# wangkenpu/rsrgan

Measured on AMD Instinct MI355X. Metric: GAN train frames/sec (G+D step), 257-dim LPS->40-dim MFCC, higher is better.
Workload: dtype f32

## Files before the change

rsrgan_amd/csrc/capi_ops.cpp:

```cpp
#include "capi_common.h"

extern "C" {

int rsrgan_op_launch_floor(int32_t n, int32_t mode, double* us_per_launch, void* stream) {
  if (n <= 0 || !us_per_launch) { set_error("op_launch_floor: bad argument"); return RSRGAN_ERR_INVALID; }
  static float* buf = nullptr;
  if (!buf && hipMalloc((void**)&buf, 2 * 65536 * 4 * sizeof(float)) != hipSuccess) { set_error("hipMalloc failed"); return RSRGAN_ERR_HIP; }
  hipStream_t s = nullptr;
  hipGraph_t g = nullptr; hipGraphExec_t ge = nullptr;
  hipEvent_t e0 = nullptr, e1 = nullptr;
  int rc = RSRGAN_ERR_HIP;
  do {
    if (hipStreamCreateWithFlags(&s, hipStreamNonBlocking) != hipSuccess) break;
    if (hipMemsetAsync(buf, 0, 2 * 65536 * 4 * sizeof(float), s) != hipSuccess) break;
    if (hipStreamBeginCapture(s, hipStreamCaptureModeThreadLocal) != hipSuccess) break;
    launch_floor_chain(buf, buf + 65536 * 4, n, mode, s);
    if (hipStreamEndCapture(s, &g) != hipSuccess) break;
    if (hipGraphInstantiate(&ge, g, nullptr, nullptr, 0) != hipSuccess) break;
    if (hipEventCreate(&e0) != hipSuccess || hipEventCreate(&e1) != hipSuccess) break;
    if (hipGraphLaunch(ge, s) != hipSuccess) break;
    if (hipEventRecord(e0, s) != hipSuccess || hipGraphLaunch(ge, s) != hipSuccess || hipEventRecord(e1, s) != hipSuccess) break;
    if (hipEventSynchronize(e1) != hipSuccess) break;
    float ms = 0.f;
    if (hipEventElapsedTime(&ms, e0, e1) != hipSuccess) break;
    *us_per_launch = 1e3 * ms / n;
    rc = RSRGAN_OK;
  } while (0);
  if (rc != RSRGAN_OK) set_error("op_launch_floor: HIP call failed");
  if (e0) (void)hipEventDestroy(e0);
  if (e1) (void)hipEventDestroy(e1);
  if (ge) (void)hipGraphExecDestroy(ge);
  if (g) (void)hipGraphDestroy(g);
  if (s) (void)hipStreamDestroy(s);
  (void)stream;
  return rc;
}

static const size_t g_op_ws_floats = (size_t)32 << 20;
static const size_t g_op_scratch_floats = (size_t)2 << 20;
static float* op_ws() {
  static float* ws = nullptr;
  if (!ws && hipMalloc((void**)&ws, g_op_ws_floats * sizeof(float)) != hipSuccess) ws = nullptr;
  return ws;
}
static float* op_scratch() {
  static float* sc = nullptr;
  if (!sc && hipMalloc((void**)&sc, g_op_scratch_floats * sizeof(float)) != hipSuccess) sc = nullptr;
  return sc;
}
struct WorkersScope {
  int saved;
  explicit WorkersScope(int w) : saved(g_gemm_workers) { if (w > 0) g_gemm_workers = w; }
  ~WorkersScope() { g_gemm_workers = saved; }
};

int rsrgan_op_gemm(const float* A, int32_t lda, int32_t a_kc, const float* B, int32_t ldb, int32_t b_kc, float* C, int32_t ldc,
                   int32_t M, int32_t N, int32_t K, const float* bias, int32_t act, float alpha, int32_t accumulate, void* stream) {
  if (!A || !B || !C || (lda & 3) || (ldb & 3)) { set_error("op_gemm: null pointer or leading dimension not a multiple of 4"); return RSRGAN_ERR_INVALID; }
  float* ws = op_ws();
  launch_gemm(A, lda, a_kc != 0, B, ldb, b_kc != 0, C, ldc, M, N, K, bias, act, alpha, accumulate != 0, (hipStream_t)stream,
              ws, ws ? g_op_ws_floats : 0);
  OP_LAUNCHED("op_gemm");
}

int rsrgan_op_gemm2(const float* A, int32_t lda, int32_t a_kc, const float* A2, int32_t lda2, int32_t M1, const float* B, int32_t ldb,
                    int32_t b_kc, float* C, int32_t ldc, int32_t M, int32_t N, int32_t K, const float* bias, int32_t act, float alpha,
                    int32_t accumulate, int32_t map_rows_per, int64_t map_outer, int64_t map_inner, int32_t workers, int32_t force_cfg,
                    void* stream) {
  OP_REFUSE(!A || !B || !C, "op_gemm2: null pointer (A, B or C)");
  OP_REFUSE(M <= 0 || N <= 0 || K <= 0, "op_gemm2: M, N, K must be positive (got %d, %d, %d)", M, N, K);
  OP_REFUSE((lda & 3) || (ldb & 3) || (ldc & 3) || (A2 && (lda2 & 3)), "op_gemm2: leading dimension not a multiple of 4 (lda %d, lda2 %d, ldb %d, ldc %d)", lda, lda2, ldb, ldc);
  OP_REFUSE(workers < 0 || workers > 256, "op_gemm2: workers = %d outside 0 (default) .. 256", workers);
  OP_REFUSE(force_cfg < -1 || force_cfg > 7, "op_gemm2: force_cfg = %d outside -1 (planner) .. 7", force_cfg);
  OP_REFUSE(map_rows_per < 0, "op_gemm2: row map with rows_per = %d", map_rows_per);
  if (map_rows_per > 0) {
    OP_REFUSE(A2 != nullptr, "op_gemm2: A2 together with a row map");
    OP_REFUSE(b_kc != 0, "op_gemm2: a row map together with b_kcontig");
    OP_REFUSE((map_outer & 3) || (map_inner & 3), "op_gemm2: row map strides not multiples of 4 (outer %lld, inner %lld)", (long long)map_outer, (long long)map_inner);
  }
  if (A2) {
    OP_REFUSE(a_kc != 0, "op_gemm2: A2 together with a_kcontig (the stacked operand is m-contiguous)");
    OP_REFUSE(M1 <= 0 || M1 >= M, "op_gemm2: M1 = %d outside (0, M = %d)", M1, M);
    OP_REFUSE(M1 & 3, "op_gemm2: M1 = %d is not a multiple of 4: every kernel moves the stacked operand in 16-byte chunks", M1);
  }
  float* ws = op_ws();
  {
    WorkersScope wsc(workers);
    const GemmRowMap ma{map_rows_per, (long long)map_outer, (long long)map_inner};
    launch_gemm_mapped(A, lda, ma, A2, lda2, M1, a_kc != 0, B, ldb, b_kc != 0, C, ldc, M, N, K, bias, act, alpha, accumulate != 0,
                       (hipStream_t)stream, ws, ws ? g_op_ws_floats : 0, force_cfg);
  }
  OP_LAUNCHED("op_gemm2");
}

int rsrgan_op_gemm_batch(int32_t nb, const float* const* A, int32_t lda, const float* const* A2, int32_t lda2, int32_t M1,
                         const float* const* B, int32_t ldb, float* const* C, int32_t ldc, int32_t M, int32_t N, int32_t K,
                         int32_t accumulate, int32_t workers, void* stream) {
  OP_REFUSE(nb < 1 || nb > 64, "op_gemm_batch: nb = %d outside 1 .. 64 (more than %d: not applicable)", nb, GEMM_MAXB);
  OP_REFUSE(!A || !B || !C, "op_gemm_batch: null pointer table (A, B or C)");
  for (int b = 0; b < nb; ++b) OP_REFUSE(!A[b] || !B[b] || !C[b] || (A2 && !A2[b]), "op_gemm_batch: null pointer in problem %d", b);
  OP_REFUSE(M <= 0 || N <= 0 || K <= 0, "op_gemm_batch: M, N, K must be positive (got %d, %d, %d)", M, N, K);
  OP_REFUSE((lda & 3) || (ldb & 3) || (ldc & 3) || (A2 && (lda2 & 3)), "op_gemm_batch: leading dimension not a multiple of 4 (lda %d, lda2 %d, ldb %d, ldc %d)", lda, lda2, ldb, ldc);
// ... 17 lines not shown
                           int32_t accumulate, void* stream) {
  OP_REFUSE(n < 1 || n > GEMM16_MAXB, "op_gemm16_batch: n = %d outside the table (1 .. %d)", n, GEMM16_MAXB);
  OP_REFUSE(!A || !B || !C, "op_gemm16_batch: null pointer table (A, B or C)");
  for (int p = 0; p < n; ++p) OP_REFUSE(!A[p] || !B[p] || !C[p] || (A2 && !A2[p]), "op_gemm16_batch: null pointer in problem %d", p);
  OP_REFUSE(M <= 0 || N <= 0 || K <= 0, "op_gemm16_batch: M, N, K must be positive (got %d, %d, %d)", M, N, K);
  OP_REFUSE((lda & 3) || (ldb & 3) || (ldc & 3) || (A2 && (lda2 & 3)), "op_gemm16_batch: leading dimension not a multiple of 4 (lda %d, lda2 %d, ldb %d, ldc %d)", lda, lda2, ldb, ldc);
  if (A2) {
    OP_REFUSE(M1 <= 0 || M1 >= M, "op_gemm16_batch: M1 = %d outside (0, M = %d)", M1, M);
    OP_REFUSE(M1 & 3, "op_gemm16_batch: M1 = %d is not a multiple of 4: k_gemm16 loads the stacked operand as float4", M1);
  }
  Gemm16Batch bt{};
  bt.n = n;
  for (int p = 0; p < n; ++p) { bt.A[p] = A[p]; bt.A2[p] = A2 ? A2[p] : nullptr; bt.B[p] = B[p]; bt.C[p] = C[p]; }
  float* ws = op_ws();
  launch_gemm16_batch(bt, lda, lda2, M1, ldb, ldc, M, N, K, accumulate != 0, (hipStream_t)stream, ws, ws ? g_op_ws_floats : 0);
  OP_LAUNCHED("op_gemm16_batch");
}

int rsrgan_op_gemm_last_plan(int32_t out[8]) {
  OP_REFUSE(!out, "op_gemm_last_plan: null pointer");
  const GemmPlanRecord& r = g_gemm_last_plan;
  out[0] = r.cls; out[1] = r.bm; out[2] = r.bn; out[3] = r.W; out[4] = r.n_dp; out[5] = r.fixup; out[6] = r.splits; out[7] = r.Ur;
  return RSRGAN_OK;
}

int rsrgan_op_lstm_colsums(int32_t nb, const float* const* dz, const float* const* cprev, const float* const* ccur, float* const* db,
                           float* const* dwi, float* const* dwf, float* const* dwo, int32_t rows, int32_t H, void* stream) {
  OP_REFUSE(nb < 1 || nb > 4, "op_lstm_colsums: nb = %d outside the table (1 .. 4)", nb);
  OP_REFUSE(!dz || !cprev || !ccur || !db || !dwi || !dwf || !dwo, "op_lstm_colsums: null pointer table");
  for (int p = 0; p < nb; ++p)
    OP_REFUSE(!dz[p] || !cprev[p] || !ccur[p] || !db[p] || !dwi[p] || !dwf[p] || !dwo[p], "op_lstm_colsums: null pointer in layer %d", p);
  OP_REFUSE(rows <= 0 || H <= 0, "op_lstm_colsums: rows and H must be positive (got %d, %d)", rows, H);
  OP_REFUSE((size_t)nb * 64 * 7 * (size_t)H > g_op_scratch_floats, "op_lstm_colsums: nb x 64 x 7 x H = %zu floats of partials exceed the entry's scratch", (size_t)nb * 64 * 7 * (size_t)H);
  float* sc = op_scratch();
  if (!sc) { set_error("op_lstm_colsums: hipMalloc failed"); return RSRGAN_ERR_HIP; }
  if (nb == 1) launch_lstm_colsums(dz[0], cprev[0], ccur[0], db[0], dwi[0], dwf[0], dwo[0], rows, H, sc, (hipStream_t)stream);
  else {
    ColsumsBatch cb{};
    cb.n = nb;
    for (int p = 0; p < nb; ++p) { cb.dz[p] = dz[p]; cb.cprev[p] = cprev[p]; cb.ccur[p] = ccur[p]; cb.db[p] = db[p]; cb.dwi[p] = dwi[p]; cb.dwf[p] = dwf[p]; cb.dwo[p] = dwo[p]; }
    launch_lstm_colsums_batch(cb, rows, H, sc, (hipStream_t)stream);
  }
  OP_LAUNCHED("op_lstm_colsums");
}

int rsrgan_op_colsum(const float* a, int32_t lda, const float* b, int32_t ldb, float* out, int32_t rows, int32_t cols, int32_t tall,
                     void* stream) {
  OP_REFUSE(!a || !out, "op_colsum: null pointer (a or out)");
  OP_REFUSE(rows <= 0 || cols <= 0, "op_colsum: rows and cols must be positive (got %d, %d)", rows, cols);
  OP_REFUSE(lda < cols || (b && ldb < cols), "op_colsum: leading dimension below cols = %d (lda %d, ldb %d)", cols, lda, ldb);
  OP_REFUSE(tall && b, "op_colsum: the tall form has no multiplier b");
  OP_REFUSE((size_t)(tall ? 512 : 64) * (size_t)cols > g_op_scratch_floats, "op_colsum: cols = %d exceeds the entry's scratch", cols);
  float* sc = op_scratch();
  if (!sc) { set_error("op_colsum: hipMalloc failed"); return RSRGAN_ERR_HIP; }
  if (tall) launch_colsum_tall(a, lda, out, rows, cols, sc, g_op_scratch_floats, (hipStream_t)stream);
  else launch_colsum(a, lda, b, ldb, out, rows, cols, sc, (hipStream_t)stream);
  OP_LAUNCHED("op_colsum");
}

int rsrgan_op_bnl_fold(const float* Wx, const float* Wh, const float* const bn[12], const float* bias, int32_t P, int32_t H, float* KxT,
                       int32_t ldI, float* KhT, int32_t ldP, float* bias_f, float* ca, float* cb, void* stream) {
  OP_REFUSE(!Wx || !Wh || !bn || !bias || !KxT || !KhT || !bias_f || !ca || !cb, "op_bnl_fold: null pointer");
  for (int k = 0; k < 12; ++k) OP_REFUSE(!bn[k], "op_bnl_fold: null pointer in bn[%d]", k);
  OP_REFUSE(P <= 0 || H <= 0, "op_bnl_fold: P and H must be positive (got %d, %d)", P, H);
  OP_REFUSE(ldI < P || ldP < P, "op_bnl_fold: leading dimension below P = %d (ldI %d, ldP %d)", P, ldI, ldP);
  OP_REFUSE((long long)H * 4 * (long long)(ldI > ldP ? ldI : ldP) > (1ll << 28), "op_bnl_fold: 4H x ld exceeds the entry's 2^28 floats");
  BnlFold f{};
  f.Wx = Wx; f.Wh = Wh; f.bias = bias;
  for (int k = 0; k < 12; ++k) f.bn[k] = bn[k];
  f.P = P; f.H = H; f.ldI = ldI; f.ldP = ldP; f.eps = 1e-3f;
  f.KxT = KxT; f.KhT = KhT; f.bias_f = bias_f; f.ca = ca; f.cb = cb;
  launch_bnl_fold(f, (hipStream_t)stream);
  OP_LAUNCHED("op_bnl_fold");
}

static float* op_conv_ft(size_t floats) {
  static thread_local float* ft = nullptr;
  static thread_local size_t cap = 0;
  if (floats > cap) {
    if (ft) { (void)hipDeviceSynchronize(); (void)hipFree(ft); ft = nullptr; cap = 0; }
    if (hipMalloc((void**)&ft, floats * sizeof(float)) != hipSuccess) { ft = nullptr; return nullptr; }
    cap = floats;
  }
  return ft;
}
static inline int op_pad4(int n) { return (n + 3) & ~3; }
#define OP_CONV_SHAPE(who) \
  OP_REFUSE(C < 1 || N < 1 || S < 1 || W < 1 || fw < 1, who ": C, N, S, W, fw must be positive (got %d, %d, %d, %d, %d)", C, N, S, W, fw); \
  OP_REFUSE(R < 1, who ": R = %d frames", R); \
  OP_REFUSE((long long)R * S * W > (1 << 24), who ": R x S x W = %lld positions exceed the entry's 2^24", (long long)R * S * W)

int rsrgan_op_conv_supported(int32_t C, int32_t N, int32_t S, int32_t W, int32_t fw) {
  OP_REFUSE(C < 1 || N < 1 || S < 1 || W < 1 || fw < 1, "op_conv_supported: C, N, S, W, fw must be positive (got %d, %d, %d, %d, %d)", C, N, S, W, fw);
  return (conv_fwd_supported(C, N, S, W, fw) ? 1 : 0) | (conv_wgrad_supported(C, N, S, W, fw) ? 2 : 0);
}

int64_t rsrgan_op_conv_ws_floats(int32_t C, int32_t R_max, int32_t S, int32_t W, int32_t fw) {
  OP_REFUSE(C < 1 || R_max < 1 || S < 1 || W < 1 || fw < 1, "op_conv_ws_floats: C, R_max, S, W, fw must be positive (got %d, %d, %d, %d, %d)", C, R_max, S, W, fw);
  return (int64_t)conv_wgrad_ws_floats(C, R_max, S, W, fw);
}

int rsrgan_op_conv_fwd(const float* in, int32_t ldc_in, int32_t C, const float* F, int32_t ldf, int32_t flip, const float* bias, int32_t relu,
                       const float* mask, float* out, int32_t ldc_out, int32_t N, int32_t R, int32_t S, int32_t W, int32_t fw, void* stream) {
  OP_REFUSE(!in || !F || !out, "op_conv_fwd: null pointer (in, F or out)");
  OP_CONV_SHAPE("op_conv_fwd");
  OP_REFUSE((ldc_in & 3) || (ldc_out & 3) || (ldf & 3), "op_conv_fwd: leading dimension not a multiple of 4 (ldc_in %d, ldc_out %d, ldf %d)", ldc_in, ldc_out, ldf);
  OP_REFUSE(ldc_in < op_pad4(C) || ldc_out < op_pad4(N) || ldf < (flip ? C : N),
            "op_conv_fwd: leading dimension below its row (ldc_in %d for C = %d, ldc_out %d for N = %d, ldf %d for %d filter columns)", ldc_in, C, ldc_out, N, ldf, flip ? C : N);
  OP_REFUSE(((size_t)in & 15) || ((size_t)out & 15) || ((size_t)mask & 15), "op_conv_fwd: in, out or mask not 16-byte aligned");
// ... 568 lines not shown
      case 0: launch_sumsq(FP(0), ct, FP(1), s); break;
      case 1: launch_dw_reduce(FP(0), (size_t)d[3], (int)d[4], dsrc, FP(1), ct, FP(2), s); break;
      case 2: launch_l2(FP(0), FP(1), ct, FP(2), FP(3), s); break;
      case 3: launch_apply_sgd(FP(0), FP(1), FP(2), ct, FP(3), FP(4), s); break;
      default: launch_apply_adam(FP(0), FP(1), FP(2), FP(3), FP(4), ct, FP(5), FP(6), s, (int)d[3]); break;
    }
    OP_LAUNCH_OK(WHO);
    HIPC(hipStreamSynchronize(s));
    return RSRGAN_OK;
  });
}
#undef WHO

#define WHO "op_step_elem"
int rsrgan_op_step_elem(int32_t op, const void* const* ptrs, const int64_t* dims, const float* fl, void* stream) {
  OP_REFUSE(!ptrs, WHO ": null table (ptrs)");
  OP_REFUSE(op < 0 || op > 8, WHO ": op = %d outside 0 .. 8", op);
  OP_REFUSE(op != 3 && !dims, WHO ": null table (dims)");
  OP_REFUSE((op == 0 || op >= 5) && !fl, WHO ": null table (fl: the clip bounds, the betas, keep or alpha)");
  const int64_t* d = dims;
  hipStream_t s = (hipStream_t)stream;
  switch (op) {
    case 0: {
      OP_DIM("T", d[0], 1); OP_DIM("Nd", d[1], 1); OP_LD("ldl", d[3], 1); OP_FLAG("clip_on", d[4]);
      OP_REFUSE(d[2] < 0 || d[2] > d[1], WHO ": n_real = %lld outside 0 .. Nd = %lld", (long long)d[2], (long long)d[1]);
      OP_REFUSE(d[0] * d[1] > (1 << 24), WHO ": T x Nd above the entry's 2^24");
      OP_BP("Nd", d[1], d[5], d[6]); OP_BP("n_real", d[2], d[5], d[6]);
      OP_PTR("logits", ptrs[0], 4); OP_OPT("dlogits", ptrs[1], 4); OP_PTR("t_real", ptrs[2], 4); OP_PTR("t_fake", ptrs[3], 4); OP_PTR("loss3", ptrs[4], 4);
      launch_lsgan(FP(0), (int)d[3], FP(1), (int)d[0], (int)d[1], (int)d[2], FP(2), FP(3), FP(4), s, d[4] != 0, fl[0], fl[1], (int)d[5], (int)d[6]);
      break;
    }
    case 1: {
      OP_DIM("T", d[0], 1); OP_DIM("Nd", d[1], 1); OP_DIM("dR", d[3], 1); OP_MUL4("dR", d[3]);
      OP_REFUSE(d[3] + 3 > 64, WHO ": dR = %lld above 60 (k_dhead2 sums 3 + dR <= 64 quantities)", (long long)d[3]);
      OP_REFUSE(d[2] < 0 || d[2] > d[1], WHO ": n_real = %lld outside 0 .. Nd = %lld", (long long)d[2], (long long)d[1]);
      OP_REFUSE(d[0] * d[1] > (1 << 24), WHO ": T x Nd above the entry's 2^24");
      OP_FLAG("want_grads", d[8]); OP_FLAG("want_wgrads", d[9]);
      OP_LD("ldt", d[4], d[3]); OP_MUL4("ldt", d[4]); OP_LD("ldw", d[5], 1); OP_LD("ldl", d[6], 1);
      if (d[8]) { OP_LD("ldo", d[7], d[3]); OP_MUL4("ldo", d[7]); }
      OP_BP("Nd", d[1], d[10], d[11]); OP_BP("n_real", d[2], d[10], d[11]);
      static const char* const names[12] = {"top", "w", "b", "logits", "dlogits", "dout", "gw", "gb", "t_real", "t_fake", "loss3", "part"};
      for (int i = 0; i < 12; ++i) {
        const bool wanted = i < 4 || i > 7 || (i < 6 ? d[8] != 0 : d[9] != 0);
        const int align = (i == 0 || i == 5) ? 16 : 4;
        if (wanted) OP_PTR(names[i], ptrs[i], align); else OP_OPT(names[i], ptrs[i], align);
      }
      const int64_t need = (d[0] * d[1] + 63) / 64 * (DH_MAXR + 3);
      OP_REFUSE(d[12] < need, WHO ": part of %lld floats below ceil(T x Nd / 64) x %d = %lld", (long long)d[12], DH_MAXR + 3, (long long)need);
      DHeadArgs a{};
      a.top = FP(0); a.ldt = (int)d[4]; a.w = FP(1); a.ldw = (int)d[5]; a.b = FP(2);
      a.logits = FP(3); a.ldl = (int)d[6]; a.dlogits = FP(4); a.dout = FP(5); a.ldo = (int)d[7]; a.gw = FP(6); a.gb = FP(7);
      a.T = (int)d[0]; a.Nd = (int)d[1]; a.n_real = (int)d[2]; a.dR = (int)d[3]; a.t_real = FP(8); a.t_fake = FP(9); a.loss3 = FP(10); a.part = FP(11);
      a.want_grads = (int)d[8]; a.want_wgrads = (int)d[9]; a.Bp = (int)d[10]; a.Bt = (int)d[11];
      launch_dhead(a, s);
      break;
    }
    case 2: {
      OP_DIM("rows", d[0], 1); OP_DIM("D", d[1], 1); OP_LD("ld", d[2], d[1]); OP_FLAG("accumulate", d[3]);
      OP_REFUSE(d[0] * d[2] > ((int64_t)1 << 30), WHO ": rows x ld above the entry's 2^30");
      OP_BP("rows", d[0], d[4], d[5]);
      OP_REFUSE(d[6] < 1024, WHO ": scratch of %lld floats below launch_mse's 1024", (long long)d[6]);
      OP_PTR("y", ptrs[0], 4); OP_PTR("lab", ptrs[1], 4); OP_OPT("dy", ptrs[2], 4); OP_PTR("lambda", ptrs[3], 4); OP_PTR("loss", ptrs[4], 4); OP_PTR("scratch", ptrs[5], 4);
      launch_mse(FP(0), FP(1), (int)d[2], FP(2), (int)d[0], (int)d[1], FP(3), d[3] != 0, FP(4), FP(5), s, (int)d[4], (int)d[5]);
      break;
    }
    case 3:
      OP_PTR("l4", ptrs[0], 4); OP_PTR("lambda", ptrs[1], 4);
      launch_g_total(FP(0), FP(1), s);
      break;
    case 4:
      OP_DIM("n", d[0], 1);
      OP_PTR("partial", ptrs[0], 4); OP_PTR("l2_scale", ptrs[1], 4); OP_PTR("out", ptrs[2], 4);
      launch_l2_total(FP(0), (int)d[0], FP(1), FP(2), s);
      break;
    case 5: {
      const bool g = d[0] == DYN_G_LR && d[1] == DYN_ADAM_LRT, dd = d[0] == DYN_D_LR && d[1] == DYN_ADAM_LRT_D;
      OP_REFUSE(!g && !dd, WHO ": slots (%lld, %lld) are neither (%d, %d) (G) nor (%d, %d) (D)", (long long)d[0], (long long)d[1], (int)DYN_G_LR,
                (int)DYN_ADAM_LRT, (int)DYN_D_LR, (int)DYN_ADAM_LRT_D);
      OP_REFUSE(!(fl[0] >= 0.f && fl[0] < 1.f) || !(fl[1] >= 0.f && fl[1] < 1.f), WHO ": beta1 = %g or beta2 = %g outside [0, 1)", (double)fl[0], (double)fl[1]);
      OP_PTR("dyn", ptrs[0], 4); OP_PTR("t", ptrs[1], 4);
      launch_adam_tick(FP(0), (int*)ptrs[1], (double)fl[0], (double)fl[1], s, (int)d[0], (int)d[1]);
      break;
    }
    case 6: case 7: case 8: {
      OP_DIM("rows", d[0], 1); OP_DIM("cols", d[1], 1); OP_LD("ld", d[2], d[1]);
      OP_REFUSE(d[0] * d[2] > ((int64_t)1 << 30), WHO ": rows x ld above the entry's 2^30");
      if (op != 8) OP_REFUSE(!(fl[0] > 0.f && fl[0] <= 1.f), WHO ": keep = %g outside (0, 1]", (double)fl[0]);
      if (op == 6) OP_REFUSE(d[4] < 0 || d[4] > (1 << 24), WHO ": thr = %lld outside 0 .. 2^24", (long long)d[4]);
      OP_PTR(op == 8 ? "h" : "y", ptrs[0], 4);
      if (op != 6) OP_PTR("d", ptrs[1], 4);
      if (op == 6) launch_dropout_fwd(FP(0), (size_t)d[0], (int)d[1], (int)d[2], (unsigned long long)d[3], (unsigned)d[4], fl[0], s);
      else if (op == 7) launch_dropout_bwd(FP(0), FP(1), (size_t)d[0], (int)d[1], (int)d[2], fl[0], s);
      else launch_lrelu_bwd(FP(0), FP(1), (size_t)d[0], (int)d[1], (int)d[2], fl[0], s);
      break;
    }
  }
  OP_LAUNCHED(WHO);
}
#undef WHO

#define OP_JOB_NAME(buf, name, j) char buf[48]; snprintf(buf, sizeof(buf), "%s of job %d", name, (int)(j))
#define WHO "op_layout"
int rsrgan_op_layout(int32_t op, const void* const* ptrs, const int64_t* dims, const float* fl, void* stream) {
  OP_REFUSE(!ptrs || !dims, WHO ": null table (ptrs or dims)");
  OP_REFUSE(op < 0 || op > 18, WHO ": op = %d outside 0 .. 18", op);
  OP_REFUSE(op == 14 && !fl, WHO ": null table (fl: the fill value)");
  const int64_t* d = dims;
  const int64_t lim = (int64_t)1 << 30;
  hipStream_t s = (hipStream_t)stream;
  switch (op) {
    case 0: case 1: {
      OP_DIM("B", d[0], 1); OP_DIM("T", d[1], 1); OP_DIM("D", d[2], 1); OP_LD("ld", d[3], d[2]);
      OP_REFUSE(d[0] * d[1] * d[3] > lim || d[0] > 65535, WHO ": B x T x ld above the entry's 2^30, or B above the grid's 65535");
      if (op == 1) OP_REFUSE(d[4] < 0 || d[4] > d[0], WHO ": Bt = %lld outside 0 (all rows) .. B = %lld", (long long)d[4], (long long)d[0]);
      OP_PTR("src", ptrs[0], 4); OP_PTR("dst", ptrs[1], 4);
      if (op == 0) launch_pack_tm(FP(0), FP(1), (int)d[0], (int)d[1], (int)d[2], (int)d[3], s);
// ... 205 lines not shown
```

rsrgan_amd/csrc/gemm.hip:

```cpp
#include <algorithm>
#include <type_traits>
#include <cstdio>
#include <cstdlib>

#include "kernels.h"

namespace rsr {

typedef float f32x16 __attribute__((ext_vector_type(16)));
typedef const __attribute__((address_space(1))) void* gptr_t;
typedef __attribute__((address_space(3))) void* lptr_t;

constexpr int GK = 32;
#ifndef RSR_GEMM_MINW
#define RSR_GEMM_MINW 2
#endif
#ifndef RSR_GEMM_ABL
#define RSR_GEMM_ABL 0
#endif
constexpr int BK = 16;
__device__ __attribute__((aligned(16))) float g_zero_chunk[4] = {0.f, 0.f, 0.f, 0.f};
#if RSR_GEMM_ABL & 8
__device__ unsigned long long g_gemm_clk[4];
#endif
// ... 594 lines not shown
        *c = v;
      }
    }
}
template <bool AKC, bool BKC>
__global__ __launch_bounds__(256) void k_gemm16(const float* __restrict__ A, int lda, const float* __restrict__ B, int ldb,
                                              float* __restrict__ C, int ldc, int M, int N, int K,
                                              const float* __restrict__ bias, int act, float alpha, int accumulate,
                                              float* __restrict__ ws, int ldw, int kt_per_split,
                                              const float* __restrict__ A2, int lda2, int M1) {
  gemm16_body<AKC, BKC>(A, lda, B, ldb, C, ldc, M, N, K, bias, act, alpha, accumulate, ws, ldw, kt_per_split, A2, lda2, M1, blockIdx.z);
}
__global__ __launch_bounds__(256) void k_gemm16_b(const Gemm16Batch bt, int lda, int ldb, int ldc, int M, int N, int K, int accumulate,
                                                  float* __restrict__ ws, int ldw, int kt_per_split, int nsplit, int lda2, int M1) {
  const int p = blockIdx.z / nsplit, zs = blockIdx.z - p * nsplit;
  gemm16_body<false, false>(bt.A[p], lda, bt.B[p], ldb, bt.C[p], ldc, M, N, K, nullptr, 0, 0.f, accumulate,
                            ws ? ws + (size_t)p * nsplit * M * ldw : nullptr, ldw, kt_per_split, bt.A2[p], lda2, M1, zs);
}
__global__ __launch_bounds__(256) void k_splitk_reduce_b(const float* __restrict__ ws, int ldw, int splits, const Gemm16Batch bt, int ldc,
                                                         int M, int N, int accumulate) {
  const int p = blockIdx.y;
  const float* w = ws + (size_t)p * splits * M * ldw;
  float* C = bt.C[p];
  const size_t total = (size_t)M * N;
  for (size_t i = (size_t)blockIdx.x * blockDim.x + threadIdx.x; i < total; i += (size_t)gridDim.x * blockDim.x) {
    const int row = (int)(i / N), col = (int)(i % N);
    float v = 0.f;
#pragma unroll 8
    for (int z = 0; z < splits; ++z) v += w[((size_t)z * M + row) * ldw + col];
    float* c = C + (size_t)row * ldc + col;
    if (accumulate) v += *c;
    *c = v;
  }
}

__global__ __launch_bounds__(256) void k_splitk_reduce(const float* __restrict__ ws, int ldw, int splits, float* __restrict__ C,
                                                       int ldc, int M, int N, const float* __restrict__ bias, int act,
                                                       float alpha, int accumulate) {
  const size_t total = (size_t)M * N;
  for (size_t i = (size_t)blockIdx.x * blockDim.x + threadIdx.x; i < total; i += (size_t)gridDim.x * blockDim.x) {
    const int row = (int)(i / N), col = (int)(i % N);
    float v = 0.f;
#pragma unroll 8
    for (int z = 0; z < splits; ++z) v += ws[((size_t)z * M + row) * ldw + col];
    if (bias) v += bias[col];
    if (act == 1) v = fmaxf(v, alpha * v);
    else if (act == 2) v = fmaxf(v, 0.f);
    float* c = C + (size_t)row * ldc + col;
    if (accumulate) v += *c;
    *c = v;
  }
}


constexpr int NBM = 256, NBN = 32, NLDA = 260, NLDB = 36;
template <bool AKC>
__global__ __launch_bounds__(256) void k_gemm_n32(const float* __restrict__ A, int lda, const float* __restrict__ B, int ldb,
                                                  float* __restrict__ C, int ldc, int M, int N, int K,
                                                  const float* __restrict__ bias, int act, float alpha, int accumulate,
                                                  float* __restrict__ ws, int ldw, int kt_per_split) {
  __shared__ __attribute__((aligned(16))) float As[BK][NLDA];
  __shared__ __attribute__((aligned(16))) float Bs[BK][NLDB];
  const int tid = threadIdx.x, lane = tid & 63, w = tid >> 6;
  const int m0 = blockIdx.y * NBM;
  const int l31 = lane & 31, lh = lane >> 5;
  f32x16 acc[2];
#pragma unroll
  for (int i = 0; i < 2; ++i)
#pragma unroll
    for (int r = 0; r < 16; ++r) acc[i][r] = 0.f;
  const int KA = AKC ? ((K + 3) & ~3) : K;
  const int MA = AKC ? M : ((M + 3) & ~3);
  const int NB = (N + 3) & ~3;
  const int nk_all = (K + BK - 1) / BK;
  const int kt0 = blockIdx.z * kt_per_split;
  const int nk = min(nk_all, kt0 + kt_per_split);
  float4 ra[4], rb;
  auto load = [&](int kt) {
    const int k0 = kt * BK;
#pragma unroll
    for (int u = 0; u < 4; ++u) {
      const int idx = tid + 256 * u;
      float4 v = make_float4(0.f, 0.f, 0.f, 0.f);
      if (AKC) {
        const int x = m0 + (idx >> 2), k = k0 + (idx & 3) * 4;
        if (x < MA && k < KA) v = *reinterpret_cast<const float4*>(A + (size_t)x * lda + k);
      } else {
        const int k = k0 + (idx >> 6), x = m0 + (idx & 63) * 4;
        if (k < K && x < MA) v = *reinterpret_cast<const float4*>(A + (size_t)k * lda + x);
      }
      ra[u] = v;
    }
    rb = make_float4(0.f, 0.f, 0.f, 0.f);
    if (tid < 128) {
      const int k = k0 + (tid >> 3), x = (tid & 7) * 4;
      if (k < K && x < NB) rb = *reinterpret_cast<const float4*>(B + (size_t)k * ldb + x);
    }
  };
  auto store = [&]() {
#pragma unroll
    for (int u = 0; u < 4; ++u) {
      const int idx = tid + 256 * u;
      if (AKC) {
        const int x = idx >> 2, k = (idx & 3) * 4;
        As[k + 0][x] = ra[u].x; As[k + 1][x] = ra[u].y; As[k + 2][x] = ra[u].z; As[k + 3][x] = ra[u].w;
      } else {
// ... 149 lines not shown
template <bool AKC, bool BKC, bool MAPA>
void launch_layout(GemmArgs& g, hipStream_t s, float* ws, size_t ws_floats, int force_cfg) {
  static const int cfgs[][2] = {{128, 128}, {96, 128}, {128, 96}, {256, 64}, {256, 32}, {256, 256}, {128, 256}, {256, 128}};
  int best = 0;
  Plan bp{};
  if (force_cfg >= 0 && force_cfg < 8) {
    best = force_cfg;
    bp = plan_cfg(g.M, g.N, g.K, cfgs[best][0], cfgs[best][1], g_gemm_workers, ws, ws_floats);
  } else
  for (int c = 0; c < (switches().gemm_self ? 8 : 5); ++c) {
    if (c >= 5 && (long long)((g.M + cfgs[c][0] - 1) / cfgs[c][0]) * ((g.N + cfgs[c][1] - 1) / cfgs[c][1]) < 2LL * g_gemm_workers) continue;
    Plan pl = plan_cfg(g.M, g.N, g.K, cfgs[c][0], cfgs[c][1], g_gemm_workers, ws, ws_floats);
    if (c == 0 || pl.cost < 0.97 * bp.cost) { best = c; bp = pl; }
  }
  switch (best) {
    case 1: launch_cfg<AKC, BKC, 3, 1, 1, MAPA>(g, bp, s, ws); break;
    case 2: launch_cfg<AKC, BKC, 1, 3, 4, MAPA>(g, bp, s, ws); break;
    case 3: launch_cfg<AKC, BKC, 2, 2, 4, MAPA>(g, bp, s, ws); break;
    case 4: launch_cfg<AKC, BKC, 2, 1, 4, MAPA>(g, bp, s, ws); break;
    case 5: launch_cfg_s<AKC, BKC, 4, 4, 2, MAPA>(g, bp, s, ws); break;
    case 6: launch_cfg_s<AKC, BKC, 2, 4, 2, MAPA>(g, bp, s, ws); break;
    case 7: launch_cfg_s<AKC, BKC, 4, 2, 2, MAPA>(g, bp, s, ws); break;
    default: launch_cfg<AKC, BKC, 2, 2, 2, MAPA>(g, bp, s, ws); break;
  }
}
}

static void launch_gemm16(const float* A, int lda, const float* A2, int lda2, int M1, bool a_kc, const float* B, int ldb, bool b_kc,
                          float* C, int ldc, int M, int N, int K, const float* bias, int act, float alpha, bool accumulate,
                          hipStream_t s, float* ws, size_t ws_floats) {
  const int gx = (N + BN - 1) / BN, gy = (M + BM - 1) / BM;
  const int nk = (K + GBK - 1) / GBK;
  int splits = 1;
  const int ldw = (N + 3) & ~3;
  if (ws && gx * gy < 192 && nk * GBK >= 128) {
    int cap = 64;
    while (cap > 1 && (size_t)cap * M * ldw > ws_floats) --cap;
    splits = pick_splits(gx * gy, nk, (size_t)M * ldw * sizeof(float), cap, 1.2 * GBK / 16, GBK == 16 ? 4 : 2);
  }
  const int per = std::max(1, (nk + splits - 1) / splits);
  splits = std::max(1, (nk + per - 1) / per);
  float* w = splits > 1 ? ws : nullptr;
  dim3 grid(gx, gy, splits), block(256);
  const int acc = accumulate ? 1 : 0;
  g_gemm_last_plan = GemmPlanRecord{GEMM_CLS_GEMM16, BM, BN, 0, 0, 0, splits, 0};
  if (a_kc && !b_kc)
    hipLaunchKernelGGL((k_gemm16<true, false>), grid, block, 0, s, A, lda, B, ldb, C, ldc, M, N, K, bias, act, alpha, acc, w, ldw, per, nullptr, 0, 0);
  else if (a_kc && b_kc)
    hipLaunchKernelGGL((k_gemm16<true, true>), grid, block, 0, s, A, lda, B, ldb, C, ldc, M, N, K, bias, act, alpha, acc, w, ldw, per, nullptr, 0, 0);
  else if (!a_kc && !b_kc)
    hipLaunchKernelGGL((k_gemm16<false, false>), grid, block, 0, s, A, lda, B, ldb, C, ldc, M, N, K, bias, act, alpha, acc, w, ldw, per, A2, lda2, M1);
  else
    hipLaunchKernelGGL((k_gemm16<false, true>), grid, block, 0, s, A, lda, B, ldb, C, ldc, M, N, K, bias, act, alpha, acc, w, ldw, per, A2, lda2, M1);
  if (splits > 1) {
    const size_t total = (size_t)M * N;
    const int blocks = (int)std::min<size_t>(2048, (total + 255) / 256);
    hipLaunchKernelGGL(k_splitk_reduce, dim3(blocks), dim3(256), 0, s, ws, ldw, splits, C, ldc, M, N, bias, act, alpha, acc);
  }
}


void launch_gemm16_batch(const Gemm16Batch& bt, int lda, int lda2, int M1, int ldb, int ldc, int M, int N, int K, bool accumulate,
                         hipStream_t s, float* ws, size_t ws_floats) {
  if (bt.n <= 0 || M <= 0 || N <= 0 || K <= 0) return;
  for (int p = 0; p < bt.n; ++p) require_m1_chunked(bt.A2[p], M1, "launch_gemm16_batch");
  const int gx = (N + BN - 1) / BN, gy = (M + BM - 1) / BM;
  const int nk = (K + GBK - 1) / GBK;
  int splits = 1;
  const int ldw = (N + 3) & ~3;
  if (ws && gx * gy * bt.n < 192 && nk * GBK >= 128) {
    int cap = 64;
    while (cap > 1 && (size_t)cap * bt.n * M * ldw > ws_floats) --cap;
    splits = pick_splits(gx * gy * bt.n, nk, (size_t)M * ldw * sizeof(float), cap, 1.2 * GBK / 16, GBK == 16 ? 4 : 2);
  }
  const int per = std::max(1, (nk + splits - 1) / splits);
  splits = std::max(1, (nk + per - 1) / per);
  float* w = splits > 1 ? ws : nullptr;
  g_gemm_last_plan = GemmPlanRecord{GEMM_CLS_GEMM16_B, BM, BN, 0, 0, 0, splits, 0};
  hipLaunchKernelGGL(k_gemm16_b, dim3(gx, gy, splits * bt.n), dim3(256), 0, s, bt, lda, ldb, ldc, M, N, K, accumulate ? 1 : 0, w, ldw, per,
                     splits, lda2, M1);
  if (splits > 1) {
    const size_t total = (size_t)M * N;
    const int blocks = (int)std::min<size_t>(2048, (total + 255) / 256);
    hipLaunchKernelGGL(k_splitk_reduce_b, dim3(blocks, bt.n), dim3(256), 0, s, ws, ldw, splits, bt, ldc, M, N, accumulate ? 1 : 0);
  }
}

void launch_gemm_mapped(const float* A, int lda, const GemmRowMap& ma, const float* A2, int lda2, int M1, bool a_kc, const float* B, int ldb,
                        bool b_kc, float* C, int ldc, int M, int N, int K, const float* bias, int act, float alpha,
                        bool accumulate, hipStream_t s, float* ws, size_t ws_floats, int force_cfg) {
  if (M <= 0 || N <= 0 || K <= 0) return;
  const bool mapped = ma.rows_per > 0;
  if (!a_kc && !mapped) require_m1_chunked(A2, M1, "launch_gemm_mapped");
  if (mapped && b_kc) { fprintf(stderr, "rsrgan: launch_gemm_mapped: a row map of A with a k-contiguous B is not instantiated\n"); abort(); }
  if (N <= NBN && !b_kc && !A2 && M >= NBM && !mapped && force_cfg < 0) {
    const int gy = (M + NBM - 1) / NBM, nk = (K + BK - 1) / BK, ldw = (N + 3) & ~3;
    int splits = 1;
    if (ws && gy < 192 && nk >= 8) {
      int cap = 64;
      while (cap > 1 && (size_t)cap * M * ldw > ws_floats) --cap;
      splits = pick_splits(gy, nk, (size_t)M * ldw * sizeof(float), cap);
    }
    const int per = std::max(1, (nk + splits - 1) / splits);
    splits = std::max(1, (nk + per - 1) / per);
    float* w = splits > 1 ? ws : nullptr;
    dim3 grid(1, gy, splits), block(256);
    const int acc = accumulate ? 1 : 0;
    g_gemm_last_plan = GemmPlanRecord{GEMM_CLS_N32, NBM, NBN, 0, 0, 0, splits, 0};
    if (a_kc) hipLaunchKernelGGL((k_gemm_n32<true>), grid, block, 0, s, A, lda, B, ldb, C, ldc, M, N, K, bias, act, alpha, acc, w, ldw, per);
    else hipLaunchKernelGGL((k_gemm_n32<false>), grid, block, 0, s, A, lda, B, ldb, C, ldc, M, N, K, bias, act, alpha, acc, w, ldw, per);
    if (splits > 1) {
      const size_t total = (size_t)M * N;
      const int blocks = (int)std::min<size_t>(2048, (total + 255) / 256);
      hipLaunchKernelGGL(k_splitk_reduce, dim3(blocks), dim3(256), 0, s, ws, ldw, splits, C, ldc, M, N, bias, act, alpha, acc);
    }
    return;
  }
  const double outs = (double)M * N;
  if (force_cfg < 0 && !mapped && !(K >= 256 && outs >= 4.0e6) && !(K >= 2048 && outs >= 1.5e6)) {
    launch_gemm16(A, lda, a_kc ? nullptr : A2, lda2, M1, a_kc, B, ldb, b_kc, C, ldc, M, N, K, bias, act, alpha, accumulate, s, ws, ws_floats);
    return;
  }
  GemmArgs g{};
  g.A = A; g.A2 = a_kc ? nullptr : A2; g.B = B; g.bias = bias; g.C = C;
  g.lda = lda; g.lda2 = lda2; g.M1 = M1; g.ldb = ldb; g.ldc = ldc; g.M = M; g.N = N; g.K = K;
  g.act = act; g.accumulate = accumulate ? 1 : 0; g.alpha = alpha;
  g.ma = ma;
  if (mapped) {
    g.A2 = nullptr;
    if (a_kc) launch_layout<true, false, true>(g, s, ws, ws_floats, force_cfg);
    else launch_layout<false, false, true>(g, s, ws, ws_floats, force_cfg);
  }
  else if (a_kc && !b_kc) launch_layout<true, false, false>(g, s, ws, ws_floats, force_cfg);
  else if (a_kc && b_kc) launch_layout<true, true, false>(g, s, ws, ws_floats, force_cfg);
  else if (!a_kc && !b_kc) launch_layout<false, false, false>(g, s, ws, ws_floats, force_cfg);
  else launch_layout<false, true, false>(g, s, ws, ws_floats, force_cfg);
}

bool launch_gemm_batch(int nb, const float* const* A, int lda, const float* const* A2, int lda2, int M1, const float* const* B, int ldb,
                       float* const* C, int ldc, int M, int N, int K, bool accumulate, hipStream_t s, float* ws, size_t ws_floats) {
  const int form = switches().gemm_batch;
  if (!form || nb < 2 || nb > GEMM_MAXB || M <= 0 || N <= 0 || K <= 0 || !ws) return false;
  const double outs = (double)M * N;
  if (!(K >= 256 && outs >= 4.0e6) && !(K >= 2048 && outs >= 1.5e6)) return false;
  if (A2) for (int b = 0; b < nb; ++b) require_m1_chunked(A2[b], M1, "launch_gemm_batch");
  GemmArgs g{};
  g.A = A[0]; g.A2 = A2 ? A2[0] : nullptr; g.B = B[0]; g.bias = nullptr; g.C = C[0];
  g.lda = lda; g.lda2 = lda2; g.M1 = M1; g.ldb = ldb; g.ldc = ldc; g.M = M; g.N = N; g.K = K;
  g.act = 0; g.accumulate = accumulate ? 1 : 0; g.alpha = 0.f;
  g.ma = GemmRowMap{0, 0, 0};
  GemmBatch bt{};
  bt.nb = nb;
  for (int b = 0; b < nb; ++b) { bt.Ab[b] = A[b]; bt.A2b[b] = A2 ? A2[b] : nullptr; bt.Bb[b] = B[b]; bt.Cb[b] = C[b]; }
  const int pad192 = (M + 191) / 192 * 192, pad128 = (M + 127) / 128 * 128;
  if (form == 1 && pad192 < pad128 && 2 * (size_t)g_gemm_workers * 192 * 256 <= ws_floats) {
    const int tn1 = (N + 255) / 256;
    const int bw = switches().gemm_batch_w;
    const Plan pl = plan_cfg(M, nb * tn1 * 256, K, 192, 256, bw ? std::min(bw, g_gemm_workers) : g_gemm_workers, ws, ws_floats);
    if (!pl.whole) { launch_cfg_s<false, false, 3, 4, 2, false, GemmBatch>(g, pl, s, ws, &bt); return true; }
  }
  const int tn1 = (N + 127) / 128;
  const Plan pl = plan_cfg(M, nb * tn1 * 128, K, 128, 128, g_gemm_workers, ws, ws_floats);
  launch_cfg<false, false, 2, 2, 2, false>(g, pl, s, ws, &bt);
  return true;
}

void launch_gemm2(const float* A, int lda, const float* A2, int lda2, int M1, bool a_kc, const float* B, int ldb, bool b_kc,
                  float* C, int ldc, int M, int N, int K, const float* bias, int act, float alpha, bool accumulate,
// ... 13 lines not shown
```

rsrgan_amd/csrc/kernels.h:

```cpp
#pragma once
#include <hip/hip_runtime.h>
#include <stdint.h>

#include <vector>

#include "switches.h"

namespace rsr {

constexpr int MAXJ = 8;

struct Place { int x0, nx, sb, se, nb, w; };
constexpr int JOBMAP_MAX = 768;
struct JobMap { int valid; unsigned char job[JOBMAP_MAX]; };
struct PlanItem { int ncol, nrow; double cost; int mult; };
int plan_places(int n, const PlanItem* items, Place* out);

enum { DYN_G_LR = 0, DYN_D_LR = 1, DYN_LAMBDA = 2, DYN_D_REAL = 3, DYN_D_FAKE = 4, DYN_L2 = 5, DYN_CLIP = 6,
       DYN_B1 = 7, DYN_B2 = 8, DYN_EPS = 9, DYN_EMA = 10, DYN_ADAM_LRT = 11, DYN_ADAM_LRT_D = 12, DYN_COUNT = 16 };

struct FwdGateJob {
  const float* x;
  const float* KxT;
  const float* m;
// ... 221 lines not shown
                 float* splitk_ws = nullptr, size_t splitk_ws_floats = 0);

struct StagePack { const float* src; float* dst; int D, ld; };
struct StageCopy { const void* src; void* dst; int n; };
struct StageJobs { StagePack pack[2]; StageCopy copy[4]; int B, T; int Bt; };
void launch_stage_inputs(const StageJobs& j, hipStream_t s);
void launch_pack_tm(const float* src_bm, float* dst_tm, int B, int T, int D, int ld, hipStream_t s);
void launch_unpack_bm(const float* src_tm, int ld, float* dst_bm, int B, int T, int D, hipStream_t s, int Bt = 0);
void launch_build_d_input(const float* lab_tm, const float* y_tm, const float* noise_r, const float* noise_f,
                          float* xd, int B, int T, int D, int ld, bool with_real, hipStream_t s);
void launch_add_noise_rows(const float* src_tm, const float* noise, float* dst, int B, int T, int D, int ld,
                           int Ns, int row0, hipStream_t s);
void launch_transpose(const float* src, int lds, float* dst, int ldd, int R, int C, hipStream_t s);
void launch_fill(float* p, size_t n, float v, hipStream_t s);
struct SwizzleJob { const float* src; float* dst; int ld, gates, H, C, c0, K1, I, P, kx, nct, nkb, blk_base; };
struct SwizzleList { int n; SwizzleJob j[24]; };
void launch_swizzle_many(SwizzleList& sl, hipStream_t s);
inline size_t swizzle_floats(int nct, int nkb) { return (size_t)nct * nkb * 256; }
struct TransposeJob { const float* src; float* dst; int lds, ldd, R, C, blk_base; };
struct TransposeList { int n; TransposeJob j[16]; };
void launch_transpose_many(TransposeList& tl, hipStream_t s);
size_t conv_prep_floats(int S, int fw, int C);
void launch_conv_prep(const float* F, int ldf_src, int S, int fw, int Cin, int Cout, bool flip, float* Ft, hipStream_t s);
bool conv_fwd_supported(int C, int N, int S, int W, int fw);
void launch_conv_fwd(const float* in, int ldc_in, int C, const float* Ft, const float* bias, bool relu, float* out, int ldc_out, int N,
                     int R, int S, int W, int fw, hipStream_t s,
                     const float* mask = nullptr );
bool conv_wgrad_supported(int C, int N, int S, int W, int fw);
size_t conv_wgrad_ws_floats(int C, int R, int S, int W, int fw);
void launch_conv_wgrad(const float* in, int ldc_in, int C, const float* d, int ldc_d, int N, float* dW, int ldw, float* ws, int R, int S,
                       int W, int fw, hipStream_t s,
                       float* db = nullptr );
enum { CONV_FAM_NONE = 0, CONV_FAM_FWD = 1 , CONV_FAM_FWD4 = 2 ,
       CONV_FAM_WGRAD = 3 , CONV_FAM_WGRAD4 = 4  };
enum { CONV_BR_WHOLE = 1, CONV_BR_MAIN = 2, CONV_BR_REM = 3, CONV_BR_WG_K2 = 1, CONV_BR_WG_ROWS = 2, CONV_BR_WG_SEARCH = 3 };
struct ConvLaunchRecord {
  int family, a0, a1, a2;
  int branch, TW, FB, gx, gy, gz, lds;
  int DH, fpg, groups, nstrips, nkg, PS, waves, gmax;
};
struct ConvPlanRecord { int n; ConvLaunchRecord l[2]; };
extern thread_local ConvPlanRecord g_conv_last_plan;
void launch_im2col(const float* src, size_t row_stride, int ldc, int C, int S, int W, int kh, int kw, float* col, int ldk, size_t M,
                   hipStream_t s);
void launch_expand_c4(const float* src, int ld_src, int n, float* dst, size_t rows, hipStream_t s);
void launch_col2im(const float* dcol, int ldk, int C, int S, int W, int kh, int kw, float* dst, int ldc, size_t M, hipStream_t s);
struct GStateLayer { float *c, *mst; int H, P, ldP, off; };
struct GStateArgs { GStateLayer L[GP_MAXL]; int nl, SF, rows, dir; float* state; size_t slot; const int* mask; };
void launch_gstate(const GStateArgs& a, hipStream_t s);
void launch_window_len(const int* len, int* dst, int n, int t0, int Tw, hipStream_t s);
struct ZeroList { int n; float* p[32]; unsigned len[32]; };
void launch_zero_many(const ZeroList& zl, hipStream_t s);
struct ColsumsBatch { const float* dz[4]; const float* cprev[4]; const float* ccur[4]; float* db[4]; float* dwi[4]; float* dwf[4]; float* dwo[4]; int n; };
void launch_lstm_colsums_batch(const ColsumsBatch& bt, int rows, int H, float* scratch, hipStream_t s);
void launch_lstm_colsums(const float* dz, const float* cprev, const float* ccur, float* db, float* dwi, float* dwf, float* dwo,
                         int rows, int H, float* scratch , hipStream_t s);
void launch_lrelu_bwd(const float* hval, float* d, size_t rows, int cols, int ld, float alpha, hipStream_t s);
void launch_dropout_fwd(float* y, size_t rows, int cols, int ld, unsigned long long key, unsigned thr, float keep, hipStream_t s);
void launch_dropout_bwd(const float* y, float* d, size_t rows, int cols, int ld, float keep, hipStream_t s);
void launch_colsum_tall(const float* a, int lda, float* out, int rows, int cols, float* scratch, size_t scratch_floats, hipStream_t s);

struct BnVars {
  float *beta, *gamma;
  float *mm, *mv, *rm, *rmw, *rs, *rsw;
};
constexpr int BN_STAT_ROWS = 6;
void launch_bn_forward(const float* z, int ldz, float* y, int ldy, int rows, int cols, const BnVars& v, float* stat, int ldc, bool training,
                       bool relu, float* scratch, size_t scratch_floats, hipStream_t s, int calls = 1);
void launch_bn_backward(float* dy, int ldd, const float* y, int ldy, const float* z, int ldz, int rows, int cols, const float* stat, int ldc,
                        float* dbeta, float* dgamma, bool accumulate, bool relu, float* sums, float* scratch, size_t scratch_floats,
                        hipStream_t s, int calls = 1);
void launch_bn_commit(int cols, const BnVars& v, const float* stat, int ldc, int times, hipStream_t s);
struct BnCommit { BnVars v; const float* stat; int cols, ldc, times0, times1; };
struct BnCommitList { int n; BnCommit e[24]; };
void launch_bn_commit_many(const BnCommitList& cl, hipStream_t s);
enum { BN_ROUTE_NONE = 0, BN_ROUTE_SMALL = 1, BN_ROUTE_SLICED = 2, BN_ROUTE_NARROW = 3 };
struct BnPlanRecord { int route, backward, calls, launches, slices, per, pgx, pgy, egrid, q, R; };
extern thread_local BnPlanRecord g_bn_last_plan;
int bn_seq_count(int rows, int Bp, int Bt);
void launch_bn_seq_forward(const float* z, int ldz, float* y, int ldy, int rows, int cols, const BnVars& v, float* stat, int ldc, bool training,
                           bool act, float alpha, int Bp, int Bt, float* scratch, size_t scratch_floats, hipStream_t s);
void launch_bn_seq_backward(float* dy, int ldd, const float* y, int ldy, const float* z, int ldz, int rows, int cols, const float* stat, int ldc,
                            float* dbeta, float* dgamma, bool accumulate, bool act, float alpha, int Bp, int Bt, float* sums, float* scratch,
                            size_t scratch_floats, hipStream_t s);
void launch_bn_seq_fold(float* W, int ldw, int K, int cols, const BnVars& v, float* bias, hipStream_t s);
void launch_feat_batch(const float* raw, long long raw_rows, const int* offsets, int B, int T, int D, int left, int right, const double* mean,
                       const double* stddev, float* out, int* lengths, hipStream_t s);
void launch_feat_frames(const float* pool, long long pool_rows, const int* picks, int N, int D, int left, int right, const double* mean,
                        const double* stddev, float* out, hipStream_t s);
void launch_feat_stream(const float* fresh, long long fresh_rows, const int* table, float* hist, int B, int H, int T, int D, int left, int right,
                        const double* mean, const double* stddev, float* out, int* lengths, hipStream_t s);
void launch_feat_denorm(const float* y, const int* lengths, int B, int T, int D, const double* mean, const double* stddev, double* out,
                        hipStream_t s);
void launch_feat_decode(const uint8_t* blob, long long blob_bytes, const long long* seg, const float* scale, const int* offsets, int B, int D,
                        const double* mean, const double* stddev, float* out, long long out_rows, hipStream_t s);
int wave_frames(int P);
void launch_feat_wave(const void* pcm, int kind, long long n_samples, const long long* seg, const int* offsets, int B, int N, int S, int P,
                      float preemph, const float* window, const float* twiddle, float* out, long long out_rows, hipStream_t s);
constexpr int HIST_MAX_TENSORS = 16;
constexpr int hist_nl() {
  int k = 0;
  for (double v = 1e-12; v < 1e20; v *= 1.1) ++k;
  return 2 * (k + 1) + 1;
}
constexpr int HIST_NL = hist_nl();
constexpr int HIST_REC = 5 + HIST_NL;
struct HistView { const float* x; long long ld, cs; unsigned rows, cols; int clip; };
const std::vector<double>& hist_limits();
bool launch_hist(int n, const HistView* views, float clip_lo, float clip_hi, double* out, hipStream_t s);
void launch_logits_dense(const float* logits, int frame_rows, int B, int T, float* out, bool clip, float clip_lo, float clip_hi, hipStream_t s);
void launch_colsum(const float* a, int lda, const float* b, int ldb, float* out, int rows, int cols,
                   float* scratch , hipStream_t s);

constexpr int DH_MAXR = 64;
struct DHeadArgs {
  const float* top; int ldt; const float* w; int ldw; const float* b;
  float* logits; int ldl; float* dlogits; float* dout; int ldo; float* gw; float* gb;
  int T, Nd, n_real, dR; const float* t_real; const float* t_fake; float* loss3; float* part; int want_grads, want_wgrads;
  int Bp, Bt;
};
void launch_dhead(const DHeadArgs& a, hipStream_t s);
void launch_lsgan(const float* logits, int ldl, float* dlogits, int T, int Nd, int n_real,
                  const float* target_real, const float* target_fake, float* loss3, hipStream_t s,
                  bool clip_on = false, float clip_lo = 0.f, float clip_hi = 0.f, int Bp = 0, int Bt = 0);
void launch_build_joint(const float* x, int ldx, int off, int dim, const float* tail, int ldt, int Dt, float* joint, int ldj,
                        int row0, int R, hipStream_t s);
void launch_slice_cols(const float* src, int lds, int off, float* dst, int ldd, int R, int C, hipStream_t s);
void launch_mse(const float* y, const float* lab, int ld, float* dy, int rows, int D, const float* lambda,
                bool accumulate, float* loss_out, float* scratch , hipStream_t s, int Bp = 0, int Bt = 0);
void launch_g_total(float* l4 , const float* lambda, hipStream_t s);
void launch_copy_f(const float* src, float* dst, int n, hipStream_t s);

struct ChunkTable {
  const int* tensor;
  const int* off;
  const int* len;
  const int* t_first;
  const int* t_count;
  const int* t_l2;
  int n_chunks, n_tensors;
};
void launch_sumsq(const float* g, const ChunkTable& ct, float* partial, hipStream_t s);
void launch_dw_reduce(const float* ws, size_t stride, int ntiles, const long long* src, float* g, const ChunkTable& ct, float* partial, hipStream_t s);
void launch_l2(const float* w, float* g, const ChunkTable& ct, const float* l2_scale, float* partial, hipStream_t s);
void launch_l2_total(const float* partial, int n_chunks, const float* l2_scale, float* out, hipStream_t s);
void launch_apply_sgd(float* w, const float* g, float* ema, const ChunkTable& ct, const float* partial,
                      const float* dyn, hipStream_t s);
void launch_apply_adam(float* w, const float* g, float* m, float* v, float* ema, const ChunkTable& ct,
                       const float* partial, const float* dyn, hipStream_t s, int lrt_slot = DYN_ADAM_LRT);
void launch_adam_tick(float* dyn, int* t, double b1, double b2, hipStream_t s, int lr_slot = DYN_G_LR, int lrt_slot = DYN_ADAM_LRT);
void launch_pad_copy(const float* dense, float* padded, int rows, int cols, int ld, bool to_padded, hipStream_t s);

}
```

rsrgan_amd/csrc/kernels.hip:

```cpp
#include <algorithm>
#include <cstdlib>

#include "kernels.h"

namespace rsr {

typedef float f32x4 __attribute__((ext_vector_type(4)));

__device__ __forceinline__ float sigmoid_(float x) { return 1.0f / (1.0f + expf(-x)); }

#ifdef RSR_TRACE
__device__ unsigned long long g_trace[8192 * 16];
#define TR_BEGIN() do { if (threadIdx.x == 0 && blockIdx.x < 8192) { unsigned long long* t_ = g_trace + (size_t)blockIdx.x * 16; \
    t_[0] = __builtin_amdgcn_s_memrealtime(); t_[1] = __builtin_amdgcn_s_memtime(); \
    t_[14] = __builtin_amdgcn_s_getreg(4 | (0 << 6) | (31 << 11)); t_[15] = __builtin_amdgcn_s_getreg(20 | (0 << 6) | (3 << 11)); \
    for (int i_ = 2; i_ < 14; ++i_) t_[i_] = 0; } } while (0)
#define TR_ID(ptr) do { if (threadIdx.x == 0 && blockIdx.x < 8192) g_trace[(size_t)blockIdx.x * 16 + 12] = (unsigned long long)(size_t)(ptr); } while (0)
#define TR(i) do { if (threadIdx.x == 0 && blockIdx.x < 8192) g_trace[(size_t)blockIdx.x * 16 + (i)] = __builtin_amdgcn_s_memtime(); } while (0)
#define TR_END() do { if (threadIdx.x == 0 && blockIdx.x < 8192) { g_trace[(size_t)blockIdx.x * 16 + 9] = __builtin_amdgcn_s_memtime(); \
    g_trace[(size_t)blockIdx.x * 16 + 13] = __builtin_amdgcn_s_memrealtime(); } } while (0)
#else
#define TR_BEGIN() do { } while (0)
#define TR_ID(ptr) do { } while (0)
#define TR(i) do { } while (0)
// ... 1216 lines not shown
    float* sm = sc + L.H;
    if (a.dir == 0) {
      for (int i = tid; i < L.H; i += blockDim.x) c[i] = sc[i];
      for (int i = tid; i < L.ldP; i += blockDim.x) m[i] = i < L.P ? sm[i] : 0.f;
    } else {
      for (int i = tid; i < L.H; i += blockDim.x) sc[i] = c[i];
      for (int i = tid; i < L.P; i += blockDim.x) sm[i] = m[i];
    }
  }
}
void launch_gstate(const GStateArgs& a, hipStream_t s) {
  if (a.rows <= 0) return;
  hipLaunchKernelGGL(k_gstate, dim3(a.rows), dim3(256), 0, s, a);
}

__global__ void k_window_len(const int* __restrict__ len, int* __restrict__ dst, int n, int t0, int Tw) {
  const int b = blockIdx.x * blockDim.x + threadIdx.x;
  if (b < n) dst[b] = min(max(len[b] - t0, 0), Tw);
}
void launch_window_len(const int* len, int* dst, int n, int t0, int Tw, hipStream_t s) {
  if (n <= 0) return;
  hipLaunchKernelGGL(k_window_len, dim3((n + 255) / 256), dim3(256), 0, s, len, dst, n, t0, Tw);
}

__global__ void k_zero_many(ZeroList zl) {
  const int j = blockIdx.y;
  if (j >= zl.n) return;
  float* p = zl.p[j];
  const size_t n = zl.len[j];
  for (size_t i = (size_t)blockIdx.x * blockDim.x + threadIdx.x; i < n; i += (size_t)gridDim.x * blockDim.x) p[i] = 0.f;
}
void launch_zero_many(const ZeroList& zl, hipStream_t s) {
  if (zl.n == 0) return;
  hipLaunchKernelGGL(k_zero_many, dim3(32, zl.n), dim3(256), 0, s, zl);
}

__global__ void k_fill(float* p, size_t n, float v) {
  for (size_t i = (size_t)blockIdx.x * blockDim.x + threadIdx.x; i < n; i += (size_t)gridDim.x * blockDim.x) p[i] = v;
}
void launch_fill(float* p, size_t n, float v, hipStream_t s) {
  if (n == 0) return;
  const int blocks = (int)min((size_t)2048, (n + 255) / 256);
  hipLaunchKernelGGL(k_fill, dim3(blocks), dim3(256), 0, s, p, n, v);
}

__global__ void k_lrelu_bwd(const float* __restrict__ hval, float* __restrict__ d, size_t rows, int cols, int ld, float alpha) {
  const size_t total = rows * (size_t)cols;
  for (size_t i = (size_t)blockIdx.x * blockDim.x + threadIdx.x; i < total; i += (size_t)gridDim.x * blockDim.x) {
    const size_t r = i / cols; const int c = (int)(i % cols);
    const size_t o = r * ld + c;
    if (!(hval[o] > 0.f)) d[o] *= alpha;
  }
}
void launch_lrelu_bwd(const float* hval, float* d, size_t rows, int cols, int ld, float alpha, hipStream_t s) {
  const size_t total = rows * cols;
  const int blocks = (int)min((size_t)2048, (total + 255) / 256);
  hipLaunchKernelGGL(k_lrelu_bwd, dim3(blocks), dim3(256), 0, s, hval, d, rows, cols, ld, alpha);
}

__global__ void k_drop_tick(unsigned long long* ctr) { if (threadIdx.x == 0) *ctr += 1ull; }
void launch_drop_tick(unsigned long long* ctr, hipStream_t s) { hipLaunchKernelGGL(k_drop_tick, dim3(1), dim3(64), 0, s, ctr); }
__global__ __launch_bounds__(256) void k_dropout_fwd(float* __restrict__ y, size_t rows, int cols, int ld, unsigned long long key, unsigned thr,
                                                     float keep) {
  const size_t n = rows * (size_t)cols;
  for (size_t i = (size_t)blockIdx.x * 256 + threadIdx.x; i < n; i += (size_t)gridDim.x * 256) {
    const size_t r = i / cols;
    float* p = y + r * ld + (i - r * cols);
    const bool on = (unsigned)(splitmix64(key + i) >> 40) < thr;
    *p = on ? *p / keep : 0.f;
  }
}
void launch_dropout_fwd(float* y, size_t rows, int cols, int ld, unsigned long long key, unsigned thr, float keep, hipStream_t s) {
  const size_t n = rows * (size_t)cols;
  if (n == 0) return;
  hipLaunchKernelGGL(k_dropout_fwd, dim3((unsigned)std::min<size_t>((n + 255) / 256, 8192)), dim3(256), 0, s, y, rows, cols, ld, key, thr, keep);
}
__global__ __launch_bounds__(256) void k_dropout_bwd(const float* __restrict__ y, float* __restrict__ d, size_t rows, int cols, int ld, float keep) {
  const size_t n = rows * (size_t)cols;
  for (size_t i = (size_t)blockIdx.x * 256 + threadIdx.x; i < n; i += (size_t)gridDim.x * 256) {
    const size_t r = i / cols, o = r * ld + (i - r * cols);
    d[o] = y[o] > 0.f ? d[o] / keep : 0.f;
  }
}
void launch_dropout_bwd(const float* y, float* d, size_t rows, int cols, int ld, float keep, hipStream_t s) {
  const size_t n = rows * (size_t)cols;
  if (n == 0) return;
  hipLaunchKernelGGL(k_dropout_bwd, dim3((unsigned)std::min<size_t>((n + 255) / 256, 8192)), dim3(256), 0, s, y, d, rows, cols, ld, keep);
}

constexpr int CS_SLICES = 64;
__global__ __launch_bounds__(256) void k_colsum1(const float* __restrict__ a, int lda, const float* __restrict__ b, int ldb,
                                                 float* __restrict__ scratch, int rows, int cols) {
  __shared__ float red[4][64];
  const int c = blockIdx.x * 64 + (threadIdx.x & 63), rl = threadIdx.x >> 6;
  const int per = (rows + CS_SLICES - 1) / CS_SLICES;
  const int rbeg = blockIdx.y * per, rend = min(rows, rbeg + per);
  float s = 0.f;
  if (c < cols) {
    for (int r = rbeg + rl; r < rend; r += 4) {
      const float v = a[(size_t)r * lda + c];
      s += b ? v * b[(size_t)r * ldb + c] : v;
    }
  }
  red[rl][threadIdx.x & 63] = s;
  __syncthreads();
  if (rl == 0 && c < cols)
    scratch[(size_t)blockIdx.y * cols + c] = ((red[0][threadIdx.x] + red[1][threadIdx.x]) + red[2][threadIdx.x]) + red[3][threadIdx.x];
}
__global__ void k_colsum2(const float* __restrict__ scratch, float* __restrict__ out, int cols) {
  const int c = blockIdx.x * blockDim.x + threadIdx.x;
  if (c >= cols) return;
  float s = 0.f;
  for (int i = 0; i < CS_SLICES; ++i) s += scratch[(size_t)i * cols + c];
  out[c] = s;
}
__global__ __launch_bounds__(256) void k_colsum1_n(const float* __restrict__ a, int lda, float* __restrict__ scratch, int rows, int cols,
                                                   int per) {
  __shared__ float red[4][64];
  const int c = blockIdx.x * 64 + (threadIdx.x & 63), rl = threadIdx.x >> 6;
  const int rbeg = blockIdx.y * per, rend = min(rows, rbeg + per);
  float s = 0.f;
  if (c < cols) {
#pragma unroll 4
    for (int r = rbeg + rl; r < rend; r += 4) s += a[(size_t)r * lda + c];
  }
  red[rl][threadIdx.x & 63] = s;
  __syncthreads();
  if (rl == 0 && c < cols)
    scratch[(size_t)blockIdx.y * cols + c] = ((red[0][threadIdx.x] + red[1][threadIdx.x]) + red[2][threadIdx.x]) + red[3][threadIdx.x];
}
__global__ __launch_bounds__(256) void k_colsum2_n(const float* __restrict__ scratch, float* __restrict__ out, int cols, int slices) {
  __shared__ float red[4][64];
  const int c = blockIdx.x * 64 + (threadIdx.x & 63), g = threadIdx.x >> 6;
  float s = 0.f;
  if (c < cols) {
#pragma unroll 4
    for (int i = g; i < slices; i += 4) s += scratch[(size_t)i * cols + c];
  }
  red[g][threadIdx.x & 63] = s;
  __syncthreads();
  if (g == 0 && c < cols) out[c] = ((red[0][threadIdx.x] + red[1][threadIdx.x]) + red[2][threadIdx.x]) + red[3][threadIdx.x];
}
void launch_colsum_tall(const float* a, int lda, float* out, int rows, int cols, float* scratch, size_t scratch_floats, hipStream_t s) {
  int slices = (int)std::min<size_t>(512, scratch_floats / (size_t)std::max(cols, 1));
  slices = std::max(1, std::min(slices, (rows + 63) / 64));
  const int per = (rows + slices - 1) / slices;
  slices = (rows + per - 1) / per;
  hipLaunchKernelGGL(k_colsum1_n, dim3((cols + 63) / 64, slices), dim3(256), 0, s, a, lda, scratch, rows, cols, per);
  hipLaunchKernelGGL(k_colsum2_n, dim3((cols + 63) / 64), dim3(256), 0, s, scratch, out, cols, slices);
}

__global__ __launch_bounds__(256) void k_lstm_colsums1(const float* __restrict__ dz, const float* __restrict__ cprev,
                                                       const float* __restrict__ ccur, float* __restrict__ scratch, int rows, int H) {
  __shared__ float red[7][4][64];
  const int c = blockIdx.x * 64 + (threadIdx.x & 63), rl = threadIdx.x >> 6;
  const int per = (rows + CS_SLICES - 1) / CS_SLICES;
  const int rbeg = blockIdx.y * per, rend = min(rows, rbeg + per);
  float s[7] = {0.f, 0.f, 0.f, 0.f, 0.f, 0.f, 0.f};
  if (c < H) {
#pragma unroll 4
    for (int r = rbeg + rl; r < rend; r += 4) {
      const float* z = dz + (size_t)r * 4 * H + c;
      const float di = z[0], dj = z[H], df = z[2 * H], d_o = z[3 * H];
      const float cp = cprev[(size_t)r * H + c], cc = ccur[(size_t)r * H + c];
      s[0] += di; s[1] += dj; s[2] += df; s[3] += d_o; s[4] += di * cp; s[5] += df * cp; s[6] += d_o * cc;
    }
  }
// ... 21 lines not shown
}
__global__ __launch_bounds__(256) void k_lstm_colsums1_b(const ColsumsBatch bt, float* __restrict__ scratch, int rows, int H) {
  __shared__ float red[7][4][64];
  const int p = blockIdx.z;
  const float* __restrict__ dz = bt.dz[p]; const float* __restrict__ cprev = bt.cprev[p]; const float* __restrict__ ccur = bt.ccur[p];
  scratch += (size_t)p * CS_SLICES * 7 * H;
  const int c = blockIdx.x * 64 + (threadIdx.x & 63), rl = threadIdx.x >> 6;
  const int per = (rows + CS_SLICES - 1) / CS_SLICES;
  const int rbeg = blockIdx.y * per, rend = min(rows, rbeg + per);
  float s[7] = {0.f, 0.f, 0.f, 0.f, 0.f, 0.f, 0.f};
  if (c < H) {
#pragma unroll 4
    for (int r = rbeg + rl; r < rend; r += 4) {
      const float* z = dz + (size_t)r * 4 * H + c;
      const float di = z[0], dj = z[H], df = z[2 * H], d_o = z[3 * H];
      const float cp = cprev[(size_t)r * H + c], cc = ccur[(size_t)r * H + c];
      s[0] += di; s[1] += dj; s[2] += df; s[3] += d_o; s[4] += di * cp; s[5] += df * cp; s[6] += d_o * cc;
    }
  }
#pragma unroll
  for (int k = 0; k < 7; ++k) red[k][rl][threadIdx.x & 63] = s[k];
  __syncthreads();
  if (rl == 0 && c < H) {
    const int x = threadIdx.x;
#pragma unroll
    for (int k = 0; k < 7; ++k)
      scratch[((size_t)blockIdx.y * 7 + k) * H + c] = ((red[k][0][x] + red[k][1][x]) + red[k][2][x]) + red[k][3][x];
  }
}
__global__ void k_lstm_colsums2_b(const float* __restrict__ scratch, const ColsumsBatch bt, int H) {
  const int p = blockIdx.y;
  scratch += (size_t)p * CS_SLICES * 7 * H;
  const int c = blockIdx.x * blockDim.x + threadIdx.x;
  if (c >= H) return;
  float s[7] = {0.f, 0.f, 0.f, 0.f, 0.f, 0.f, 0.f};
#pragma unroll 8
  for (int i = 0; i < CS_SLICES; ++i)
#pragma unroll
    for (int k = 0; k < 7; ++k) s[k] += scratch[((size_t)i * 7 + k) * H + c];
  float* db = bt.db[p];
  db[c] = s[0]; db[H + c] = s[1]; db[2 * H + c] = s[2]; db[3 * H + c] = s[3];
  bt.dwi[p][c] = s[4]; bt.dwf[p][c] = s[5]; bt.dwo[p][c] = s[6];
}
void launch_lstm_colsums_batch(const ColsumsBatch& bt, int rows, int H, float* scratch, hipStream_t s) {
  hipLaunchKernelGGL(k_lstm_colsums1_b, dim3((H + 63) / 64, CS_SLICES, bt.n), dim3(256), 0, s, bt, scratch, rows, H);
  hipLaunchKernelGGL(k_lstm_colsums2_b, dim3((H + 255) / 256, bt.n), dim3(256), 0, s, scratch, bt, H);
}
void launch_lstm_colsums(const float* dz, const float* cprev, const float* ccur, float* db, float* dwi, float* dwf, float* dwo,
                         int rows, int H, float* scratch, hipStream_t s) {
  hipLaunchKernelGGL(k_lstm_colsums1, dim3((H + 63) / 64, CS_SLICES), dim3(256), 0, s, dz, cprev, ccur, scratch, rows, H);
  hipLaunchKernelGGL(k_lstm_colsums2, dim3((H + 255) / 256), dim3(256), 0, s, scratch, db, dwi, dwf, dwo, H);
}

void launch_colsum(const float* a, int lda, const float* b, int ldb, float* out, int rows, int cols, float* scratch, hipStream_t s) {
  hipLaunchKernelGGL(k_colsum1, dim3((cols + 63) / 64, CS_SLICES), dim3(256), 0, s, a, lda, b, ldb, scratch, rows, cols);
  hipLaunchKernelGGL(k_colsum2, dim3((cols + 255) / 256), dim3(256), 0, s, scratch, out, cols);
}

__device__ __forceinline__ float block_sum_1024(float v, float* red) {
  for (int o = 32; o > 0; o >>= 1) v += __shfl_down(v, o, 64);
  const int w = threadIdx.x >> 6;
  if ((threadIdx.x & 63) == 0) red[w] = v;
  __syncthreads();
  float s = 0.f;
  const int nw = (blockDim.x + 63) >> 6;
  for (int i = 0; i < nw; ++i) s += red[i];
  __syncthreads();
  return s;
}

__global__ __launch_bounds__(1024) void k_lsgan(const float* __restrict__ logits, int ldl, float* __restrict__ dlogits,
                                                int T, int Nd, int n_real, const float* __restrict__ t_real,
                                                const float* __restrict__ t_fake, float* __restrict__ loss3,
                                                int clip_on, float clip_lo, float clip_hi, int Bp, int Bt) {
  __shared__ float red[16];
  const int rows = T * Nd;
  const float tr = *t_real, tf = *t_fake;
  const int nr_ = Bp > 0 ? n_real / Bp * Bt : n_real, nf_ = Bp > 0 ? (Nd - n_real) / Bp * Bt : Nd - n_real;
  const float cr = (float)T * (float)nr_, cf = (float)T * (float)nf_;
  float sr = 0.f, sf = 0.f;
  for (int r = threadIdx.x; r < rows; r += blockDim.x) {
    const bool real = (r % Nd) < n_real;
    const bool valid = Bp <= 0 || ((r % Nd) % Bp) < Bt;
    const float raw = logits[(size_t)r * ldl];
    const float val = clip_on ? fminf(fmaxf(raw, clip_lo), clip_hi) : raw;
    const float d = valid ? val - (real ? tr : tf) : 0.f;
    if (real) sr += d * d; else sf += d * d;
    if (dlogits) dlogits[(size_t)r * ldl] = (clip_on && (raw < clip_lo || raw > clip_hi)) ? 0.f : 2.f * d / (real ? cr : cf);
  }
  sr = block_sum_1024(sr, red);
  sf = block_sum_1024(sf, red);
  if (threadIdx.x == 0) {
    const float lr_ = n_real > 0 ? sr / cr : 0.f;
    const float lf_ = (Nd - n_real) > 0 ? sf / cf : 0.f;
    loss3[0] = lr_; loss3[1] = lf_; loss3[2] = lr_ + lf_;
  }
}
void launch_lsgan(const float* logits, int ldl, float* dlogits, int T, int Nd, int n_real,
                  const float* t_real, const float* t_fake, float* loss3, hipStream_t s, bool clip_on, float clip_lo, float clip_hi,
                  int Bp, int Bt) {
  hipLaunchKernelGGL(k_lsgan, dim3(1), dim3(1024), 0, s, logits, ldl, dlogits, T, Nd, n_real, t_real, t_fake, loss3,
                     clip_on ? 1 : 0, clip_lo, clip_hi, Bp, Bt);
}

__global__ __launch_bounds__(64) void k_dhead1(const DHeadArgs a) {
  __shared__ float wsh[DH_MAXR + 1];
  const int lane = threadIdx.x;
  const int rows = a.T * a.Nd, dR = a.dR;
  if (lane < dR) wsh[lane] = a.w[(size_t)lane * a.ldw];
  if (lane == 0) wsh[DH_MAXR] = a.b[0];
  __syncthreads();
  const int r = blockIdx.x * 64 + lane;
  const bool on = r < rows;
  const float tr = *a.t_real, tf = *a.t_fake;
  const int nr_ = a.Bp > 0 ? a.n_real / a.Bp * a.Bt : a.n_real, nf_ = a.Bp > 0 ? (a.Nd - a.n_real) / a.Bp * a.Bt : a.Nd - a.n_real;
  const float cr = (float)a.T * (float)nr_, cf = (float)a.T * (float)nf_;
  float x[DH_MAXR];
  float logit = wsh[DH_MAXR];
  const float* xr = a.top + (size_t)(on ? r : 0) * a.ldt;
#pragma unroll
  for (int c = 0; c < DH_MAXR; c += 4) {
    float4 v = make_float4(0.f, 0.f, 0.f, 0.f);
    if (c < dR) v = *reinterpret_cast<const float4*>(xr + c);
    x[c] = v.x; x[c + 1] = v.y; x[c + 2] = v.z; x[c + 3] = v.w;
  }
#pragma unroll
  for (int c = 0; c < DH_MAXR; ++c) if (c < dR) logit += x[c] * wsh[c];
  const bool real = on && (r % a.Nd) < a.n_real;
  const bool valid = a.Bp <= 0 || ((r % a.Nd) % a.Bp) < a.Bt;
  const float d = valid ? logit - (real ? tr : tf) : 0.f;
  float sr = (on && real) ? d * d : 0.f, sf = (on && !real) ? d * d : 0.f;
  const float dl = on ? 2.f * d / (real ? cr : cf) : 0.f;
  if (on) {
    a.logits[(size_t)r * a.ldl] = logit;
    if (a.want_grads) {
      a.dlogits[(size_t)r * a.ldl] = dl;
      float* o = a.dout + (size_t)r * a.ldo;
#pragma unroll
      for (int c = 0; c < DH_MAXR; c += 4)
        if (c < dR) *reinterpret_cast<float4*>(o + c) = make_float4(dl * wsh[c], dl * wsh[c + 1], dl * wsh[c + 2], dl * wsh[c + 3]);
    }
  }
  auto wsum = [&](float v) { for (int o = 32; o > 0; o >>= 1) v += __shfl_down(v, o, 64); return v; };
  float* part = a.part + (size_t)blockIdx.x * (DH_MAXR + 3);
  sr = wsum(sr); sf = wsum(sf);
  if (lane == 0) { part[0] = sr; part[1] = sf; }
  if (a.want_wgrads) {
    const float sd = wsum(dl);
    if (lane == 0) part[2] = sd;
#pragma unroll
    for (int c = 0; c < DH_MAXR; ++c)
      if (c < dR) { const float v = wsum(x[c] * dl); if (lane == 0) part[3 + c] = v; }
  }
}
__global__ __launch_bounds__(1024) void k_dhead2(const DHeadArgs a, int nblocks) {
  __shared__ float tot[DH_MAXR + 3];
  const int q = threadIdx.x >> 4, j = threadIdx.x & 15;
  const int nq = a.want_wgrads ? 3 + a.dR : 2;
  float s = 0.f;
  if (q < nq)
    for (int b = j; b < nblocks; b += 16) s += a.part[(size_t)b * (DH_MAXR + 3) + q];
  s += __shfl_xor(s, 8); s += __shfl_xor(s, 4); s += __shfl_xor(s, 2); s += __shfl_xor(s, 1);
  if (q < nq && j == 0) {
    tot[q] = s;
    if (a.want_wgrads) {
      if (q == 2) a.gb[0] = s;
      if (q >= 3) a.gw[(size_t)(q - 3) * a.ldw] = s;
    }
  }
  __syncthreads();
  if (threadIdx.x == 0) {
    const int nr_ = a.Bp > 0 ? a.n_real / a.Bp * a.Bt : a.n_real, nf_ = a.Bp > 0 ? (a.Nd - a.n_real) / a.Bp * a.Bt : a.Nd - a.n_real;
    const float cr = (float)a.T * (float)nr_, cf = (float)a.T * (float)nf_;
    const float lr_ = a.n_real > 0 ? tot[0] / cr : 0.f;
    const float lf_ = (a.Nd - a.n_real) > 0 ? tot[1] / cf : 0.f;
    a.loss3[0] = lr_; a.loss3[1] = lf_; a.loss3[2] = lr_ + lf_;
  }
}
void launch_dhead(const DHeadArgs& a, hipStream_t s) {
  const int rows = a.T * a.Nd, nb = (rows + 63) / 64;
  hipLaunchKernelGGL(k_dhead1, dim3(nb), dim3(64), 0, s, a);
  hipLaunchKernelGGL(k_dhead2, dim3(1), dim3(1024), 0, s, a, nb);
}

__global__ void k_build_joint(const float* __restrict__ x, int ldx, int off, int dim, const float* __restrict__ tail, int ldt, int Dt,
                              float* __restrict__ joint, int ldj, int row0, int R) {
  const int W = dim + Dt;
  const size_t total = (size_t)R * W;
  for (size_t i = (size_t)blockIdx.x * blockDim.x + threadIdx.x; i < total; i += (size_t)gridDim.x * blockDim.x) {
    const int r = (int)(i / W), c = (int)(i % W);
    joint[(size_t)(row0 + r) * ldj + c] = c < dim ? x[(size_t)r * ldx + off + c] : tail[(size_t)r * ldt + (c - dim)];
  }
}
void launch_build_joint(const float* x, int ldx, int off, int dim, const float* tail, int ldt, int Dt, float* joint, int ldj,
                        int row0, int R, hipStream_t s) {
  const size_t total = (size_t)R * (dim + Dt);
  const int blocks = (int)min((size_t)2048, (total + 255) / 256);
  hipLaunchKernelGGL(k_build_joint, dim3(blocks), dim3(256), 0, s, x, ldx, off, dim, tail, ldt, Dt, joint, ldj, row0, R);
}
__global__ void k_slice_cols(const float* __restrict__ src, int lds_, int off, float* __restrict__ dst, int ldd, int R, int C) {
  const size_t total = (size_t)R * C;
  for (size_t i = (size_t)blockIdx.x * blockDim.x + threadIdx.x; i < total; i += (size_t)gridDim.x * blockDim.x) {
    const int r = (int)(i / C), c = (int)(i % C);
    dst[(size_t)r * ldd + c] = src[(size_t)r * lds_ + off + c];
  }
}
void launch_slice_cols(const float* src, int lds_, int off, float* dst, int ldd, int R, int C, hipStream_t s) {
  const size_t total = (size_t)R * C;
  const int blocks = (int)min((size_t)2048, (total + 255) / 256);
  hipLaunchKernelGGL(k_slice_cols, dim3(blocks), dim3(256), 0, s, src, lds_, off, dst, ldd, R, C);
}

constexpr int MSE_BLOCKS = 256;
__global__ __launch_bounds__(256) void k_mse1(const float* __restrict__ y, const float* __restrict__ lab, int ld,
                                              float* __restrict__ dy, int rows, int D, const float* __restrict__ lambda,
                                              int accumulate, float* __restrict__ scratch, int Bp, int Bt) {
  __shared__ float red[16];
  const size_t total = (size_t)rows * D;
  const int rows_eff = Bp > 0 ? rows / Bp * Bt : rows;
  const float scale = dy ? (*lambda) / (float)rows_eff : 0.f;
  float s = 0.f;
  for (size_t i = (size_t)blockIdx.x * blockDim.x + threadIdx.x; i < total; i += (size_t)gridDim.x * blockDim.x) {
    const size_t r = i / D; const int c = (int)(i % D);
    const size_t o = r * ld + c;
    const bool valid = Bp <= 0 || (int)(r % Bp) < Bt;
    const float d = valid ? y[o] - lab[o] : 0.f;
    s += d * d;
    if (dy) dy[o] = (accumulate ? dy[o] : 0.f) + scale * d;
  }
  s = block_sum_1024(s, red);
  if (threadIdx.x == 0) scratch[blockIdx.x] = s;
}
__global__ void k_mse2(const float* __restrict__ scratch, int rows, float* __restrict__ out) {
  if (threadIdx.x == 0) {
    float s = 0.f;
    for (int i = 0; i < MSE_BLOCKS; ++i) s += scratch[i];
    *out = 0.5f * s / (float)rows;
  }
}
void launch_mse(const float* y, const float* lab, int ld, float* dy, int rows, int D, const float* lambda,
                bool accumulate, float* loss_out, float* scratch, hipStream_t s, int Bp, int Bt) {
  hipLaunchKernelGGL(k_mse1, dim3(MSE_BLOCKS), dim3(256), 0, s, y, lab, ld, dy, rows, D, lambda, accumulate ? 1 : 0, scratch, Bp, Bt);
  hipLaunchKernelGGL(k_mse2, dim3(1), dim3(64), 0, s, scratch, Bp > 0 ? rows / Bp * Bt : rows, loss_out);
}

__global__ void k_g_total(float* l4, const float* lambda) {
  if (threadIdx.x == 0) l4[3] = l4[0] + (*lambda) * l4[1] + l4[2];
}
void launch_g_total(float* l4, const float* lambda, hipStream_t s) {
  hipLaunchKernelGGL(k_g_total, dim3(1), dim3(64), 0, s, l4, lambda);
}
__global__ void k_copy_f(const float* src, float* dst, int n) {
  const int i = blockIdx.x * blockDim.x + threadIdx.x;
  if (i < n) dst[i] = src[i];
}
void launch_copy_f(const float* src, float* dst, int n, hipStream_t s) {
  hipLaunchKernelGGL(k_copy_f, dim3((n + 255) / 256), dim3(256), 0, s, src, dst, n);
}


__global__ __launch_bounds__(256) void k_sumsq(const float* __restrict__ g, ChunkTable ct, float* __restrict__ partial) {
  __shared__ float red[16];
  const int c = blockIdx.x;
  const float* p = g + ct.off[c];
  const int n = ct.len[c];
  float s = 0.f;
  for (int i = threadIdx.x * 4; i < n; i += 1024) {
    const float4 v = *reinterpret_cast<const float4*>(p + i);
    s += (v.x * v.x + v.y * v.y) + (v.z * v.z + v.w * v.w);
  }
  s = block_sum_1024(s, red);
  if (threadIdx.x == 0) partial[c] = s;
}
void launch_sumsq(const float* g, const ChunkTable& ct, float* partial, hipStream_t s) {
  hipLaunchKernelGGL(k_sumsq, dim3(ct.n_chunks), dim3(256), 0, s, g, ct, partial);
}

__global__ __launch_bounds__(256) void k_dw_reduce(const float* __restrict__ ws, size_t stride, int ntiles, const long long* __restrict__ src,
                                                   float* __restrict__ g, ChunkTable ct, float* __restrict__ partial) {
  __shared__ float red[16];
  const int c = blockIdx.x;
  const int t = ct.tensor[c];
  const int off = ct.off[c], n = ct.len[c];
  const long long so = src[t];
  float s = 0.f;
  if (so < 0) {
    for (int i = threadIdx.x * 4; i < n; i += 1024) {
      const float4 v = *reinterpret_cast<const float4*>(g + off + i);
      s += (v.x * v.x + v.y * v.y) + (v.z * v.z + v.w * v.w);
    }
  } else {
    const float* p = ws + so + (off - ct.off[ct.t_first[t]]);
    for (int i = threadIdx.x * 4; i < n; i += 1024) {
      float4 a = *reinterpret_cast<const float4*>(p + i);
      for (int r = 1; r < ntiles; ++r) {
        const float4 b = *reinterpret_cast<const float4*>(p + (size_t)r * stride + i);
        a.x += b.x; a.y += b.y; a.z += b.z; a.w += b.w;
      }
      *reinterpret_cast<float4*>(g + off + i) = a;
      s += (a.x * a.x + a.y * a.y) + (a.z * a.z + a.w * a.w);
    }
  }
  s = block_sum_1024(s, red);
  if (threadIdx.x == 0) partial[c] = s;
}
void launch_dw_reduce(const float* ws, size_t stride, int ntiles, const long long* src, float* g, const ChunkTable& ct, float* partial, hipStream_t s) {
  hipLaunchKernelGGL(k_dw_reduce, dim3(ct.n_chunks), dim3(256), 0, s, ws, stride, ntiles, src, g, ct, partial);
}

__global__ __launch_bounds__(256) void k_l2(const float* __restrict__ w, float* __restrict__ g, ChunkTable ct,
                                            const float* __restrict__ l2_scale, float* __restrict__ partial) {
  __shared__ float red[16];
  const int c = blockIdx.x;
  const bool on = ct.t_l2[ct.tensor[c]] != 0;
  const int off = ct.off[c], n = ct.len[c];
  const float sc = *l2_scale;
  float s = 0.f;
  if (on) {
    for (int i = threadIdx.x; i < n; i += 256) {
      const float v = w[off + i];
      s += v * v;
      g[off + i] += sc * v;
    }
  }
  s = block_sum_1024(s, red);
  if (threadIdx.x == 0) partial[c] = s;
}
void launch_l2(const float* w, float* g, const ChunkTable& ct, const float* l2_scale, float* partial, hipStream_t s) {
  hipLaunchKernelGGL(k_l2, dim3(ct.n_chunks), dim3(256), 0, s, w, g, ct, l2_scale, partial);
}
__global__ __launch_bounds__(1024) void k_l2_total(const float* __restrict__ partial, int n, const float* __restrict__ l2_scale, float* out) {
  __shared__ float red[16];
  float s = 0.f;
  for (int i = threadIdx.x; i < n; i += blockDim.x) s += partial[i];
  s = block_sum_1024(s, red);
  if (threadIdx.x == 0) *out = 0.5f * (*l2_scale) * s;
}
void launch_l2_total(const float* partial, int n, const float* l2_scale, float* out, hipStream_t s) {
  hipLaunchKernelGGL(k_l2_total, dim3(1), dim3(1024), 0, s, partial, n, l2_scale, out);
}

__device__ __forceinline__ float tensor_clip_scale(const ChunkTable& ct, const float* partial, int c, float clip, float* red) {
  const int t = ct.tensor[c];
  const int first = ct.t_first[t], cnt = ct.t_count[t];
  float s = 0.f;
  for (int i = threadIdx.x; i < cnt; i += blockDim.x) s += partial[first + i];
  s = block_sum_1024(s, red);
  if (!(clip > 0.f)) return 1.0f;
  const float inv = s > 0.f ? 1.0f / sqrtf(s) : __builtin_inff();
  return clip * fminf(inv, 1.0f / clip);
}

__global__ __launch_bounds__(256) void k_apply_sgd(float* __restrict__ w, const float* __restrict__ g, float* __restrict__ ema,
                                                   ChunkTable ct, const float* __restrict__ partial, const float* __restrict__ dyn) {
  __shared__ float red[16];
  const int c = blockIdx.x;
  const float scale = tensor_clip_scale(ct, partial, c, dyn[DYN_CLIP], red);
  const float lr = dyn[DYN_D_LR], dec = dyn[DYN_EMA];
  const int off = ct.off[c], n = ct.len[c];
  for (int i = threadIdx.x; i < n; i += 256) {
    const float nw = w[off + i] - lr * (g[off + i] * scale);
    w[off + i] = nw;
    if (ema) ema[off + i] = dec * ema[off + i] + (1.f - dec) * nw;
  }
}
void launch_apply_sgd(float* w, const float* g, float* ema, const ChunkTable& ct, const float* partial, const float* dyn, hipStream_t s) {
  hipLaunchKernelGGL(k_apply_sgd, dim3(ct.n_chunks), dim3(256), 0, s, w, g, ema, ct, partial, dyn);
}

__global__ __launch_bounds__(256) void k_apply_adam(float* __restrict__ w, const float* __restrict__ g, float* __restrict__ m,
                                                    float* __restrict__ v, float* __restrict__ ema, ChunkTable ct,
                                                    const float* __restrict__ partial, const float* __restrict__ dyn, int lrt_slot) {
  __shared__ float red[16];
  const int c = blockIdx.x;
  const float scale = tensor_clip_scale(ct, partial, c, dyn[DYN_CLIP], red);
  const float b1 = dyn[DYN_B1], b2 = dyn[DYN_B2], eps = dyn[DYN_EPS], lrt = dyn[lrt_slot], dec = dyn[DYN_EMA];
  const int off = ct.off[c], n = ct.len[c];
  for (int i = threadIdx.x; i < n; i += 256) {
    const float gg = g[off + i] * scale;
    const float mm = b1 * m[off + i] + (1.f - b1) * gg;
    const float vv = b2 * v[off + i] + (1.f - b2) * gg * gg;
    m[off + i] = mm; v[off + i] = vv;
    const float nw = w[off + i] - lrt * mm / (sqrtf(vv) + eps);
    w[off + i] = nw;
    if (ema) ema[off + i] = dec * ema[off + i] + (1.f - dec) * nw;
  }
}
void launch_apply_adam(float* w, const float* g, float* m, float* v, float* ema, const ChunkTable& ct,
                       const float* partial, const float* dyn, hipStream_t s, int lrt_slot) {
  hipLaunchKernelGGL(k_apply_adam, dim3(ct.n_chunks), dim3(256), 0, s, w, g, m, v, ema, ct, partial, dyn, lrt_slot);
}

__global__ void k_adam_tick(float* dyn, int* t, double b1, double b2, int lr_slot, int lrt_slot) {
  if (threadIdx.x == 0) {
    const int tt = *t + 1;
    *t = tt;
    dyn[lrt_slot] = (float)((double)dyn[lr_slot] * sqrt(1.0 - pow(b2, (double)tt)) / (1.0 - pow(b1, (double)tt)));
  }
}
void launch_adam_tick(float* dyn, int* t, double b1, double b2, hipStream_t s, int lr_slot, int lrt_slot) {
  hipLaunchKernelGGL(k_adam_tick, dim3(1), dim3(64), 0, s, dyn, t, b1, b2, lr_slot, lrt_slot);
}

__global__ void k_pad_copy(const float* __restrict__ dense_c, float* __restrict__ dense_m, float* __restrict__ padded,
                           int rows, int cols, int ld, int to_padded) {
  const size_t total = (size_t)rows * cols;
  for (size_t i = (size_t)blockIdx.x * blockDim.x + threadIdx.x; i < total; i += (size_t)gridDim.x * blockDim.x) {
    const size_t r = i / cols; const int c = (int)(i % cols);
    if (to_padded) padded[r * ld + c] = dense_c[i];
    else dense_m[i] = padded[r * ld + c];
  }
}
void launch_pad_copy(const float* dense, float* padded, int rows, int cols, int ld, bool to_padded, hipStream_t s) {
  const size_t total = (size_t)rows * cols;
  const int blocks = (int)min((size_t)1024, (total + 255) / 256);
  hipLaunchKernelGGL(k_pad_copy, dim3(blocks), dim3(256), 0, s, dense, const_cast<float*>(dense), padded, rows, cols, ld, to_padded ? 1 : 0);
}

}
```

rsrgan_amd/csrc/model.h:

```cpp
#pragma once
#include <hip/hip_runtime.h>
#include <stdint.h>
#include <string>
#include <unordered_map>
#include <functional>
#include <vector>

#include "../../include/rsrgan.h"
#include "kernels.h"

namespace rsr {

inline int pad4(int x) { return (x + 3) & ~3; }

struct TensorDesc {
  std::string name;
  int rows, cols, ld;
  int64_t off;
  int64_t dense_off;
  bool l2;
  bool trainable = true;
  bool is_vector;
  int xavier_fan_out = 0;
  float bias_init = 0.f;
// ... 298 lines not shown
  std::vector<float> g_w0_host;
  bool g_fc_in_unfolded = false;
  void seq_bn_fold(hipStream_t s);
  void d_dnn_forward_loss(int T, int Nd, int n_real, bool want_grads, float* loss3, hipStream_t s, int calls = 1, int call0 = 0);
  void bn_commit_run(bool with_d, hipStream_t s);
  int dnn_d_backward(const float* x, const float* labels, int T, float* out_losses, bool want_grads, hipStream_t s);
  int dnn_g_backward(const float* x, const float* labels, int T, float* out_losses, bool want_grads, bool reuse, hipStream_t s);

  float *dyn = nullptr;
  int *adam_t_dev = nullptr;
  float *losses = nullptr;
  float *tmp3 = nullptr;
  float *scratch = nullptr;
  double scal[RSRGAN_SCALAR_COUNT_] = {0};
  bool g_fwd_valid = false;
  int cur_T = 0;
  bool d_grads_ready = false, g_grads_ready = false;
  std::vector<void*> allocs;
  size_t alloc_bytes = 0;

  int init(const rsrgan_cfg& c, uint64_t seed);
  int check_cfg() const;
  void build_tables();
  void plan_rows();
  int alloc_params();
  int alloc_generator();
  void alloc_rced();
  int alloc_discriminator();
  int alloc_shared();
  int plan_persistent();
  int plan_dpersist();
  int plan_gpersist();
  int init_values(uint64_t seed);
  size_t frame_rows() const { return (size_t)Tmax * B; }
  int g_ldP() const { return g_dnn() ? 4 : pad4(gR); }
  int d_ldP() const { return d_dnn() ? 4 : pad4(dR); }
  bool res_sums() const { return cfg.g_type == RSRGAN_G_RES_LSTM_L || cfg.g_type == RSRGAN_G_RES_LSTM_I; }
  bool ema_on() const { return cfg.ema_decay > 0.f && !infer(); }
  template <typename T> T* alloc(size_t n);
  template <typename T> T* alloc_opt(size_t n);
  void* alloc_raw(size_t bytes, bool required);
  int alloc_status(const char* stage) const;
  bool alloc_fail = false;
  size_t alloc_fail_bytes = 0;
  void destroy();

  int prepare_batch(const float* x, const float* labels, const int32_t* lengths, int T, hipStream_t s, const float** nr = nullptr,
                    const float** nf = nullptr, hipStream_t early = nullptr);
  void g_forward(int T, hipStream_t s, Chain* extra = nullptr);
  void g_forward_head(int T, hipStream_t s);
  void g_forward_tail(int T, hipStream_t s);
  void d_logits(int N, int T, hipStream_t s);
  void d_backward_pass(int N, int T, bool want_wgrads, bool need_dx0, const float* dlog, hipStream_t s, bool head_done = false);
  bool d_head(int N, int T, int n_real, const float* t_real, const float* t_fake, float* loss3, bool want_grads, bool want_wgrads, hipStream_t s);
  void g_backward_pass(int T, float* dy, hipStream_t s);
  void g_fc_out_wgrads(const float* dy, int R, hipStream_t q);
  float* wire_g_bptt(Chain& ch, float* a, float* b);
  float* wire_d_bptt(Chain& ch, bool want_wgrads, float* din0, bool accumulate0);
  FcStage g_out_fc_stage(const float* nf, int Ns2, int row02);
  bool d_head_or_logits(int N, int T, int n_real, const float* t_fake, float* loss3, bool want_grads, bool want_wgrads, hipStream_t s);
  void g_loss_tail(bool l2, hipStream_t s);
  GRunPlan plan_g_run(int T, const float* nf, bool want_grads, bool reuse, hipStream_t s);
  void g_fc_side_pair(const GRunPlan& p, StreamFn& pre, StreamFn& post);
  bool g_run_forward(const GRunPlan& p, hipStream_t s);
  void g_run_d_forward(const GRunPlan& p, hipStream_t s);
  bool g_run_loss_head(const GRunPlan& p, hipStream_t s);
  bool g_run_backward(const GRunPlan& p, bool g_head, hipStream_t s);
  bool g_run_bptt_fused(const GRunPlan& p, hipStream_t s);
  void g_run_bwd_rest(const GRunPlan& p, hipStream_t s);
  void g_run_tail(const GRunPlan& p, hipStream_t s);
  int g_supervised_step(const float* x, const float* labels, const int32_t* lengths, int T, float* out_losses, bool want_grads, hipStream_t s);
  DRunPlan plan_d_run(int T, const float* nr, const float* nf, bool want_grads, hipStream_t s);
  void d_run_forward(const DRunPlan& p, hipStream_t s);
  void d_run_head_backward(const DRunPlan& p, hipStream_t s);
  bool g_forward_persist(int T, hipStream_t s);
  int d_backward(const float* x, const float* labels, const int32_t* lengths, int T, const float* nr, const float* nf,
                 float* out_losses, bool want_grads, hipStream_t s);
  int g_backward(const float* x, const float* labels, const int32_t* lengths, int T, const float* nf,
                 float* out_losses, bool want_grads, bool reuse, hipStream_t s);
  int apply(int net, hipStream_t s);
  void apply_body(int net, hipStream_t s);
  int apply_inlined = 0;
  void refresh_transposes(int net, hipStream_t s);
  void refresh_swizzles(int net, hipStream_t s);
  bool lazy_sw = false;

  void rnn_forward(std::vector<Chain>& chains, int T, hipStream_t s, const std::vector<int>* offsets = nullptr,
                   const std::vector<FcStage>* fcs = nullptr);
  void rnn_backward(std::vector<Chain>& chains, int T, hipStream_t s, const std::vector<int>* offsets = nullptr,
                    const std::vector<FcStage>* fcs = nullptr);
  void layer_wgrads(const LayerRun& R, int T, hipStream_t s);
  void chain_wgrads(const Chain& ch, int T, hipStream_t s, const StreamFn& between, const StreamFn& pre = nullptr, const StreamFn& post = nullptr);
  void layer_wgrads_gemms(const LayerRun& R, int t0, int t1, bool accumulate, hipStream_t s, bool do_dK = true, bool do_dWp = true);
  int trail_nrt() const;
  bool batch_wgrads(const Chain& ch, int T, hipStream_t s, bool dK_too, bool* dK_done, bool check_only = false);
  void layer_wgrads_colsums(const LayerRun& R, int T, hipStream_t s, float* scr);
  hipStream_t side = nullptr;
  struct GradBucket { int64_t off = 0, count = 0; hipEvent_t ev = nullptr; bool marked = false; };
  std::vector<GradBucket> gbk[2];
  bool fused_apply = false;
  bool defer_wgrads = false;
  int build_buckets();
  void mark_bucket(int net, int i, hipStream_t s);
  void finish_buckets(int net, hipStream_t s);
  bool prof_on = false;
  std::vector<hipEvent_t> prof_ev;
  int prof_n = 0;
  double prof_flops = 0.0;
  std::vector<hipEvent_t> prof_gp_ev;
  int prof_gp_n = 0;
  double prof_gp_flops = 0.0;
  std::vector<hipEvent_t> prof_gb_ev;
  int prof_gb_n = 0;
  int prof_fdt_n = 0;
  int prof_cnt[9] = {};
  double prof_gb_flops = 0.0;
  void gates_launch(const FwdGateJobs& gj, int blocks, int kb, hipStream_t s);
  int gates_blocks(int H, int N) const;
  int proj_blocks(int P, int N) const;
  int bwd_a_blocks(int H, int N) const;
  void run_bwd_b_splitk(BwdBJobs& bj, hipStream_t s);
  hipEvent_t ev_pool[16] = {};
  int ev_next = 0;
  float* gemm_ws2 = nullptr;
  float* dk_tmp = nullptr;
  size_t dk_tmp_per = 0;
  float* scratch2 = nullptr;
  bool overlap() const { return side != nullptr && (cfg.flags & RSRGAN_FLAG_OVERLAP) != 0; }
  Chain g_chain(int T);
  Chain d_chain(int N, int Ns, int row0);
  void gemm(const float* A, int lda, bool a_kc, const float* B, int ldb, bool b_kc, float* C, int ldc, int M, int N,
            int K, const float* bias, int act, float alpha, bool accumulate, hipStream_t s);
  bool supervised() const { return (cfg.flags & RSRGAN_FLAG_SUPERVISED) != 0; }
  bool infer() const { return (cfg.flags & RSRGAN_FLAG_INFER) != 0; }
  static constexpr int INFER_WINDOW = 64;
  int inf_W = 0;
  int* len_win = nullptr;
  int inf_t0 = 0, inf_slot = 0;
  bool inf_failed = false;
  bool infer_fallback_stash();
  void infer_forward(int T, hipStream_t s);
  void infer_window_launches(int t0, int Tw, hipStream_t s);
  void infer_state_to_slot0(hipStream_t s);
  bool wavefront() const { return (cfg.flags & RSRGAN_FLAG_WAVEFRONT) != 0; }
  float* g_fc_out_wT = nullptr;
  float* bwdb_ws = nullptr;
  size_t bwdb_ws_floats = 0;
  bool bwd_b_splitk_ok(const BwdBJobs& jobs) const;
  float* gemm_ws = nullptr;
  size_t gemm_ws_floats = 0;

  struct GraphSlot { int uses = 0; hipGraphExec_t exec = nullptr; };
  std::unordered_map<uint64_t, GraphSlot> graphs;
  hipStream_t main_s = nullptr;
  hipEvent_t ev_in = nullptr, ev_out = nullptr;
  hipEvent_t ev_last = nullptr; bool ev_last_set = false;
  float *noise_r_buf = nullptr, *noise_f_buf = nullptr;
  bool graphs_on() const { return (cfg.flags & RSRGAN_FLAG_GRAPH) != 0 && wavefront() && !overlap() && !prof_on && !g_dnn() && sw.graphs; }
  template <class F> void run_seg(uint64_t key, hipStream_t s, F&& body);
  void drop_graphs();
  hipStream_t enter(hipStream_t caller);
  void leave(hipStream_t caller, hipStream_t work);
  const float* stage_noise(const float* src, float* buf, hipStream_t s);
};

void set_error(const char* fmt, ...);
const char* get_error();

#define HIPC(expr)                                                                   \
  do {                                                                               \
    hipError_t e_ = (expr);                                                          \
    if (e_ != hipSuccess) {                                                          \
      rsr::set_error("%s failed: %s (%s:%d)", #expr, hipGetErrorString(e_), __FILE__, __LINE__); \
      return RSRGAN_ERR_HIP;                                                         \
    }                                                                                \
  } while (0)

}
```

rsrgan_amd/csrc/model_init.cpp:

```cpp
#include "model.h"

#include <algorithm>
#include <cmath>
#include <random>

namespace rsr {

int ParamSet::add(const std::string& name, int rows, int cols, bool is_vector) {
  TensorDesc d;
  d.name = name;
  d.rows = rows; d.cols = cols; d.ld = pad4(cols);
  d.off = padded; d.dense_off = dense;
  d.l2 = name.find("bias") == std::string::npos;
  d.is_vector = is_vector;
  padded += ((int64_t)rows * d.ld + 63) / 64 * 64;
  dense += (int64_t)rows * cols;
  t.push_back(d);
  return (int)t.size() - 1;
}

void* Model::alloc_raw(size_t bytes, bool required) {
  void* p = nullptr;
  if (hipMalloc(&p, bytes) != hipSuccess) {
    if (required && !alloc_fail) { alloc_fail = true; alloc_fail_bytes = bytes; }
// ... 448 lines not shown
      LstmStash S = d_st[l];
      S.mst = alloc<float>((size_t)(Tmax + 1) * 2 * B * F.ldP);
      S.out = nullptr; S.dmt = nullptr; S.dmst = nullptr;
      d_fold_st[l] = S;
    }
  }
  const int dmaxld = std::max(d_ldP(), ldDout);
  if (!inf) { d_dA = alloc<float>(TB2 * dmaxld); d_dB = alloc<float>(TB2 * dmaxld); }
  return alloc_status("discriminator buffers");
}

int Model::alloc_shared() {
  const rsrgan_cfg& c = cfg;
  const bool inf = infer();
  drop_ctr = (unsigned long long*)alloc<float>(4);
  len_dev = alloc<int>(2 * B);
  if (inf) len_win = alloc<int>(B);
  zeros = alloc<float>(64);
  if (!inf) { noise_r_buf = alloc<float>((size_t)B * Dout); noise_f_buf = alloc<float>((size_t)B * Dout); }
  if (hipStreamCreateWithFlags(&main_s, hipStreamNonBlocking) != hipSuccess) main_s = nullptr;
  if (main_s && (hipEventCreateWithFlags(&ev_in, hipEventDisableTiming) != hipSuccess ||
                 hipEventCreateWithFlags(&ev_out, hipEventDisableTiming) != hipSuccess)) { (void)hipStreamDestroy(main_s); main_s = nullptr; }
  dyn = alloc<float>(DYN_COUNT); adam_t_dev = alloc<int>(1);
  losses = alloc<float>(8); tmp3 = alloc<float>(4);
  size_t maxcols = 7 * (size_t)std::max(c.g_cells, c.d_cells);
  maxcols = std::max(maxcols, (size_t)Din + 4);
  maxcols = std::max(maxcols, (size_t)std::max(g_ldP(), ldDin));
  scratch_floats = std::max<size_t>(4 * 64 * maxcols, 16384);
  if (!inf) {
    scratch = alloc<float>(scratch_floats);
    scratch2 = alloc<float>(std::max<size_t>(4 * 64 * maxcols, 1024));
    g_fc_out_wT = g_dnn() ? nullptr : alloc<float>((size_t)Dout * g_ldP());
  }
  if (inf || hipStreamCreateWithFlags(&side, hipStreamNonBlocking) != hipSuccess) side = nullptr;
  if (hipEventCreateWithFlags(&ev_last, hipEventDisableTiming) != hipSuccess) ev_last = nullptr;
  if (side) {
    for (auto& e : ev_pool)
      if (hipEventCreateWithFlags(&e, hipEventDisableTiming) != hipSuccess) { side = nullptr; break; }
  }
  gemm_ws_floats = (size_t)32 << 20;
  gemm_ws = alloc_opt<float>(gemm_ws_floats);
  if (!gemm_ws) gemm_ws_floats = 0;
  bwdb_ws_floats = inf ? 0 : (size_t)8 << 20;
  if (!inf) {
    bwdb_ws = alloc_opt<float>(bwdb_ws_floats);
    gemm_ws2 = alloc_opt<float>(gemm_ws_floats ? gemm_ws_floats : 1);
  }
  if (!inf && switches().dk_pad && !gl.empty() && gl[0].has_proj && gl[0].I % 4 != 0 && gl[0].ldI % 4 == 0 && gl.size() <= (size_t)GEMM_MAXB) {
    dk_tmp_per = (size_t)(gl[0].ldI + gl[0].P) * 4 * gl[0].H;
    dk_tmp = alloc_opt<float>(dk_tmp_per * gl.size());
    if (!dk_tmp) dk_tmp_per = 0;
  }
  if (!gemm_ws2) side = nullptr;
  if (int rc = alloc_status("shared work space")) return rc;
  HIPC(hipMemset(drop_ctr, 0, 16));
  return RSRGAN_OK;
}

int Model::plan_persistent() {
  if (int rc = plan_dpersist()) return rc;
  if (int rc = plan_gpersist()) return rc;
  if (bnl_infer() && !gp_fwd_on()) {
    set_error("g_type bnlstm with RSRGAN_FLAG_INFER: no persistent forward plan for this configuration (batch_size=%d padded to %d rows, %d x %d / p%d; "
              "gpersist_plan's shapes, every workgroup of a row group resident at once, RSRGAN_GPERSIST / RSRGAN_PAD_ROWS not switched off), "
              "and a launch-per-phase forward of the folded cell is not built", Bt, B, cfg.g_layers, cfg.g_cells, cfg.g_proj);
    return RSRGAN_ERR_INVALID;
  }
  GPersistArgs ga{};
  if (sw.trail && dp_gran && (dp_live & 2) && gp_gran1 && gp_gran3 && !gp_noproj && (gp_live & 2) && B % 32 == 0 && gpersist_args(ga, gp_Tcap))
    trail_fits = resident_probe(gpersist_grid(ga) + ((dpersist_trail_grid((int)dl.size(), B) + 7) & ~7), GP_THREADS,
                                std::max(gpersist_lds_bytes(), dpersist_trail_lds_bytes()));
  lazy_sw = switches().lazy_swizzle && wavefront() && gp_gran1 && gp_gran3 && (gp_live & 3) == 3 && dp_gran && (dp_live & 3) == 3;
  if (sw.dpipe > 0 && trail_fits && side && !d_dnn() && dp_max_grid >= dpersist_grid((int)dl.size(), B)) {
    const size_t gb = dpersist_granule_bytes((int)dl.size(), B, Tmax) / 2;
    dp_gran2 = (unsigned long long*)alloc_opt<float>(gb / sizeof(float));
    dp_ctl2 = (unsigned*)alloc_opt<float>(16);
    if (dp_gran2 && dp_ctl2 && hipEventCreateWithFlags(&ev_dfree, hipEventDisableTiming) == hipSuccess &&
        hipEventCreateWithFlags(&ev_real, hipEventDisableTiming) == hipSuccess) {
      HIPC(ctl_reset(dp_ctl2));
      dpipe = true;
    }
  }
  return RSRGAN_OK;
}

int Model::plan_dpersist() {
  if (dp_live && !dl.empty() && dl.size() <= (size_t)DP_MAXL && B % 16 == 0) {
    const int nl_ = (int)dl.size();
    for (int rows : {2 * B, B}) {
      const int g_ = dpersist_grid(nl_, rows);
      if (g_ <= 128 && resident_probe(g_, 512, dpersist_lds_bytes())) { dp_max_grid = g_; break; }
    }
  }
  if (dp_max_grid <= 0) return RSRGAN_OK;
  dp_gran_bytes = dpersist_granule_bytes((int)dl.size(), 2 * B, Tmax);
  dp_gran = (unsigned long long*)alloc<float>(dp_gran_bytes / sizeof(float));
  dp_ctl = (unsigned*)alloc<float>(16);
  if (int rc = alloc_status("persistent discriminator rings")) return rc;
  HIPC(ctl_reset(dp_ctl));
  DPersistArgs pa{};
  pa.nl = (int)dl.size(); pa.N = 2 * B; pa.H = dl[0].H;
  for (size_t l = 0; l < dl.size(); ++l) { pa.L[l].I = dl[l].I; pa.L[l].P = dl[l].P; pa.L[l].ldP = dl[l].ldP; pa.L[l].ldI = dl[l].ldI; }
  bool shapes = switches().dw_inkernel && (dp_live & 2) && dpersist_dw_supported(pa) && !d_adam();
  for (auto& L : dl) shapes = shapes && L.has_proj && L.H == dl[0].H && L.ldH == dl[0].ldH;
  if (shapes && dpersist_grid(pa.nl, pa.N) == dp_max_grid) {
    const int nt = pa.N / 16;
// ... 167 lines not shown
```

rsrgan_amd/csrc/model_step.cpp:

```cpp
#include "model.h"

#include <cmath>
#include <cstdio>
#include <cstdlib>
#include <cstring>

namespace rsr {

static inline uint64_t seg_key(int seg, int T, unsigned bits) { return ((uint64_t)seg << 48) | ((uint64_t)(unsigned)T << 16) | (bits & 0xffffu); }
enum { SEG_D = 1, SEG_G_MAIN = 2, SEG_G_FCIN = 3, SEG_G_LAYER0 = 4 , SEG_G_L2 = 20, SEG_G_TAIL = 21, SEG_APPLY_D = 22, SEG_APPLY_G = 23, SEG_G_BATCH = 24, SEG_BNL = 25 };

template <class F>
void Model::run_seg(uint64_t key, hipStream_t s, F&& body) {
  if (!graphs_on() || s == nullptr) { body(); return; }
  if (graphs.size() > 96) drop_graphs();
  GraphSlot& g = graphs[key];
  if (g.exec) { if (hipGraphLaunch(g.exec, s) != hipSuccess) { (void)hipGetLastError(); g.exec = nullptr; g.uses = -1; body(); } return; }
  if (g.uses < 0) { body(); return; }
  if (g.uses++ == 0) { body(); return; }
  if (hipStreamBeginCapture(s, hipStreamCaptureModeThreadLocal) != hipSuccess) { (void)hipGetLastError(); g.uses = -1; body(); return; }
  body();
  hipGraph_t gr = nullptr;
  if (hipStreamEndCapture(s, &gr) != hipSuccess || !gr) {
    (void)hipGetLastError(); g.uses = -1;
// ... 79 lines not shown
  return ch;
}

Chain Model::d_chain(int N, int Ns, int row0) {
  Chain ch;
  for (size_t l = 0; l < dl.size(); ++l) {
    LayerRun R;
    R.ps = &D; R.L = &dl[l]; R.S = &d_st[l]; R.in = l == 0 ? xd : d_st[l - 1].out;
    R.N = N; R.Ns = Ns; R.row0 = row0; R.len = len_dev + row0;
    R.zx_batched = false;
    ch.push_back(R);
  }
  return ch;
}

void Model::gstate_xfer(int dir, int T, int rows, const int* mask, hipStream_t s) {
  GStateArgs a{};
  a.nl = (int)gl.size(); a.SF = g_state_sf; a.rows = rows; a.dir = dir; a.state = g_state; a.slot = (size_t)T * B; a.mask = mask;
  int off = 0;
  for (size_t l = 0; l < gl.size(); ++l) {
    a.L[l] = GStateLayer{g_st[l].c, g_st[l].mst, gl[l].H, gl[l].P, gl[l].ldP, off};
    off += gl[l].H + gl[l].P;
  }
  launch_gstate(a, s);
}

void Model::g_forward_head(int T, hipStream_t s) {
  if (cfg.g_type == RSRGAN_G_LSTM || g_bnl()) {
    const int P = gR, ldP = pad4(P);
    if (seq_bn_infer()) {
      gemm(x_tm, ldDin, true, G.W(g_fc_in_w), ldP, false, g_h0, ldP, T * B, P, Din, g_bn_fold_b, 1, cfg.lrelu_alpha, false, s);
      return;
    }
    if (seq_bn()) {
      gemm(x_tm, ldDin, true, G.W(g_fc_in_w), ldP, false, g_z0, ldP, T * B, P, Din, nullptr, 0, 0.f, false, s);
      g_fwd_bn_train = bn_training();
      launch_bn_seq_forward(g_z0, ldP, g_h0, ldP, T * B, P, bn_vars(G, g_bn_t), g_bn_stat, ldP, g_fwd_bn_train, true, cfg.lrelu_alpha, pad_Bp(), Bt,
                            g_bn_scr, (size_t)64 * ldP, s);
      return;
    }
    gemm(x_tm, ldDin, true, G.W(g_fc_in_w), ldP, false, g_h0, ldP, T * B, P, Din, G.W(g_fc_in_b), 1, g_bnl() ? 0.f : cfg.lrelu_alpha, false, s);
  }
}
void Model::g_fc_in_backward(float* d, int R, float* colsum_scratch, hipStream_t q) {
  const int P = gR, ldP = pad4(P);
  if (seq_bn()) {
    launch_bn_seq_backward(d, ldP, g_h0, ldP, g_z0, ldP, R, P, g_bn_stat, ldP, G.Gd(g_bn_t[0]), G.Gd(g_bn_t[1]), false, true, cfg.lrelu_alpha,
                           pad_Bp(), Bt, g_bn_sums, g_bn_scr, (size_t)64 * ldP, q);
    gemm(x_tm, ldDin, false, d, ldP, false, G.Gd(g_fc_in_w), ldP, Din, P, R, nullptr, 0, 0.f, false, q);
    return;
  }
  launch_lrelu_bwd(g_h0, d, (size_t)R, P, ldP, cfg.lrelu_alpha, q);
  gemm(x_tm, ldDin, false, d, ldP, false, G.Gd(g_fc_in_w), ldP, Din, P, R, nullptr, 0, 0.f, false, q);
  launch_colsum(d, ldP, nullptr, 0, G.Gd(g_fc_in_b), R, P, colsum_scratch, q);
}
void Model::seq_bn_fold(hipStream_t s) {
  if (!g_fc_in_unfolded) return;
  const TensorDesc& t = G.t[g_fc_in_w];
  g_w0_host.resize((size_t)t.rows * t.ld);
  if (hipMemcpyAsync(g_w0_host.data(), G.W(g_fc_in_w), g_w0_host.size() * sizeof(float), hipMemcpyDeviceToHost, s) != hipSuccess ||
      hipStreamSynchronize(s) != hipSuccess) {
    set_error("RSRGAN_FLAG_BATCH_NORM | RSRGAN_FLAG_INFER: copying the input FC's weights to the host failed");
    inf_failed = true;
    return;
  }
  launch_bn_seq_fold(G.W(g_fc_in_w), t.ld, t.rows, gR, bn_vars(G, g_bn_t), g_bn_fold_b, s);
  g_fc_in_unfolded = false;
}
void Model::seq_bn_commit(int times, hipStream_t s) {
  launch_bn_commit(gR, bn_vars(G, g_bn_t), g_bn_stat, pad4(gR), times, s);
}
void Model::g_forward_tail(int T, hipStream_t s) {
  const int P = gR, ldP = pad4(P);
  gemm(g_ins[gl.size()], ldP, true, G.W(g_fc_out_w), ldDout, false, y_tm, ldDout, T * B, Dout, P, G.W(g_fc_out_b), 0, 0.f, false, s);
  g_fwd_valid = true;
}
void Model::g_forward(int T, hipStream_t s, Chain* extra) {
  if (g_dnn()) { bn_eval_call = false; g_frame_forward(T * B, s); g_fwd_valid = true; return; }
  if (g_bnl() && !infer()) { bnl_forward(T, false, s); return; }
  g_forward_head(T, s);
  if (infer()) { infer_forward(T, s); g_forward_tail(T, s); return; }
  if (!extra && persist_forward_g(T, s)) { g_forward_tail(T, s); return; }
  std::vector<Chain> chains;
  chains.push_back(g_chain(T));
  if (extra) chains.push_back(*extra);
  rnn_forward(chains, T, s);
  g_forward_tail(T, s);
}

bool Model::infer_fallback_stash() {
  for (size_t l = 0; l < gl.size(); ++l) {
    LstmStash& S = g_st[l];
    if (!S.gates) S.gates = alloc_opt<float>((size_t)inf_W * B * 4 * gl[l].H);
    if (!S.h) S.h = alloc_opt<float>((size_t)inf_W * B * gl[l].ldH);
    if (!S.gates || !S.h) return false;
  }
  return true;
}
void Model::infer_window_launches(int t0, int Tw, hipStream_t s) {
  const bool res_l = cfg.g_type == RSRGAN_G_RES_LSTM_L, res_any = res_l || g_resi();
  const size_t top = gl.size() - 1;
  const float* x0 = g_ins[0] + (size_t)t0 * B * gl[0].ldI;
  std::vector<LstmStash> st(g_st);
  Chain ch;
  for (size_t l = 0; l < gl.size(); ++l) {
    const size_t o = l == top ? (size_t)t0 * B * gl[l].ldP : 0;
    if (!res_any) st[l].out += o;
    LayerRun R;
    R.ps = &G; R.L = &gl[l]; R.S = &st[l]; R.in = l == 0 ? x0 : g_ins[l];
    R.N = B; R.Ns = B; R.row0 = 0; R.len = len_win;
    R.zx_batched = (l == 0);
    R.carry = g_carry;
    if (res_l) { R.res_in = R.in; R.res_out = g_res[l] + o; }
    if (g_resi()) { R.res_in = x0; R.res_out = g_res[l] + o; }
    ch.push_back(R);
  }
  std::vector<Chain> chains{ch};
  rnn_forward(chains, Tw, s);
}
void Model::infer_forward(int T, hipStream_t s) {
  const bool carry_in = g_carry;
  bool persist = gp_fwd_on() && wavefront();
  for (int t0 = 0; t0 < T;) {
    const int Tw = std::min(T - t0, persist ? gp_Tcap : inf_W);
    g_carry = carry_in || t0 > 0;
    inf_t0 = t0;
    launch_window_len(len_dev, len_win, B, t0, Tw, s);
    if (persist && persist_forward_g(Tw, s)) {
      inf_slot = 1;
    } else if (bnl_infer()) {
      set_error("g_type bnlstm inference handle: the persistent forward is off after a reported device failure, and no other forward is built");
      inf_failed = true; break;
    } else if (persist) {
      persist = false;
      continue;
    } else {
      if (!infer_fallback_stash()) { set_error("hipMalloc failed (the launch path's stash of an inference handle)"); inf_failed = true; break; }
      infer_window_launches(t0, Tw, s);
      inf_slot = Tw;
    }
    t0 += Tw;
    if (t0 < T) infer_state_to_slot0(s);
  }
  g_carry = carry_in;
  inf_t0 = 0;
}
void Model::infer_state_to_slot0(hipStream_t s) {
  for (size_t l = 0; l < gl.size(); ++l) {
    const size_t nc = (size_t)B * gl[l].H, nm = (size_t)B * gl[l].ldP;
    (void)hipMemcpyAsync(g_st[l].c, g_st[l].c + (size_t)inf_slot * nc, nc * sizeof(float), hipMemcpyDeviceToDevice, s);
    (void)hipMemcpyAsync(g_st[l].mst, g_st[l].mst + (size_t)inf_slot * nm, nm * sizeof(float), hipMemcpyDeviceToDevice, s);
  }
}

void Model::d_logits(int N, int T, hipStream_t s) {
  const int ldPd = pad4(dR);
  gemm(d_st[dl.size() - 1].out, ldPd, true, D.W(d_fc_w), 4, false, logits, 4, T * N, 1, dR, D.W(d_fc_b), 0, 0.f, false, s);
}

bool Model::d_head(int N, int T, int n_real, const float* t_real, const float* t_fake, float* loss3, bool want_grads, bool want_wgrads,
                   hipStream_t s) {
  const int ldPd = pad4(dR), nb = (T * N + 63) / 64;
  if (!switches().dhead || d_dnn() || dl.empty() || dR % 4 != 0 || dR + 3 > 64 ||
      (size_t)nb * (DH_MAXR + 3) > scratch_floats) return false;
  DHeadArgs a{};
  a.top = d_st[dl.size() - 1].out; a.ldt = ldPd; a.w = D.W(d_fc_w); a.ldw = 4; a.b = D.W(d_fc_b);
  a.logits = logits; a.ldl = 4; a.dlogits = dlogits; a.dout = d_dB; a.ldo = ldPd; a.gw = D.Gd(d_fc_w); a.gb = D.Gd(d_fc_b);
  a.T = T; a.Nd = N; a.n_real = n_real; a.dR = dR; a.t_real = t_real; a.t_fake = t_fake; a.loss3 = loss3; a.part = scratch;
  a.want_grads = want_grads ? 1 : 0; a.want_wgrads = want_wgrads ? 1 : 0;
  a.Bp = pad_Bp(); a.Bt = Bt;
  launch_dhead(a, s);
  return true;
}

bool Model::d_head_or_logits(int N, int T, int n_real, const float* t_fake, float* loss3, bool want_grads, bool want_wgrads, hipStream_t s) {
  if (d_head(N, T, n_real, dyn + DYN_D_REAL, t_fake, loss3, want_grads, want_wgrads, s)) return true;
  d_logits(N, T, s);
  launch_lsgan(logits, 4, want_grads ? dlogits : nullptr, T, N, n_real, dyn + DYN_D_REAL, t_fake, loss3, s, false, 0.f, 0.f, pad_Bp(), Bt);
  return false;
}

float* Model::wire_d_bptt(Chain& ch, bool want_wgrads, float* din0, bool accumulate0) {
  float* cur = d_dB;
  float* other = d_dA;
  for (int l = (int)ch.size() - 1; l >= 0; --l) {
    ch[l].dout = cur; ch[l].want_wgrads = want_wgrads;
    if (l == 0) { ch[l].din = din0; ch[l].din_accumulate = accumulate0; }
    else { ch[l].din = other; ch[l].din_accumulate = false; std::swap(cur, other); }
  }
  return other;
}

float* Model::wire_g_bptt(Chain& ch, float* a, float* b) {
  for (int l = (int)ch.size() - 1; l >= 0; --l) {
    ch[l].want_wgrads = true;
    if (cfg.g_type == RSRGAN_G_RES_LSTM_L) {
      ch[l].dout = a; ch[l].din = l > 0 ? a : nullptr; ch[l].din_accumulate = true;
    } else {
      const bool need = cfg.g_type == RSRGAN_G_LSTM || l > 0;
      ch[l].dout = a; ch[l].din = need ? b : nullptr; ch[l].din_accumulate = false;
      std::swap(a, b);
    }
  }
  return a;
}

void Model::g_fc_out_wgrads(const float* dy, int R, hipStream_t q) {
  const int P = gR, ldP = pad4(P);
  gemm(g_ins[gl.size()], ldP, false, dy, ldDout, false, G.Gd(g_fc_out_w), ldDout, P, Dout, R, nullptr, 0, 0.f, false, q);
  launch_colsum(dy, ldDout, nullptr, 0, G.Gd(g_fc_out_b), R, Dout, (side && q == side) ? scratch2 : scratch, q);
}

FcStage Model::g_out_fc_stage(const float* nf, int Ns2, int row02) {
  FcStage F;
  F.offset = (int)gl.size(); F.N = B; F.K = gR; F.D = Dout;
  F.in = g_ins[gl.size()]; F.ld_in = pad4(gR); F.WT = g_fc_out_wT; F.bias = G.W(g_fc_out_b); F.noise = nf;
  F.y = y_tm; F.ldy = ldDout; F.out2 = xd; F.ld2 = ldDout; F.Ns2 = Ns2; F.row02 = row02;
  return F;
}

void Model::g_loss_tail(bool l2, hipStream_t s) {
  if (l2) {
    launch_l2(G.w, G.g, G.ct, dyn + DYN_L2, G.partial, s);
    launch_l2_total(G.partial, G.ct.n_chunks, dyn + DYN_L2, losses + 5, s);
  } else {
    (void)hipMemsetAsync(losses + 5, 0, sizeof(float), s);
  }
  launch_g_total(losses + 3, dyn + DYN_LAMBDA, s);
}

bool Model::g_forward_persist(int T, hipStream_t s) {
  if (!persist_forward_g(T, s)) return false;
  g_forward_tail(T, s);
  return true;
}

void Model::d_backward_pass(int N, int T, bool want_wgrads, bool need_dx0, const float* dlog, hipStream_t s, bool head_done) {
  const int R = T * N;
  const int ldPd = pad4(dR);
  const float* top = d_st[dl.size() - 1].out;
  if (want_wgrads && !head_done) {
    gemm(top, ldPd, false, dlog, 4, false, D.Gd(d_fc_w), 4, dR, 1, R, nullptr, 0, 0.f, false, s);
    launch_colsum(dlog, 4, nullptr, 0, D.Gd(d_fc_b), R, 1, scratch, s);
  }
  if (!head_done) gemm(dlog, 4, true, D.W(d_fc_w), 4, true, d_dB, ldPd, R, dR, 1, nullptr, 0, 0.f, false, s);
  std::vector<Chain> chains(1, d_chain(N, N, 0));
  Chain& ch = chains[0];
  last_dx0 = wire_d_bptt(ch, want_wgrads, nullptr, false);
  if (need_dx0) ch[0].din = last_dx0;
  if (!persist_backward(ch, T, s)) rnn_backward(chains, T, s);
}

void Model::g_backward_pass(int T, float* dy, hipStream_t s) {
  const int R = T * B;
  const int P = gR, ldP = pad4(P);
  g_fc_out_wgrads(dy, R, s);
  gemm(dy, ldDout, true, G.W(g_fc_out_w), ldDout, true, g_dA, ldP, R, P, Dout, nullptr, 0, 0.f, false, s);
  std::vector<Chain> chains(1, g_chain(T));
  float* dh0 = wire_g_bptt(chains[0], g_dA, g_dB);
  if (!persist_backward_g(chains[0], T, s)) rnn_backward(chains, T, s);
  if (cfg.g_type == RSRGAN_G_LSTM) g_fc_in_backward(dh0, R, scratch, s);
}

DRunPlan Model::plan_d_run(int T, const float* nr, const float* nf, bool want_grads, hipStream_t s) {
  DRunPlan p;
  p.T = T; p.want_grads = want_grads; p.nr = nr; p.nf = nf;
  if (dpipe && (!nr || sw.dpipe >= 2) && wavefront() && gp_fwd_on() && !d_dnn() && !seq_drop_on() && T > 0 && T <= Tmax) {
    Chain dchk = d_chain(B, 2 * B, B);
    p.dsplit = persist_forward_real(T, side, true) && persist_forward_g_trail(dchk, T, s, nf, true);
  }
  p.inl = fused_apply && switches().fused_seg && want_grads && !d_dnn() && graphs_on();
  return p;
}

void Model::d_run_forward(const DRunPlan& p, hipStream_t s) {
  const int T = p.T;
  if (p.dsplit) {
    g_forward_head(T, s);
    Chain dch = d_chain(B, 2 * B, B);
    if (persist_forward_g_trail(dch, T, s, p.nf)) return;
  }
  if (wavefront() && gp_fwd_on()) {
    g_forward_head(T, s);
    if (g_forward_persist(T, s)) {
      launch_add_noise_rows(y_tm, p.nf, xd, B, T, Dout, ldDout, 2 * B, B, s);
      if (!d_dnn()) {
        std::vector<Chain> chains(1, d_chain(2 * B, 2 * B, 0));
        if (!persist_forward(chains[0], T, s)) rnn_forward(chains, T, s);
      }
      return;
    }
  }
  if (wavefront()) {
    if (!gp_fwd_on()) g_forward_head(T, s);
    const int Lg = (int)gl.size();
    std::vector<Chain> chains{g_chain(T)};
// ... 80 lines not shown
  p.fcs_inside = p.wave_bwd && !p.bucketed && side && fc_side_env && cfg.g_type == RSRGAN_G_LSTM && p.g_bptt_persist;
  p.inl = fused_apply && fused_seg && p.wave_bwd && !p.bucketed && graphs_on() && !(cfg.g_type == RSRGAN_G_LSTM && !p.fcs_inside);
  p.kbits = (want_grads ? 1u : 0u) | (nf ? 2u : 0u) | (reuse ? 4u : 0u) | (p.l2_on ? 8u : 0u) | (p.bucketed ? 16u : 0u) | (p.inl ? 32u : 0u);
  if (p.g_bptt_persist) {
    Chain dc0 = p.dch;
    dc0[0].din = nullptr;
    p.trail_plan = persist_backward_trail(dc0, T, s, p.dy, ldDout, g_dA, pad4(gR), true);
  }
  p.gsplit = dpipe && p.trail_plan;
  return p;
}

void Model::g_fc_side_pair(const GRunPlan& p, StreamFn& pre, StreamFn& post) {
  if (!p.fcs_inside) return;
  const float* dy = p.dy; float* dh0 = p.dh0; const int R = p.R;
  pre = [this, dy, R](hipStream_t q) { g_fc_out_wgrads(dy, R, q); };
  post = [this, dh0, R](hipStream_t q) { g_fc_in_backward(dh0, R, (side && q == side) ? scratch2 : scratch, q); };
}

bool Model::g_run_forward(const GRunPlan& p, hipStream_t s) {
  const int T = p.T;
  if (p.reuse) return false;
  if (!wavefront()) { g_forward(T, s); return false; }
  if (gp_fwd_on()) {
    g_forward_head(T, s);
    if (!d_dnn()) {
      Chain dch = d_chain(B, B, 0);
      if (persist_forward_g_trail(dch, T, s, p.nf)) return true;
    }
    if (g_forward_persist(T, s)) return false;
  }
  if (!gp_fwd_on()) g_forward_head(T, s);
  std::vector<Chain> chains{g_chain(T)};
  std::vector<int> offs{0};
  if (!d_dnn()) { chains.push_back(d_chain(B, B, 0)); offs.push_back((int)gl.size() + 1); }
  std::vector<FcStage> fcs{g_out_fc_stage(p.nf, B, 0)};
  rnn_forward(chains, T, s, &offs, &fcs);
  return true;
}

void Model::g_run_d_forward(const GRunPlan& p, hipStream_t s) {
  const int T = p.T;
  const bool direct = !p.nf && !d_dnn() && dl[0].ldI == ldDout;
  if (!direct) launch_add_noise_rows(y_tm, p.nf, xd, B, T, Dout, ldDout, B, 0, s);
  if (d_dnn()) return;
  std::vector<Chain> chains(1, d_chain(B, B, 0));
  if (direct) chains[0][0].in = y_tm;
  if (!persist_forward(chains[0], T, s) && !fold_forward(chains[0], T, s)) rnn_forward(chains, T, s);
}

bool Model::g_run_loss_head(const GRunPlan& p, hipStream_t s) {
  bool g_head = false;
  if (d_dnn()) d_dnn_forward_loss(p.T, B, 0, p.want_grads, tmp3, s);
  else g_head = d_head_or_logits(B, p.T, 0, dyn + DYN_D_REAL, tmp3, p.want_grads, false, s);
  launch_copy_f(tmp3 + 1, losses + 3, 1, s);
  return g_head;
}

bool Model::g_run_backward(const GRunPlan& p, bool g_head, hipStream_t s) {
  const int T = p.T, R = p.R;
  if (!p.want_grads) {
    launch_mse(y_tm, lab_tm, ldDout, nullptr, R, Dout, dyn + DYN_LAMBDA, false, losses + 4, scratch, s, pad_Bp(), Bt);
    return true;
  }
  if (d_dnn()) {
    float* dyd = fc_backward(D, dfc, d_act, R, dlogits, false, true, s);
    launch_mse(y_tm, lab_tm, ldDout, dyd, R, Dout, dyn + DYN_LAMBDA, true, losses + 4, scratch, s, pad_Bp(), Bt);
    g_backward_pass(T, dyd, s);
    return true;
  }
  if (!p.wave_bwd) {
    d_backward_pass(B, T, false, true, dlogits, s, g_head);
    float* dyd = last_dx0;
    launch_mse(y_tm, lab_tm, ldDout, dyd, R, Dout, dyn + DYN_LAMBDA, true, losses + 4, scratch, s, pad_Bp(), Bt);
    g_backward_pass(T, dyd, s);
    return true;
  }
  const int Ld = (int)dl.size(), ldPd = pad4(dR);
  if (!g_head) gemm(dlogits, 4, true, D.W(d_fc_w), 4, true, d_dB, ldPd, R, dR, 1, nullptr, 0, 0.f, false, s);
  launch_mse(y_tm, lab_tm, ldDout, p.dy, R, Dout, dyn + DYN_LAMBDA, false, losses + 4, scratch, s, pad_Bp(), Bt);
  if (p.g_bptt_persist) {
    if (!g_run_bptt_fused(p, s)) return false;
  } else {
    FcStage F;
    F.offset = Ld; F.N = B; F.K = Dout; F.D = gR;
    F.in = p.dy; F.ld_in = ldDout; F.WT = G.W(g_fc_out_w); F.y = g_dA; F.ldy = pad4(gR); F.accumulate = false;
    std::vector<int> offs{0, Ld + 1};
    std::vector<FcStage> fcs{F};
    std::vector<Chain> chains{p.dch, p.gch};
    ScopedSet<bool> defer(defer_wgrads, p.bucketed);
    rnn_backward(chains, T, s, &offs, &fcs);
  }
  if (!p.fcs_inside) g_fc_out_wgrads(p.dy, R, s);
  return true;
}

bool Model::g_run_bptt_fused(const GRunPlan& p, hipStream_t s) {
  const int T = p.T, R = p.R, ldP = pad4(gR);
  ScopedSet<bool> defer(defer_wgrads, p.bucketed);
  std::vector<Chain> dc1(1, p.dch);
  dc1[0][0].din = nullptr;
  const bool trailed = p.trail_plan && persist_backward_trail(dc1[0], T, s, p.dy, ldDout, g_dA, ldP);
  if (!trailed) {
    if (!persist_backward(dc1[0], T, s)) rnn_backward(dc1, T, s);
    const int H4d = 4 * dl[0].H;
    gemm(d_st[0].gates, H4d, true, D.W(dl[0].tK), H4d, true, p.dy, ldDout, R, dl[0].I, H4d, nullptr, 0, 0.f, true, s);
    gemm(p.dy, ldDout, true, G.W(g_fc_out_w), ldDout, true, g_dA, ldP, R, gR, Dout, nullptr, 0, 0.f, false, s);
  }
  ScopedSet<bool> trail(gp_trail_next, trailed);
  StreamFn pre, post;
  g_fc_side_pair(p, pre, post);
  ScopedSet<int> phase(gp_phase, p.gsplit ? 1 : 0);
  persist_backward_g(p.gch, T, s, false, pre, post);
  return !p.gsplit;
}

void Model::g_run_bwd_rest(const GRunPlan& p, hipStream_t s) {
  StreamFn pre, post;
  g_fc_side_pair(p, pre, post);
  {
    ScopedSet<int> workers(g_gemm_workers, std::min(g_gemm_workers, switches().dpipe_w));
    {
      ScopedSet<bool> defer(defer_wgrads, p.bucketed);
      ScopedSet<int> phase(gp_phase, 2);
      persist_backward_g(p.gch, p.T, s, false, pre, post);
    }
    if (!p.fcs_inside) g_fc_out_wgrads(p.dy, p.R, s);
  }
  if (p.inl) { g_run_tail(p, s); apply_body(RSRGAN_NET_G, s); }
}

void Model::g_run_tail(const GRunPlan& p, hipStream_t s) {
  g_loss_tail(p.want_grads && p.l2_on, s);
// ... 28 lines not shown

  run_seg(seg_key(SEG_G_MAIN, T, p.kbits | (p.trail_plan ? 64u : 0u) | (p.gsplit ? 128u : 0u)), s, [&]() {
    if (p.trail_plan) gpersist_arm_bytes(g_dA, (size_t)T * B * pad4(gR) * sizeof(float), s);
    if (!g_run_forward(p, s)) g_run_d_forward(p, s);
    const bool g_head = g_run_loss_head(p, s);
    if (!g_run_backward(p, g_head, s)) return;
    if (p.inl) { g_run_tail(p, s); apply_body(RSRGAN_NET_G, s); }
  });
  if (p.gsplit) {
    (void)hipEventRecord(ev_dfree, s);
    dfree_inside = true; dfree_current = true;
    run_seg(seg_key(SEG_G_MAIN, T, p.kbits | 64u | 256u), s, [&]() { g_run_bwd_rest(p, s); });
  }
  if (p.inl) apply_inlined |= 1;
  if (!reuse) g_fwd_valid = true;
  if (p.wave_bwd) {
    int bi = 0;
    if (p.bucketed) mark_bucket(RSRGAN_NET_G, bi++, s);
    if (cfg.g_type == RSRGAN_G_LSTM && !p.fcs_inside) {
      run_seg(seg_key(SEG_G_FCIN, T, p.kbits), s, [&]() { g_fc_in_backward(p.dh0, p.R, scratch, s); });
      if (p.bucketed) mark_bucket(RSRGAN_NET_G, bi++, s);
    }
    if (p.bucketed) {
      bool dkd = false;
      const bool gb = batch_wgrads(p.gch, T, s, false, &dkd, true);
      if (gb) run_seg(seg_key(SEG_G_BATCH, T, p.kbits), s, [&]() { bool d_ = false; (void)batch_wgrads(p.gch, T, s, false, &d_); });
      int li = 0;
      for (auto& Rr : p.gch) {
        run_seg(seg_key(SEG_G_LAYER0 + li, T, p.kbits), s, [&]() { if (gb) layer_wgrads_gemms(Rr, 0, T, false, s, true, false); else layer_wgrads(Rr, T, s); });
        mark_bucket(RSRGAN_NET_G, bi++, s);
        ++li;
      }
    }
  }
  if (!p.inl) run_seg(seg_key(SEG_G_TAIL, T, p.kbits), s, [&]() { g_run_tail(p, s); });
  if (want_grads) {
    if (p.l2_on) for (auto& bk : gbk[RSRGAN_NET_G]) bk.marked = false;
    finish_buckets(RSRGAN_NET_G, s);
    g_grads_ready = true;
  }
  if (out_losses) launch_copy_f(losses + 3, out_losses, 4, s);
  HIPC(hipGetLastError());
  return RSRGAN_OK;
}

int Model::g_supervised_step(const float* x, const float* labels, const int32_t* lengths, int T, float* out_losses, bool want_grads, hipStream_t s) {
  int rc = prepare_batch(x, labels, lengths, T, s);
  if (rc) return rc;
  g_forward(T, s);
  const bool l2s = !cfg.cross_validation && scal[RSRGAN_L2_SCALE] > 0.0;
  HIPC(hipMemsetAsync(losses + 3, 0, sizeof(float), s));
  if (want_grads) {
    float* dy = g_dC;
    launch_mse(y_tm, lab_tm, ldDout, dy, T * B, Dout, dyn + DYN_LAMBDA, false, losses + 4, scratch, s, pad_Bp(), Bt);
    g_backward_pass(T, dy, s);
    if (l2s) {
      launch_l2(G.w, G.g, G.ct, dyn + DYN_L2, G.partial, s);
      launch_l2_total(G.partial, G.ct.n_chunks, dyn + DYN_L2, losses + 5, s);
    }
    if (seq_bn() && bn_training()) seq_bn_commit(2, s);
    { finish_buckets(RSRGAN_NET_G, s); g_grads_ready = true; }
  } else {
    launch_mse(y_tm, lab_tm, ldDout, nullptr, T * B, Dout, dyn + DYN_LAMBDA, false, losses + 4, scratch, s, pad_Bp(), Bt);
  }
  if (!(want_grads && l2s)) HIPC(hipMemsetAsync(losses + 5, 0, sizeof(float), s));
  launch_g_total(losses + 3, dyn + DYN_LAMBDA, s);
  if (out_losses) launch_copy_f(losses + 3, out_losses, 4, s);
  HIPC(hipGetLastError());
  return RSRGAN_OK;
}

int Model::bnl_step(const float* x, const float* labels, const int32_t* lengths, int T, float* out_losses, bool want_grads, hipStream_t s) {
  if (want_grads && cfg.cross_validation) {
    set_error("g_type bnlstm: gradients of the cross_validation model (moving-statistics batch norm) are not built");
    return RSRGAN_ERR_INVALID;
  }
  int rc = prepare_batch(x, labels, lengths, T, s);
  if (rc) return rc;
  const bool l2s = want_grads && scal[RSRGAN_L2_SCALE] > 0.0;
  run_seg(seg_key(SEG_BNL, T, (want_grads ? 1u : 0u) | (l2s ? 2u : 0u)), s, [&]() {
    bnl_forward(T, want_grads, s);
    (void)hipMemsetAsync(losses + 3, 0, sizeof(float), s);
    float* dy = want_grads ? g_dC : nullptr;
    launch_mse(y_tm, lab_tm, ldDout, dy, T * B, Dout, dyn + DYN_LAMBDA, false, losses + 4, scratch, s, pad_Bp(), Bt);
    if (want_grads) bnl_backward(T, dy, s);
    g_loss_tail(l2s, s);
  });
  if (want_grads) { finish_buckets(RSRGAN_NET_G, s); g_grads_ready = true; }
  g_fwd_valid = false;
  if (out_losses) launch_copy_f(losses + 3, out_losses, 4, s);
  HIPC(hipGetLastError());
  return RSRGAN_OK;
}

void Model::apply_body(int net, hipStream_t s) {
  if (net == RSRGAN_NET_D) {
    if (!d_partial_fresh) launch_sumsq(D.g, D.ct, D.partial, s);
    d_partial_fresh = false;
    if (d_adam()) {
      launch_adam_tick(dyn, adam_t_dev_d, (double)cfg.adam_beta1, (double)cfg.adam_beta2, s, DYN_D_LR, DYN_ADAM_LRT_D);
      launch_apply_adam(D.w, D.g, D.m, D.v, D.ema, D.ct, D.partial, dyn, s, DYN_ADAM_LRT_D);
    } else {
      launch_apply_sgd(D.w, D.g, D.ema, D.ct, D.partial, dyn, s);
    }
    refresh_transposes(RSRGAN_NET_D, s);
  } else {
    launch_sumsq(G.g, G.ct, G.partial, s);
    launch_adam_tick(dyn, adam_t_dev, (double)cfg.adam_beta1, (double)cfg.adam_beta2, s);
    launch_apply_adam(G.w, G.g, G.m, G.v, G.ema, G.ct, G.partial, dyn, s);
    refresh_transposes(RSRGAN_NET_G, s);
  }
}

int Model::apply(int net, hipStream_t s) {
  if (net == RSRGAN_NET_D) {
    if (!d_grads_ready) { set_error("apply(D) without gradients"); return RSRGAN_ERR_STATE; }
    if (!(apply_inlined & 2)) run_seg(seg_key(SEG_APPLY_D, 0, 0), s, [&]() { apply_body(RSRGAN_NET_D, s); });
    apply_inlined &= ~2;
    if (d_adam()) scal[RSRGAN_ADAM_STEP_D] += 1;
    d_grads_ready = false;
  } else if (net == RSRGAN_NET_G) {
    if (!g_grads_ready) { set_error("apply(G) without gradients"); return RSRGAN_ERR_STATE; }
    if (!(apply_inlined & 1)) run_seg(seg_key(SEG_APPLY_G, 0, 0), s, [&]() { apply_body(RSRGAN_NET_G, s); });
    if (dfree_current) dfree_inside = true;
    apply_inlined &= ~1;
    scal[RSRGAN_ADAM_STEP] += 1;
    g_grads_ready = false;
    g_fwd_valid = false;
  } else {
    set_error("bad net %d", net);
    return RSRGAN_ERR_INVALID;
  }
  HIPC(hipGetLastError());
  return RSRGAN_OK;
}

}
```

Before: 1.334 million.

## Fuse two-stage reductions via last-block tickets and vectorise split-K and lrelu kernels

```diff
diff --git a/rsrgan_amd/csrc/capi_ops.cpp b/rsrgan_amd/csrc/capi_ops.cpp
--- a/rsrgan_amd/csrc/capi_ops.cpp
+++ b/rsrgan_amd/csrc/capi_ops.cpp
@@ -48,6 +48,14 @@
   if (!sc && hipMalloc((void**)&sc, g_op_scratch_floats * sizeof(float)) != hipSuccess) sc = nullptr;
   return sc;
 }
+static unsigned* op_tickets() {
+  static unsigned* tk = nullptr;
+  if (!tk) {
+    if (hipMalloc((void**)&tk, RED_TICKETS * sizeof(unsigned)) != hipSuccess) tk = nullptr;
+    else if (hipMemset(tk, 0, RED_TICKETS * sizeof(unsigned)) != hipSuccess) { (void)hipFree(tk); tk = nullptr; }
+  }
+  return tk;
+}
 struct WorkersScope {
   int saved;
   explicit WorkersScope(int w) : saved(g_gemm_workers) { if (w > 0) g_gemm_workers = w; }
@@ -171,9 +179,10 @@
   OP_REFUSE(tall && b, "op_colsum: the tall form has no multiplier b");
   OP_REFUSE((size_t)(tall ? 512 : 64) * (size_t)cols > g_op_scratch_floats, "op_colsum: cols = %d exceeds the entry's scratch", cols);
   float* sc = op_scratch();
-  if (!sc) { set_error("op_colsum: hipMalloc failed"); return RSRGAN_ERR_HIP; }
+  unsigned* tk = op_tickets();
+  if (!sc || !tk) { set_error("op_colsum: hipMalloc failed"); return RSRGAN_ERR_HIP; }
   if (tall) launch_colsum_tall(a, lda, out, rows, cols, sc, g_op_scratch_floats, (hipStream_t)stream);
-  else launch_colsum(a, lda, b, ldb, out, rows, cols, sc, (hipStream_t)stream);
+  else launch_colsum(a, lda, b, ldb, out, rows, cols, sc, (hipStream_t)stream, tk);
   OP_LAUNCHED("op_colsum");
 }
 
@@ -848,6 +857,10 @@
       a.logits = FP(3); a.ldl = (int)d[6]; a.dlogits = FP(4); a.dout = FP(5); a.ldo = (int)d[7]; a.gw = FP(6); a.gb = FP(7);
       a.T = (int)d[0]; a.Nd = (int)d[1]; a.n_real = (int)d[2]; a.dR = (int)d[3]; a.t_real = FP(8); a.t_fake = FP(9); a.loss3 = FP(10); a.part = FP(11);
       a.want_grads = (int)d[8]; a.want_wgrads = (int)d[9]; a.Bp = (int)d[10]; a.Bt = (int)d[11];
+      if (!a.want_wgrads) {
+        a.ticket = op_tickets();
+        if (!a.ticket) { set_error(WHO ": hipMalloc failed"); return RSRGAN_ERR_HIP; }
+      }
       launch_dhead(a, s);
       break;
     }
@@ -857,7 +870,9 @@
       OP_BP("rows", d[0], d[4], d[5]);
       OP_REFUSE(d[6] < 1024, WHO ": scratch of %lld floats below launch_mse's 1024", (long long)d[6]);
       OP_PTR("y", ptrs[0], 4); OP_PTR("lab", ptrs[1], 4); OP_OPT("dy", ptrs[2], 4); OP_PTR("lambda", ptrs[3], 4); OP_PTR("loss", ptrs[4], 4); OP_PTR("scratch", ptrs[5], 4);
-      launch_mse(FP(0), FP(1), (int)d[2], FP(2), (int)d[0], (int)d[1], FP(3), d[3] != 0, FP(4), FP(5), s, (int)d[4], (int)d[5]);
+      unsigned* tk = op_tickets();
+      if (!tk) { set_error(WHO ": hipMalloc failed"); return RSRGAN_ERR_HIP; }
+      launch_mse(FP(0), FP(1), (int)d[2], FP(2), (int)d[0], (int)d[1], FP(3), d[3] != 0, FP(4), FP(5), s, (int)d[4], (int)d[5], tk);
       break;
     }
     case 3:
diff --git a/rsrgan_amd/csrc/gemm.hip b/rsrgan_amd/csrc/gemm.hip
--- a/rsrgan_amd/csrc/gemm.hip
+++ b/rsrgan_amd/csrc/gemm.hip
@@ -670,6 +670,76 @@
   }
 }
 
+__device__ __forceinline__ float splitk_finish(float v, const float* __restrict__ bias, int col, int act, float alpha) {
+  if (bias) v += bias[col];
+  if (act == 1) v = fmaxf(v, alpha * v);
+  else if (act == 2) v = fmaxf(v, 0.f);
+  return v;
+}
+__device__ __forceinline__ void splitk_reduce_quads(const float* __restrict__ ws, int ldw, int splits, float* __restrict__ C, int ldc,
+                                                    int M, int N, const float* __restrict__ bias, int act, float alpha, int accumulate) {
+  const unsigned q = (unsigned)(N + 3) >> 2, total = (unsigned)M * q;
+  for (unsigned i = blockIdx.x * 256u + threadIdx.x; i < total; i += gridDim.x * 256u) {
+    const unsigned row = i / q; const int col = (int)(i - row * q) * 4;
+    const float* w = ws + (size_t)row * ldw + col;
+    float* c = C + (size_t)row * ldc + col;
+    const size_t zs = (size_t)M * ldw;
+    if (col + 4 <= N) {
+      float4 v = make_float4(0.f, 0.f, 0.f, 0.f);
+      int z = 0;
+      for (; z + 8 <= splits; z += 8) {
+        float4 p[8];
+#pragma unroll
+        for (int u = 0; u < 8; ++u) p[u] = *reinterpret_cast<const float4*>(w + (z + u) * zs);
+#pragma unroll
+        for (int u = 0; u < 8; ++u) { v.x += p[u].x; v.y += p[u].y; v.z += p[u].z; v.w += p[u].w; }
+      }
+      for (; z < splits; ++z) {
+        const float4 p = *reinterpret_cast<const float4*>(w + z * zs);
+        v.x += p.x; v.y += p.y; v.z += p.z; v.w += p.w;
+      }
+      v.x = splitk_finish(v.x, bias, col, act, alpha); v.y = splitk_finish(v.y, bias, col + 1, act, alpha);
+      v.z = splitk_finish(v.z, bias, col + 2, act, alpha); v.w = splitk_finish(v.w, bias, col + 3, act, alpha);
+      if (accumulate) { const float4 o = *reinterpret_cast<const float4*>(c); v.x += o.x; v.y += o.y; v.z += o.z; v.w += o.w; }
+      *reinterpret_cast<float4*>(c) = v;
+    } else {
+      for (int k = 0; col + k < N; ++k) {
+        float v = 0.f;
+#pragma unroll 8
+        for (int z = 0; z < splits; ++z) v += w[z * zs + k];
+        v = splitk_finish(v, bias, col + k, act, alpha);
+        if (accumulate) v += c[k];
+        c[k] = v;
+      }
+    }
+  }
+}
+__global__ __launch_bounds__(256) void k_splitk_reduce4(const float* __restrict__ ws, int ldw, int splits, float* __restrict__ C,
+                                                        int ldc, int M, int N, const float* __restrict__ bias, int act,
+                                                        float alpha, int accumulate) {
+  splitk_reduce_quads(ws, ldw, splits, C, ldc, M, N, bias, act, alpha, accumulate);
+}
+__global__ __launch_bounds__(256) void k_splitk_reduce4_b(const float* __restrict__ ws, int ldw, int splits, const Gemm16Batch bt, int ldc,
+                                                          int M, int N, int accumulate) {
+  const int p = blockIdx.y;
+  splitk_reduce_quads(ws + (size_t)p * splits * M * ldw, ldw, splits, bt.C[p], ldc, M, N, nullptr, 0, 0.f, accumulate);
+}
+static bool splitk_quads_ok(const float* ws, int ldw, const float* C, int ldc, int M, int N) {
+  return ldw % 4 == 0 && ldc % 4 == 0 && ((size_t)ws & 15) == 0 && ((size_t)C & 15) == 0 && (size_t)M * ((N + 3) / 4) < ((size_t)1 << 31);
+}
+static void launch_splitk_reduce(const float* ws, int ldw, int splits, float* C, int ldc, int M, int N, const float* bias, int act,
+                                 float alpha, int acc, hipStream_t s) {
+  if (splitk_quads_ok(ws, ldw, C, ldc, M, N)) {
+    const size_t total = (size_t)M * ((N + 3) / 4);
+    const int blocks = (int)std::min<size_t>(2048, (total + 255) / 256);
+    hipLaunchKernelGGL(k_splitk_reduce4, dim3(blocks), dim3(256), 0, s, ws, ldw, splits, C, ldc, M, N, bias, act, alpha, acc);
+    return;
+  }
+  const size_t total = (size_t)M * N;
+  const int blocks = (int)std::min<size_t>(2048, (total + 255) / 256);
+  hipLaunchKernelGGL(k_splitk_reduce, dim3(blocks), dim3(256), 0, s, ws, ldw, splits, C, ldc, M, N, bias, act, alpha, acc);
+}
+
 
 constexpr int NBM = 256, NBN = 32, NLDA = 260, NLDB = 36;
 template <bool AKC>
@@ -925,11 +995,7 @@
     hipLaunchKernelGGL((k_gemm16<false, false>), grid, block, 0, s, A, lda, B, ldb, C, ldc, M, N, K, bias, act, alpha, acc, w, ldw, per, A2, lda2, M1);
   else
     hipLaunchKernelGGL((k_gemm16<false, true>), grid, block, 0, s, A, lda, B, ldb, C, ldc, M, N, K, bias, act, alpha, acc, w, ldw, per, A2, lda2, M1);
-  if (splits > 1) {
-    const size_t total = (size_t)M * N;
-    const int blocks = (int)std::min<size_t>(2048, (total + 255) / 256);
-    hipLaunchKernelGGL(k_splitk_reduce, dim3(blocks), dim3(256), 0, s, ws, ldw, splits, C, ldc, M, N, bias, act, alpha, acc);
-  }
+  if (splits > 1) launch_splitk_reduce(ws, ldw, splits, C, ldc, M, N, bias, act, alpha, acc, s);
 }
 
 
@@ -953,9 +1019,12 @@
   hipLaunchKernelGGL(k_gemm16_b, dim3(gx, gy, splits * bt.n), dim3(256), 0, s, bt, lda, ldb, ldc, M, N, K, accumulate ? 1 : 0, w, ldw, per,
                      splits, lda2, M1);
   if (splits > 1) {
-    const size_t total = (size_t)M * N;
+    bool quads = true;
+    for (int p = 0; p < bt.n; ++p) quads = quads && splitk_quads_ok(ws, ldw, bt.C[p], ldc, M, N);
+    const size_t total = quads ? (size_t)M * ((N + 3) / 4) : (size_t)M * N;
     const int blocks = (int)std::min<size_t>(2048, (total + 255) / 256);
-    hipLaunchKernelGGL(k_splitk_reduce_b, dim3(blocks, bt.n), dim3(256), 0, s, ws, ldw, splits, bt, ldc, M, N, accumulate ? 1 : 0);
+    if (quads) hipLaunchKernelGGL(k_splitk_reduce4_b, dim3(blocks, bt.n), dim3(256), 0, s, ws, ldw, splits, bt, ldc, M, N, accumulate ? 1 : 0);
+    else hipLaunchKernelGGL(k_splitk_reduce_b, dim3(blocks, bt.n), dim3(256), 0, s, ws, ldw, splits, bt, ldc, M, N, accumulate ? 1 : 0);
   }
 }
 
@@ -982,11 +1051,7 @@
     g_gemm_last_plan = GemmPlanRecord{GEMM_CLS_N32, NBM, NBN, 0, 0, 0, splits, 0};
     if (a_kc) hipLaunchKernelGGL((k_gemm_n32<true>), grid, block, 0, s, A, lda, B, ldb, C, ldc, M, N, K, bias, act, alpha, acc, w, ldw, per);
     else hipLaunchKernelGGL((k_gemm_n32<false>), grid, block, 0, s, A, lda, B, ldb, C, ldc, M, N, K, bias, act, alpha, acc, w, ldw, per);
-    if (splits > 1) {
-      const size_t total = (size_t)M * N;
-      const int blocks = (int)std::min<size_t>(2048, (total + 255) / 256);
-      hipLaunchKernelGGL(k_splitk_reduce, dim3(blocks), dim3(256), 0, s, ws, ldw, splits, C, ldc, M, N, bias, act, alpha, acc);
-    }
+    if (splits > 1) launch_splitk_reduce(ws, ldw, splits, C, ldc, M, N, bias, act, alpha, acc, s);
     return;
   }
   const double outs = (double)M * N;
diff --git a/rsrgan_amd/csrc/kernels.h b/rsrgan_amd/csrc/kernels.h
--- a/rsrgan_amd/csrc/kernels.h
+++ b/rsrgan_amd/csrc/kernels.h
@@ -297,6 +297,7 @@
 struct ZeroList { int n; float* p[32]; unsigned len[32]; };
 void launch_zero_many(const ZeroList& zl, hipStream_t s);
 struct ColsumsBatch { const float* dz[4]; const float* cprev[4]; const float* ccur[4]; float* db[4]; float* dwi[4]; float* dwf[4]; float* dwo[4]; int n; };
+constexpr int RED_TICKETS = 256;
 void launch_lstm_colsums_batch(const ColsumsBatch& bt, int rows, int H, float* scratch, hipStream_t s);
 void launch_lstm_colsums(const float* dz, const float* cprev, const float* ccur, float* db, float* dwi, float* dwf, float* dwo,
                          int rows, int H, float* scratch , hipStream_t s);
@@ -355,7 +356,7 @@
 bool launch_hist(int n, const HistView* views, float clip_lo, float clip_hi, double* out, hipStream_t s);
 void launch_logits_dense(const float* logits, int frame_rows, int B, int T, float* out, bool clip, float clip_lo, float clip_hi, hipStream_t s);
 void launch_colsum(const float* a, int lda, const float* b, int ldb, float* out, int rows, int cols,
-                   float* scratch , hipStream_t s);
+                   float* scratch , hipStream_t s, unsigned* tickets = nullptr);
 
 constexpr int DH_MAXR = 64;
 struct DHeadArgs {
@@ -363,6 +364,8 @@
   float* logits; int ldl; float* dlogits; float* dout; int ldo; float* gw; float* gb;
   int T, Nd, n_real, dR; const float* t_real; const float* t_fake; float* loss3; float* part; int want_grads, want_wgrads;
   int Bp, Bt;
+  float* adv_out;
+  unsigned* ticket;
 };
 void launch_dhead(const DHeadArgs& a, hipStream_t s);
 void launch_lsgan(const float* logits, int ldl, float* dlogits, int T, int Nd, int n_real,
@@ -372,8 +375,9 @@
                         int row0, int R, hipStream_t s);
 void launch_slice_cols(const float* src, int lds, int off, float* dst, int ldd, int R, int C, hipStream_t s);
 void launch_mse(const float* y, const float* lab, int ld, float* dy, int rows, int D, const float* lambda,
-                bool accumulate, float* loss_out, float* scratch , hipStream_t s, int Bp = 0, int Bt = 0);
-void launch_g_total(float* l4 , const float* lambda, hipStream_t s);
+                bool accumulate, float* loss_out, float* scratch , hipStream_t s, int Bp = 0, int Bt = 0,
+                unsigned* ticket = nullptr);
+void launch_g_total(float* l4 , const float* lambda, hipStream_t s, bool no_l2 = false);
 void launch_copy_f(const float* src, float* dst, int n, hipStream_t s);
 
 struct ChunkTable {
@@ -385,7 +389,8 @@
   const int* t_l2;
   int n_chunks, n_tensors;
 };
-void launch_sumsq(const float* g, const ChunkTable& ct, float* partial, hipStream_t s);
+struct AdamTick { float* dyn; int* t; double b1, b2; int lr_slot, lrt_slot; };
+void launch_sumsq(const float* g, const ChunkTable& ct, float* partial, hipStream_t s, const AdamTick* tick = nullptr);
 void launch_dw_reduce(const float* ws, size_t stride, int ntiles, const long long* src, float* g, const ChunkTable& ct, float* partial, hipStream_t s);
 void launch_l2(const float* w, float* g, const ChunkTable& ct, const float* l2_scale, float* partial, hipStream_t s);
 void launch_l2_total(const float* partial, int n_chunks, const float* l2_scale, float* out, hipStream_t s);
diff --git a/rsrgan_amd/csrc/kernels.hip b/rsrgan_amd/csrc/kernels.hip
--- a/rsrgan_amd/csrc/kernels.hip
+++ b/rsrgan_amd/csrc/kernels.hip
@@ -1292,7 +1292,35 @@
     if (!(hval[o] > 0.f)) d[o] *= alpha;
   }
 }
+__global__ __launch_bounds__(256) void k_lrelu_bwd4(const float* __restrict__ hval, float* __restrict__ d, unsigned rows, int cols, int ld,
+                                                    float alpha) {
+  const unsigned q = (unsigned)(cols + 3) >> 2, total = rows * q;
+  for (unsigned i = blockIdx.x * 256u + threadIdx.x; i < total; i += gridDim.x * 256u) {
+    const unsigned r = i / q; const int c = (int)(i - r * q) * 4;
+    const size_t o = (size_t)r * ld + c;
+    if (c + 4 <= cols) {
+      const float4 h = *reinterpret_cast<const float4*>(hval + o);
+      float4 x = *reinterpret_cast<const float4*>(d + o);
+      if (!(h.x > 0.f)) x.x *= alpha;
+      if (!(h.y > 0.f)) x.y *= alpha;
+      if (!(h.z > 0.f)) x.z *= alpha;
+      if (!(h.w > 0.f)) x.w *= alpha;
+      *reinterpret_cast<float4*>(d + o) = x;
+    } else {
+      for (int k = 0; c + k < cols; ++k)
+        if (!(hval[o + k] > 0.f)) d[o + k] *= alpha;
+    }
+  }
+}
+inline bool aligned16(const void* p) { return ((size_t)p & 15) == 0; }
 void launch_lrelu_bwd(const float* hval, float* d, size_t rows, int cols, int ld, float alpha, hipStream_t s) {
+  const size_t quads = rows * (size_t)((cols + 3) / 4);
+  if (ld % 4 == 0 && aligned16(hval) && aligned16(d) && quads < ((size_t)1 << 31)) {
+    if (quads == 0) return;
+    const int blocks = (int)min((size_t)2048, (quads + 255) / 256);
+    hipLaunchKernelGGL(k_lrelu_bwd4, dim3(blocks), dim3(256), 0, s, hval, d, (unsigned)rows, cols, ld, alpha);
+    return;
+  }
   const size_t total = rows * cols;
   const int blocks = (int)min((size_t)2048, (total + 255) / 256);
   hipLaunchKernelGGL(k_lrelu_bwd, dim3(blocks), dim3(256), 0, s, hval, d, rows, cols, ld, alpha);
@@ -1328,10 +1356,34 @@
   hipLaunchKernelGGL(k_dropout_bwd, dim3((unsigned)std::min<size_t>((n + 255) / 256, 8192)), dim3(256), 0, s, y, d, rows, cols, ld, keep);
 }
 
+__device__ __forceinline__ void store_partial(float* p, float v) { __hip_atomic_store(p, v, __ATOMIC_RELAXED, __HIP_MEMORY_SCOPE_AGENT); }
+__device__ __forceinline__ bool arrived_last(unsigned* ticket, unsigned n, int* flag) {
+  asm volatile("s_waitcnt vmcnt(0)" ::: "memory");
+  __syncthreads();
+  if (threadIdx.x == 0) {
+    const unsigned drawn = __hip_atomic_fetch_add(ticket, 1u, __ATOMIC_RELAXED, __HIP_MEMORY_SCOPE_AGENT);
+    const int last = drawn == n - 1 ? 1 : 0;
+    if (last) {
+      __hip_atomic_store(ticket, 0u, __ATOMIC_RELAXED, __HIP_MEMORY_SCOPE_AGENT);
+      __builtin_amdgcn_fence(__ATOMIC_ACQUIRE, "agent");
+      asm volatile("s_waitcnt vmcnt(0)" ::: "memory");
+    }
+    *flag = last;
+  }
+  __syncthreads();
+  return *flag != 0;
+}
+
 constexpr int CS_SLICES = 64;
+__device__ __forceinline__ void colsum_stage2(const float* scratch, float* __restrict__ out, int cols, int c) {
+  float s = 0.f;
+  for (int i = 0; i < CS_SLICES; ++i) s += scratch[(size_t)i * cols + c];
+  out[c] = s;
+}
 __global__ __launch_bounds__(256) void k_colsum1(const float* __restrict__ a, int lda, const float* __restrict__ b, int ldb,
-                                                 float* __restrict__ scratch, int rows, int cols) {
+                                                 float* scratch, int rows, int cols, float* __restrict__ out, unsigned* tickets) {
   __shared__ float red[4][64];
+  __shared__ int last;
   const int c = blockIdx.x * 64 + (threadIdx.x & 63), rl = threadIdx.x >> 6;
   const int per = (rows + CS_SLICES - 1) / CS_SLICES;
   const int rbeg = blockIdx.y * per, rend = min(rows, rbeg + per);
@@ -1344,15 +1396,17 @@
   }
   red[rl][threadIdx.x & 63] = s;
   __syncthreads();
-  if (rl == 0 && c < cols)
-    scratch[(size_t)blockIdx.y * cols + c] = ((red[0][threadIdx.x] + red[1][threadIdx.x]) + red[2][threadIdx.x]) + red[3][threadIdx.x];
+  if (rl == 0 && c < cols) {
+    const float v = ((red[0][threadIdx.x] + red[1][threadIdx.x]) + red[2][threadIdx.x]) + red[3][threadIdx.x];
+    if (tickets) store_partial(scratch + (size_t)blockIdx.y * cols + c, v); else scratch[(size_t)blockIdx.y * cols + c] = v;
+  }
+  if (!tickets || !arrived_last(tickets + blockIdx.x, gridDim.y, &last)) return;
+  if (rl == 0 && c < cols) colsum_stage2(scratch, out, cols, c);
 }
 __global__ void k_colsum2(const float* __restrict__ scratch, float* __restrict__ out, int cols) {
   const int c = blockIdx.x * blockDim.x + threadIdx.x;
   if (c >= cols) return;
-  float s = 0.f;
-  for (int i = 0; i < CS_SLICES; ++i) s += scratch[(size_t)i * cols + c];
-  out[c] = s;
+  colsum_stage2(scratch, out, cols, c);
 }
 __global__ __launch_bounds__(256) void k_colsum1_n(const float* __restrict__ a, int lda, float* __restrict__ scratch, int rows, int cols,
                                                    int per) {
@@ -1480,9 +1534,11 @@
   hipLaunchKernelGGL(k_lstm_colsums2, dim3((H + 255) / 256), dim3(256), 0, s, scratch, db, dwi, dwf, dwo, H);
 }
 
-void launch_colsum(const float* a, int lda, const float* b, int ldb, float* out, int rows, int cols, float* scratch, hipStream_t s) {
-  hipLaunchKernelGGL(k_colsum1, dim3((cols + 63) / 64, CS_SLICES), dim3(256), 0, s, a, lda, b, ldb, scratch, rows, cols);
-  hipLaunchKernelGGL(k_colsum2, dim3((cols + 255) / 256), dim3(256), 0, s, scratch, out, cols);
+void launch_colsum(const float* a, int lda, const float* b, int ldb, float* out, int rows, int cols, float* scratch, hipStream_t s,
+                   unsigned* tickets) {
+  if (tickets && (cols + 63) / 64 > RED_TICKETS) tickets = nullptr;
+  hipLaunchKernelGGL(k_colsum1, dim3((cols + 63) / 64, CS_SLICES), dim3(256), 0, s, a, lda, b, ldb, scratch, rows, cols, out, tickets);
+  if (!tickets) hipLaunchKernelGGL(k_colsum2, dim3((cols + 255) / 256), dim3(256), 0, s, scratch, out, cols);
 }
 
 __device__ __forceinline__ float block_sum_1024(float v, float* red) {
@@ -1531,8 +1587,38 @@
                      clip_on ? 1 : 0, clip_lo, clip_hi, Bp, Bt);
 }
 
+template <int NT>
+__device__ __forceinline__ void dhead_stage2(const DHeadArgs& a, int nblocks, float* tot) {
+  const int nq = a.want_wgrads ? 3 + a.dR : 2;
+  for (int lt0 = 0; lt0 < 1024 && (lt0 >> 4) < nq; lt0 += NT) {
+    const int lt = lt0 + (int)threadIdx.x;
+    const int q = lt >> 4, j = lt & 15;
+    float s = 0.f;
+    if (q < nq)
+      for (int b = j; b < nblocks; b += 16) s += a.part[(size_t)b * (DH_MAXR + 3) + q];
+    s += __shfl_xor(s, 8); s += __shfl_xor(s, 4); s += __shfl_xor(s, 2); s += __shfl_xor(s, 1);
+    if (q < nq && j == 0) {
+      tot[q] = s;
+      if (a.want_wgrads) {
+        if (q == 2) a.gb[0] = s;
+        if (q >= 3) a.gw[(size_t)(q - 3) * a.ldw] = s;
+      }
+    }
+  }
+  __syncthreads();
+  if (threadIdx.x == 0) {
+    const int nr_ = a.Bp > 0 ? a.n_real / a.Bp * a.Bt : a.n_real, nf_ = a.Bp > 0 ? (a.Nd - a.n_real) / a.Bp * a.Bt : a.Nd - a.n_real;
+    const float cr = (float)a.T * (float)nr_, cf = (float)a.T * (float)nf_;
+    const float lr_ = a.n_real > 0 ? tot[0] / cr : 0.f;
+    const float lf_ = (a.Nd - a.n_real) > 0 ? tot[1] / cf : 0.f;
+    a.loss3[0] = lr_; a.loss3[1] = lf_; a.loss3[2] = lr_ + lf_;
+    if (a.adv_out) *a.adv_out = lf_;
+  }
+}
 __global__ __launch_bounds__(64) void k_dhead1(const DHeadArgs a) {
   __shared__ float wsh[DH_MAXR + 1];
+  __shared__ float tot[DH_MAXR + 3];
+  __shared__ int last;
   const int lane = threadIdx.x;
   const int rows = a.T * a.Nd, dR = a.dR;
   if (lane < dR) wsh[lane] = a.w[(size_t)lane * a.ldw];
@@ -1571,44 +1657,27 @@
   }
   auto wsum = [&](float v) { for (int o = 32; o > 0; o >>= 1) v += __shfl_down(v, o, 64); return v; };
   float* part = a.part + (size_t)blockIdx.x * (DH_MAXR + 3);
+  auto put = [&](float* p, float v) { if (a.ticket) store_partial(p, v); else *p = v; };
   sr = wsum(sr); sf = wsum(sf);
-  if (lane == 0) { part[0] = sr; part[1] = sf; }
+  if (lane == 0) { put(part, sr); put(part + 1, sf); }
   if (a.want_wgrads) {
     const float sd = wsum(dl);
-    if (lane == 0) part[2] = sd;
+    if (lane == 0) put(part + 2, sd);
 #pragma unroll
     for (int c = 0; c < DH_MAXR; ++c)
-      if (c < dR) { const float v = wsum(x[c] * dl); if (lane == 0) part[3 + c] = v; }
-  }
+      if (c < dR) { const float v = wsum(x[c] * dl); if (lane == 0) put(part + 3 + c, v); }
+  }
+  if (!a.ticket || !arrived_last(a.ticket, gridDim.x, &last)) return;
+  dhead_stage2<64>(a, (int)gridDim.x, tot);
 }
 __global__ __launch_bounds__(1024) void k_dhead2(const DHeadArgs a, int nblocks) {
   __shared__ float tot[DH_MAXR + 3];
-  const int q = threadIdx.x >> 4, j = threadIdx.x & 15;
-  const int nq = a.want_wgrads ? 3 + a.dR : 2;
-  float s = 0.f;
-  if (q < nq)
-    for (int b = j; b < nblocks; b += 16) s += a.part[(size_t)b * (DH_MAXR + 3) + q];
-  s += __shfl_xor(s, 8); s += __shfl_xor(s, 4); s += __shfl_xor(s, 2); s += __shfl_xor(s, 1);
-  if (q < nq && j == 0) {
-    tot[q] = s;
-    if (a.want_wgrads) {
-      if (q == 2) a.gb[0] = s;
-      if (q >= 3) a.gw[(size_t)(q - 3) * a.ldw] = s;
-    }
-  }
-  __syncthreads();
-  if (threadIdx.x == 0) {
-    const int nr_ = a.Bp > 0 ? a.n_real / a.Bp * a.Bt : a.n_real, nf_ = a.Bp > 0 ? (a.Nd - a.n_real) / a.Bp * a.Bt : a.Nd - a.n_real;
-    const float cr = (float)a.T * (float)nr_, cf = (float)a.T * (float)nf_;
-    const float lr_ = a.n_real > 0 ? tot[0] / cr : 0.f;
-    const float lf_ = (a.Nd - a.n_real) > 0 ? tot[1] / cf : 0.f;
-    a.loss3[0] = lr_; a.loss3[1] = lf_; a.loss3[2] = lr_ + lf_;
-  }
+  dhead_stage2<1024>(a, nblocks, tot);
 }
 void launch_dhead(const DHeadArgs& a, hipStream_t s) {
   const int rows = a.T * a.Nd, nb = (rows + 63) / 64;
   hipLaunchKernelGGL(k_dhead1, dim3(nb), dim3(64), 0, s, a);
-  hipLaunchKernelGGL(k_dhead2, dim3(1), dim3(1024), 0, s, a, nb);
+  if (!a.ticket) hipLaunchKernelGGL(k_dhead2, dim3(1), dim3(1024), 0, s, a, nb);
 }
 
 __global__ void k_build_joint(const float* __restrict__ x, int ldx, int off, int dim, const float* __restrict__ tail, int ldt, int Dt,
@@ -1640,10 +1709,18 @@
 }
 
 constexpr int MSE_BLOCKS = 256;
+__device__ __forceinline__ float mse_stage2(const float* parts, int rows) {
+  float s = 0.f;
+  for (int i = 0; i < MSE_BLOCKS; ++i) s += parts[i];
+  return 0.5f * s / (float)rows;
+}
 __global__ __launch_bounds__(256) void k_mse1(const float* __restrict__ y, const float* __restrict__ lab, int ld,
                                               float* __restrict__ dy, int rows, int D, const float* __restrict__ lambda,
-                                              int accumulate, float* __restrict__ scratch, int Bp, int Bt) {
+                                              int accumulate, float* scratch, int Bp, int Bt, float* __restrict__ out,
+                                              unsigned* ticket) {
   __shared__ float red[16];
+  __shared__ float parts[MSE_BLOCKS];
+  __shared__ int last;
   const size_t total = (size_t)rows * D;
   const int rows_eff = Bp > 0 ? rows / Bp * Bt : rows;
   const float scale = dy ? (*lambda) / (float)rows_eff : 0.f;
@@ -1657,26 +1734,31 @@
     if (dy) dy[o] = (accumulate ? dy[o] : 0.f) + scale * d;
   }
   s = block_sum_1024(s, red);
-  if (threadIdx.x == 0) scratch[blockIdx.x] = s;
+  if (threadIdx.x == 0) { if (ticket) store_partial(scratch + blockIdx.x, s); else scratch[blockIdx.x] = s; }
+  if (!ticket || !arrived_last(ticket, gridDim.x, &last)) return;
+  parts[threadIdx.x] = scratch[threadIdx.x];
+  __syncthreads();
+  if (threadIdx.x == 0) *out = mse_stage2(parts, rows_eff);
 }
 __global__ void k_mse2(const float* __restrict__ scratch, int rows, float* __restrict__ out) {
+  if (threadIdx.x == 0) *out = mse_stage2(scratch, rows);
+}
+void launch_mse(const float* y, const float* lab, int ld, float* dy, int rows, int D, const float* lambda,
+                bool accumulate, float* loss_out, float* scratch, hipStream_t s, int Bp, int Bt, unsigned* ticket) {
+  hipLaunchKernelGGL(k_mse1, dim3(MSE_BLOCKS), dim3(256), 0, s, y, lab, ld, dy, rows, D, lambda, accumulate ? 1 : 0, scratch, Bp, Bt, loss_out,
+                     ticket);
+  if (!ticket) hipLaunchKernelGGL(k_mse2, dim3(1), dim3(64), 0, s, scratch, Bp > 0 ? rows / Bp * Bt : rows, loss_out);
+}
+
+__global__ void k_g_total(float* l4, const float* lambda, int no_l2) {
   if (threadIdx.x == 0) {
-    float s = 0.f;
-    for (int i = 0; i < MSE_BLOCKS; ++i) s += scratch[i];
-    *out = 0.5f * s / (float)rows;
-  }
-}
-void launch_mse(const float* y, const float* lab, int ld, float* dy, int rows, int D, const float* lambda,
-                bool accumulate, float* loss_out, float* scratch, hipStream_t s, int Bp, int Bt) {
-  hipLaunchKernelGGL(k_mse1, dim3(MSE_BLOCKS), dim3(256), 0, s, y, lab, ld, dy, rows, D, lambda, accumulate ? 1 : 0, scratch, Bp, Bt);
-  hipLaunchKernelGGL(k_mse2, dim3(1), dim3(64), 0, s, scratch, Bp > 0 ? rows / Bp * Bt : rows, loss_out);
-}
-
-__global__ void k_g_total(float* l4, const float* lambda) {
-  if (threadIdx.x == 0) l4[3] = l4[0] + (*lambda) * l4[1] + l4[2];
-}
-void launch_g_total(float* l4, const float* lambda, hipStream_t s) {
-  hipLaunchKernelGGL(k_g_total, dim3(1), dim3(64), 0, s, l4, lambda);
+    if (no_l2) l4[2] = 0.f;
+    const float l2 = no_l2 ? 0.f : l4[2];
+    l4[3] = l4[0] + (*lambda) * l4[1] + l2;
+  }
+}
+void launch_g_total(float* l4, const float* lambda, hipStream_t s, bool no_l2) {
+  hipLaunchKernelGGL(k_g_total, dim3(1), dim3(64), 0, s, l4, lambda, no_l2 ? 1 : 0);
 }
 __global__ void k_copy_f(const float* src, float* dst, int n) {
   const int i = blockIdx.x * blockDim.x + threadIdx.x;
@@ -1687,9 +1769,16 @@
 }
 
 
-__global__ __launch_bounds__(256) void k_sumsq(const float* __restrict__ g, ChunkTable ct, float* __restrict__ partial) {
+__device__ __noinline__ void adam_tick(float* dyn, int* t, double b1, double b2, int lr_slot, int lrt_slot) {
+  const int tt = *t + 1;
+  *t = tt;
+  dyn[lrt_slot] = (float)((double)dyn[lr_slot] * sqrt(1.0 - pow(b2, (double)tt)) / (1.0 - pow(b1, (double)tt)));
+}
+
+__global__ __launch_bounds__(256) void k_sumsq(const float* __restrict__ g, ChunkTable ct, float* __restrict__ partial, AdamTick tick) {
   __shared__ float red[16];
   const int c = blockIdx.x;
+  if (tick.t && c == 0 && threadIdx.x == 0) adam_tick(tick.dyn, tick.t, tick.b1, tick.b2, tick.lr_slot, tick.lrt_slot);
   const float* p = g + ct.off[c];
   const int n = ct.len[c];
   float s = 0.f;
@@ -1700,8 +1789,8 @@
   s = block_sum_1024(s, red);
   if (threadIdx.x == 0) partial[c] = s;
 }
-void launch_sumsq(const float* g, const ChunkTable& ct, float* partial, hipStream_t s) {
-  hipLaunchKernelGGL(k_sumsq, dim3(ct.n_chunks), dim3(256), 0, s, g, ct, partial);
+void launch_sumsq(const float* g, const ChunkTable& ct, float* partial, hipStream_t s, const AdamTick* tick) {
+  hipLaunchKernelGGL(k_sumsq, dim3(ct.n_chunks), dim3(256), 0, s, g, ct, partial, tick ? *tick : AdamTick{});
 }
 
 __global__ __launch_bounds__(256) void k_dw_reduce(const float* __restrict__ ws, size_t stride, int ntiles, const long long* __restrict__ src,
@@ -1779,39 +1868,90 @@
   return clip * fminf(inv, 1.0f / clip);
 }
 
+constexpr int UPD_Q = 4;
+__device__ __forceinline__ float sgd_elem(float w, float g, float scale, float lr) {
+#pragma clang fp contract(off)
+  return __builtin_fmaf(-lr, g * scale, w);
+}
+__device__ __forceinline__ float ema_elem(float e, float nw, float dec) {
+#pragma clang fp contract(off)
+  return dec * e + (1.f - dec) * nw;
+}
 __global__ __launch_bounds__(256) void k_apply_sgd(float* __restrict__ w, const float* __restrict__ g, float* __restrict__ ema,
                                                    ChunkTable ct, const float* __restrict__ partial, const float* __restrict__ dyn) {
   __shared__ float red[16];
   const int c = blockIdx.x;
+  const int off = ct.off[c], n = ct.len[c];
+  float4 g4[UPD_Q], w4[UPD_Q], e4[UPD_Q];
+#pragma unroll
+  for (int k = 0; k < UPD_Q; ++k) {
+    const int i = threadIdx.x * 4 + k * 1024, at = off + (i < n ? i : 0);
+    g4[k] = *reinterpret_cast<const float4*>(g + at);
+    w4[k] = *reinterpret_cast<const float4*>(w + at);
+    e4[k] = *reinterpret_cast<const float4*>((ema ? ema : w) + at);
+  }
   const float scale = tensor_clip_scale(ct, partial, c, dyn[DYN_CLIP], red);
   const float lr = dyn[DYN_D_LR], dec = dyn[DYN_EMA];
-  const int off = ct.off[c], n = ct.len[c];
-  for (int i = threadIdx.x; i < n; i += 256) {
-    const float nw = w[off + i] - lr * (g[off + i] * scale);
-    w[off + i] = nw;
-    if (ema) ema[off + i] = dec * ema[off + i] + (1.f - dec) * nw;
+#pragma unroll
+  for (int k = 0; k < UPD_Q; ++k) {
+    const int i = threadIdx.x * 4 + k * 1024;
+    if (i >= n) break;
+    float4 x = w4[k];
+    x.x = sgd_elem(x.x, g4[k].x, scale, lr); x.y = sgd_elem(x.y, g4[k].y, scale, lr);
+    x.z = sgd_elem(x.z, g4[k].z, scale, lr); x.w = sgd_elem(x.w, g4[k].w, scale, lr);
+    *reinterpret_cast<float4*>(w + off + i) = x;
+    if (ema) {
+      float4 e = e4[k];
+      e.x = ema_elem(e.x, x.x, dec); e.y = ema_elem(e.y, x.y, dec); e.z = ema_elem(e.z, x.z, dec); e.w = ema_elem(e.w, x.w, dec);
+      *reinterpret_cast<float4*>(ema + off + i) = e;
+    }
   }
 }
 void launch_apply_sgd(float* w, const float* g, float* ema, const ChunkTable& ct, const float* partial, const float* dyn, hipStream_t s) {
   hipLaunchKernelGGL(k_apply_sgd, dim3(ct.n_chunks), dim3(256), 0, s, w, g, ema, ct, partial, dyn);
 }
 
+__device__ __forceinline__ void adam_elem(float& w, float g, float& m, float& v, float scale, float b1, float b2, float eps, float lrt) {
+#pragma clang fp contract(off)
+  const float gg = g * scale;
+  const float mm = __builtin_fmaf(b1, m, (1.f - b1) * gg);
+  const float vv = __builtin_fmaf(b2, v, (1.f - b2) * gg * gg);
+  m = mm; v = vv;
+  w = w - lrt * mm / (sqrtf(vv) + eps);
+}
 __global__ __launch_bounds__(256) void k_apply_adam(float* __restrict__ w, const float* __restrict__ g, float* __restrict__ m,
                                                     float* __restrict__ v, float* __restrict__ ema, ChunkTable ct,
                                                     const float* __restrict__ partial, const float* __restrict__ dyn, int lrt_slot) {
   __shared__ float red[16];
   const int c = blockIdx.x;
+  const int off = ct.off[c], n = ct.len[c];
+  float4 g4[UPD_Q], m4[UPD_Q], v4[UPD_Q], w4[UPD_Q], e4[UPD_Q];
+#pragma unroll
+  for (int k = 0; k < UPD_Q; ++k) {
+    const int i = threadIdx.x * 4 + k * 1024, at = off + (i < n ? i : 0);
+    g4[k] = *reinterpret_cast<const float4*>(g + at);
+    m4[k] = *reinterpret_cast<const float4*>(m + at);
+    v4[k] = *reinterpret_cast<const float4*>(v + at);
+    w4[k] = *reinterpret_cast<const float4*>(w + at);
+    e4[k] = *reinterpret_cast<const float4*>((ema ? ema : w) + at);
+  }
   const float scale = tensor_clip_scale(ct, partial, c, dyn[DYN_CLIP], red);
   const float b1 = dyn[DYN_B1], b2 = dyn[DYN_B2], eps = dyn[DYN_EPS], lrt = dyn[lrt_slot], dec = dyn[DYN_EMA];
-  const int off = ct.off[c], n = ct.len[c];
-  for (int i = threadIdx.x; i < n; i += 256) {
-    const float gg = g[off + i] * scale;
-    const float mm = b1 * m[off + i] + (1.f - b1) * gg;
-    const float vv = b2 * v[off + i] + (1.f - b2) * gg * gg;
-    m[off + i] = mm; v[off + i] = vv;
-    const float nw = w[off + i] - lrt * mm / (sqrtf(vv) + eps);
-    w[off + i] = nw;
-    if (ema) ema[off + i] = dec * ema[off + i] + (1.f - dec) * nw;
+#pragma unroll
+  for (int k = 0; k < UPD_Q; ++k) {
+    const int i = threadIdx.x * 4 + k * 1024;
+    if (i >= n) break;
+    float4 x = w4[k], mm = m4[k], vv = v4[k];
+    adam_elem(x.x, g4[k].x, mm.x, vv.x, scale, b1, b2, eps, lrt); adam_elem(x.y, g4[k].y, mm.y, vv.y, scale, b1, b2, eps, lrt);
+    adam_elem(x.z, g4[k].z, mm.z, vv.z, scale, b1, b2, eps, lrt); adam_elem(x.w, g4[k].w, mm.w, vv.w, scale, b1, b2, eps, lrt);
+    *reinterpret_cast<float4*>(m + off + i) = mm;
+    *reinterpret_cast<float4*>(v + off + i) = vv;
+    *reinterpret_cast<float4*>(w + off + i) = x;
+    if (ema) {
+      float4 e = e4[k];
+      e.x = ema_elem(e.x, x.x, dec); e.y = ema_elem(e.y, x.y, dec); e.z = ema_elem(e.z, x.z, dec); e.w = ema_elem(e.w, x.w, dec);
+      *reinterpret_cast<float4*>(ema + off + i) = e;
+    }
   }
 }
 void launch_apply_adam(float* w, const float* g, float* m, float* v, float* ema, const ChunkTable& ct,
@@ -1820,11 +1960,7 @@
 }
 
 __global__ void k_adam_tick(float* dyn, int* t, double b1, double b2, int lr_slot, int lrt_slot) {
-  if (threadIdx.x == 0) {
-    const int tt = *t + 1;
-    *t = tt;
-    dyn[lrt_slot] = (float)((double)dyn[lr_slot] * sqrt(1.0 - pow(b2, (double)tt)) / (1.0 - pow(b1, (double)tt)));
-  }
+  if (threadIdx.x == 0) adam_tick(dyn, t, b1, b2, lr_slot, lrt_slot);
 }
 void launch_adam_tick(float* dyn, int* t, double b1, double b2, hipStream_t s, int lr_slot, int lrt_slot) {
   hipLaunchKernelGGL(k_adam_tick, dim3(1), dim3(64), 0, s, dyn, t, b1, b2, lr_slot, lrt_slot);
diff --git a/rsrgan_amd/csrc/model.h b/rsrgan_amd/csrc/model.h
--- a/rsrgan_amd/csrc/model.h
+++ b/rsrgan_amd/csrc/model.h
@@ -374,13 +374,15 @@
   void g_forward_tail(int T, hipStream_t s);
   void d_logits(int N, int T, hipStream_t s);
   void d_backward_pass(int N, int T, bool want_wgrads, bool need_dx0, const float* dlog, hipStream_t s, bool head_done = false);
-  bool d_head(int N, int T, int n_real, const float* t_real, const float* t_fake, float* loss3, bool want_grads, bool want_wgrads, hipStream_t s);
+  bool d_head(int N, int T, int n_real, const float* t_real, const float* t_fake, float* loss3, bool want_grads, bool want_wgrads, hipStream_t s,
+              float* adv_out = nullptr);
   void g_backward_pass(int T, float* dy, hipStream_t s);
   void g_fc_out_wgrads(const float* dy, int R, hipStream_t q);
   float* wire_g_bptt(Chain& ch, float* a, float* b);
   float* wire_d_bptt(Chain& ch, bool want_wgrads, float* din0, bool accumulate0);
   FcStage g_out_fc_stage(const float* nf, int Ns2, int row02);
-  bool d_head_or_logits(int N, int T, int n_real, const float* t_fake, float* loss3, bool want_grads, bool want_wgrads, hipStream_t s);
+  bool d_head_or_logits(int N, int T, int n_real, const float* t_fake, float* loss3, bool want_grads, bool want_wgrads, hipStream_t s,
+                        float* adv_out = nullptr);
   void g_loss_tail(bool l2, hipStream_t s);
   GRunPlan plan_g_run(int T, const float* nf, bool want_grads, bool reuse, hipStream_t s);
   void g_fc_side_pair(const GRunPlan& p, StreamFn& pre, StreamFn& post);
@@ -448,6 +450,9 @@
   float* dk_tmp = nullptr;
   size_t dk_tmp_per = 0;
   float* scratch2 = nullptr;
+  unsigned* red_tickets = nullptr;
+  unsigned* red_tickets2 = nullptr;
+  unsigned* tk(const float* scr) const { return scr == scratch2 ? red_tickets2 : red_tickets; }
   bool overlap() const { return side != nullptr && (cfg.flags & RSRGAN_FLAG_OVERLAP) != 0; }
   Chain g_chain(int T);
   Chain d_chain(int N, int Ns, int row0);
diff --git a/rsrgan_amd/csrc/model_init.cpp b/rsrgan_amd/csrc/model_init.cpp
--- a/rsrgan_amd/csrc/model_init.cpp
+++ b/rsrgan_amd/csrc/model_init.cpp
@@ -524,6 +524,11 @@
     if (!dk_tmp) dk_tmp_per = 0;
   }
   if (!gemm_ws2) side = nullptr;
+  if (!inf && gemm_ws && gemm_ws2) {
+    gemm_ws_floats -= RED_TICKETS;
+    red_tickets = reinterpret_cast<unsigned*>(gemm_ws + gemm_ws_floats);
+    red_tickets2 = reinterpret_cast<unsigned*>(gemm_ws2 + gemm_ws_floats);
+  }
   if (int rc = alloc_status("shared work space")) return rc;
   HIPC(hipMemset(drop_ctr, 0, 16));
   return RSRGAN_OK;
diff --git a/rsrgan_amd/csrc/model_step.cpp b/rsrgan_amd/csrc/model_step.cpp
--- a/rsrgan_amd/csrc/model_step.cpp
+++ b/rsrgan_amd/csrc/model_step.cpp
@@ -155,7 +155,7 @@
   }
   launch_lrelu_bwd(g_h0, d, (size_t)R, P, ldP, cfg.lrelu_alpha, q);
   gemm(x_tm, ldDin, false, d, ldP, false, G.Gd(g_fc_in_w), ldP, Din, P, R, nullptr, 0, 0.f, false, q);
-  launch_colsum(d, ldP, nullptr, 0, G.Gd(g_fc_in_b), R, P, colsum_scratch, q);
+  launch_colsum(d, ldP, nullptr, 0, G.Gd(g_fc_in_b), R, P, colsum_scratch, q, tk(colsum_scratch));
 }
 void Model::seq_bn_fold(hipStream_t s) {
   if (!g_fc_in_unfolded) return;
@@ -262,7 +262,7 @@
 }
 
 bool Model::d_head(int N, int T, int n_real, const float* t_real, const float* t_fake, float* loss3, bool want_grads, bool want_wgrads,
-                   hipStream_t s) {
+                   hipStream_t s, float* adv_out) {
   const int ldPd = pad4(dR), nb = (T * N + 63) / 64;
   if (!switches().dhead || d_dnn() || dl.empty() || dR % 4 != 0 || dR + 3 > 64 ||
       (size_t)nb * (DH_MAXR + 3) > scratch_floats) return false;
@@ -271,13 +271,15 @@
   a.logits = logits; a.ldl = 4; a.dlogits = dlogits; a.dout = d_dB; a.ldo = ldPd; a.gw = D.Gd(d_fc_w); a.gb = D.Gd(d_fc_b);
   a.T = T; a.Nd = N; a.n_real = n_real; a.dR = dR; a.t_real = t_real; a.t_fake = t_fake; a.loss3 = loss3; a.part = scratch;
   a.want_grads = want_grads ? 1 : 0; a.want_wgrads = want_wgrads ? 1 : 0;
-  a.Bp = pad_Bp(); a.Bt = Bt;
+  a.Bp = pad_Bp(); a.Bt = Bt; a.adv_out = adv_out;
+  a.ticket = want_wgrads ? nullptr : tk(scratch);
   launch_dhead(a, s);
   return true;
 }
 
-bool Model::d_head_or_logits(int N, int T, int n_real, const float* t_fake, float* loss3, bool want_grads, bool want_wgrads, hipStream_t s) {
-  if (d_head(N, T, n_real, dyn + DYN_D_REAL, t_fake, loss3, want_grads, want_wgrads, s)) return true;
+bool Model::d_head_or_logits(int N, int T, int n_real, const float* t_fake, float* loss3, bool want_grads, bool want_wgrads, hipStream_t s,
+                             float* adv_out) {
+  if (d_head(N, T, n_real, dyn + DYN_D_REAL, t_fake, loss3, want_grads, want_wgrads, s, adv_out)) return true;
   d_logits(N, T, s);
   launch_lsgan(logits, 4, want_grads ? dlogits : nullptr, T, N, n_real, dyn + DYN_D_REAL, t_fake, loss3, s, false, 0.f, 0.f, pad_Bp(), Bt);
   return false;
@@ -311,7 +313,8 @@
 void Model::g_fc_out_wgrads(const float* dy, int R, hipStream_t q) {
   const int P = gR, ldP = pad4(P);
   gemm(g_ins[gl.size()], ldP, false, dy, ldDout, false, G.Gd(g_fc_out_w), ldDout, P, Dout, R, nullptr, 0, 0.f, false, q);
-  launch_colsum(dy, ldDout, nullptr, 0, G.Gd(g_fc_out_b), R, Dout, (side && q == side) ? scratch2 : scratch, q);
+  float* scr = (side && q == side) ? scratch2 : scratch;
+  launch_colsum(dy, ldDout, nullptr, 0, G.Gd(g_fc_out_b), R, Dout, scr, q, tk(scr));
 }
 
 FcStage Model::g_out_fc_stage(const float* nf, int Ns2, int row02) {
@@ -326,10 +329,8 @@
   if (l2) {
     launch_l2(G.w, G.g, G.ct, dyn + DYN_L2, G.partial, s);
     launch_l2_total(G.partial, G.ct.n_chunks, dyn + DYN_L2, losses + 5, s);
-  } else {
-    (void)hipMemsetAsync(losses + 5, 0, sizeof(float), s);
-  }
-  launch_g_total(losses + 3, dyn + DYN_LAMBDA, s);
+  }
+  launch_g_total(losses + 3, dyn + DYN_LAMBDA, s, !l2);
 }
 
 bool Model::g_forward_persist(int T, hipStream_t s) {
@@ -344,7 +345,7 @@
   const float* top = d_st[dl.size() - 1].out;
   if (want_wgrads && !head_done) {
     gemm(top, ldPd, false, dlog, 4, false, D.Gd(d_fc_w), 4, dR, 1, R, nullptr, 0, 0.f, false, s);
-    launch_colsum(dlog, 4, nullptr, 0, D.Gd(d_fc_b), R, 1, scratch, s);
+    launch_colsum(dlog, 4, nullptr, 0, D.Gd(d_fc_b), R, 1, scratch, s, tk(scratch));
   }
   if (!head_done) gemm(dlog, 4, true, D.W(d_fc_w), 4, true, d_dB, ldPd, R, dR, 1, nullptr, 0, 0.f, false, s);
   std::vector<Chain> chains(1, d_chain(N, N, 0));
@@ -531,33 +532,33 @@
 bool Model::g_run_loss_head(const GRunPlan& p, hipStream_t s) {
   bool g_head = false;
   if (d_dnn()) d_dnn_forward_loss(p.T, B, 0, p.want_grads, tmp3, s);
-  else g_head = d_head_or_logits(B, p.T, 0, dyn + DYN_D_REAL, tmp3, p.want_grads, false, s);
-  launch_copy_f(tmp3 + 1, losses + 3, 1, s);
+  else g_head = d_head_or_logits(B, p.T, 0, dyn + DYN_D_REAL, tmp3, p.want_grads, false, s, losses + 3);
+  if (!g_head) launch_copy_f(tmp3 + 1, losses + 3, 1, s);
   return g_head;
 }
 
 bool Model::g_run_backward(const GRunPlan& p, bool g_head, hipStream_t s) {
   const int T = p.T, R = p.R;
   if (!p.want_grads) {
-    launch_mse(y_tm, lab_tm, ldDout, nullptr, R, Dout, dyn + DYN_LAMBDA, false, losses + 4, scratch, s, pad_Bp(), Bt);
+    launch_mse(y_tm, lab_tm, ldDout, nullptr, R, Dout, dyn + DYN_LAMBDA, false, losses + 4, scratch, s, pad_Bp(), Bt, tk(scratch));
     return true;
   }
   if (d_dnn()) {
     float* dyd = fc_backward(D, dfc, d_act, R, dlogits, false, true, s);
-    launch_mse(y_tm, lab_tm, ldDout, dyd, R, Dout, dyn + DYN_LAMBDA, true, losses + 4, scratch, s, pad_Bp(), Bt);
+    launch_mse(y_tm, lab_tm, ldDout, dyd, R, Dout, dyn + DYN_LAMBDA, true, losses + 4, scratch, s, pad_Bp(), Bt, tk(scratch));
     g_backward_pass(T, dyd, s);
     return true;
   }
   if (!p.wave_bwd) {
     d_backward_pass(B, T, false, true, dlogits, s, g_head);
     float* dyd = last_dx0;
-    launch_mse(y_tm, lab_tm, ldDout, dyd, R, Dout, dyn + DYN_LAMBDA, true, losses + 4, scratch, s, pad_Bp(), Bt);
+    launch_mse(y_tm, lab_tm, ldDout, dyd, R, Dout, dyn + DYN_LAMBDA, true, losses + 4, scratch, s, pad_Bp(), Bt, tk(scratch));
     g_backward_pass(T, dyd, s);
     return true;
   }
   const int Ld = (int)dl.size(), ldPd = pad4(dR);
   if (!g_head) gemm(dlogits, 4, true, D.W(d_fc_w), 4, true, d_dB, ldPd, R, dR, 1, nullptr, 0, 0.f, false, s);
-  launch_mse(y_tm, lab_tm, ldDout, p.dy, R, Dout, dyn + DYN_LAMBDA, false, losses + 4, scratch, s, pad_Bp(), Bt);
+  launch_mse(y_tm, lab_tm, ldDout, p.dy, R, Dout, dyn + DYN_LAMBDA, false, losses + 4, scratch, s, pad_Bp(), Bt, tk(scratch));
   if (p.g_bptt_persist) {
     if (!g_run_bptt_fused(p, s)) return false;
   } else {
@@ -692,7 +693,7 @@
   HIPC(hipMemsetAsync(losses + 3, 0, sizeof(float), s));
   if (want_grads) {
     float* dy = g_dC;
-    launch_mse(y_tm, lab_tm, ldDout, dy, T * B, Dout, dyn + DYN_LAMBDA, false, losses + 4, scratch, s, pad_Bp(), Bt);
+    launch_mse(y_tm, lab_tm, ldDout, dy, T * B, Dout, dyn + DYN_LAMBDA, false, losses + 4, scratch, s, pad_Bp(), Bt, tk(scratch));
     g_backward_pass(T, dy, s);
     if (l2s) {
       launch_l2(G.w, G.g, G.ct, dyn + DYN_L2, G.partial, s);
@@ -701,10 +702,9 @@
     if (seq_bn() && bn_training()) seq_bn_commit(2, s);
     { finish_buckets(RSRGAN_NET_G, s); g_grads_ready = true; }
   } else {
-    launch_mse(y_tm, lab_tm, ldDout, nullptr, T * B, Dout, dyn + DYN_LAMBDA, false, losses + 4, scratch, s, pad_Bp(), Bt);
-  }
-  if (!(want_grads && l2s)) HIPC(hipMemsetAsync(losses + 5, 0, sizeof(float), s));
-  launch_g_total(losses + 3, dyn + DYN_LAMBDA, s);
+    launch_mse(y_tm, lab_tm, ldDout, nullptr, T * B, Dout, dyn + DYN_LAMBDA, false, losses + 4, scratch, s, pad_Bp(), Bt, tk(scratch));
+  }
+  launch_g_total(losses + 3, dyn + DYN_LAMBDA, s, !(want_grads && l2s));
   if (out_losses) launch_copy_f(losses + 3, out_losses, 4, s);
   HIPC(hipGetLastError());
   return RSRGAN_OK;
@@ -722,7 +722,7 @@
     bnl_forward(T, want_grads, s);
     (void)hipMemsetAsync(losses + 3, 0, sizeof(float), s);
     float* dy = want_grads ? g_dC : nullptr;
-    launch_mse(y_tm, lab_tm, ldDout, dy, T * B, Dout, dyn + DYN_LAMBDA, false, losses + 4, scratch, s, pad_Bp(), Bt);
+    launch_mse(y_tm, lab_tm, ldDout, dy, T * B, Dout, dyn + DYN_LAMBDA, false, losses + 4, scratch, s, pad_Bp(), Bt, tk(scratch));
     if (want_grads) bnl_backward(T, dy, s);
     g_loss_tail(l2s, s);
   });
@@ -735,18 +735,19 @@
 
 void Model::apply_body(int net, hipStream_t s) {
   if (net == RSRGAN_NET_D) {
-    if (!d_partial_fresh) launch_sumsq(D.g, D.ct, D.partial, s);
+    const AdamTick tick{dyn, adam_t_dev_d, (double)cfg.adam_beta1, (double)cfg.adam_beta2, DYN_D_LR, DYN_ADAM_LRT_D};
+    if (!d_partial_fresh) launch_sumsq(D.g, D.ct, D.partial, s, d_adam() ? &tick : nullptr);
+    else if (d_adam()) launch_adam_tick(dyn, adam_t_dev_d, tick.b1, tick.b2, s, DYN_D_LR, DYN_ADAM_LRT_D);
     d_partial_fresh = false;
     if (d_adam()) {
-      launch_adam_tick(dyn, adam_t_dev_d, (double)cfg.adam_beta1, (double)cfg.adam_beta2, s, DYN_D_LR, DYN_ADAM_LRT_D);
       launch_apply_adam(D.w, D.g, D.m, D.v, D.ema, D.ct, D.partial, dyn, s, DYN_ADAM_LRT_D);
     } else {
       launch_apply_sgd(D.w, D.g, D.ema, D.ct, D.partial, dyn, s);
     }
     refresh_transposes(RSRGAN_NET_D, s);
   } else {
-    launch_sumsq(G.g, G.ct, G.partial, s);
-    launch_adam_tick(dyn, adam_t_dev, (double)cfg.adam_beta1, (double)cfg.adam_beta2, s);
+    const AdamTick tick{dyn, adam_t_dev, (double)cfg.adam_beta1, (double)cfg.adam_beta2, DYN_G_LR, DYN_ADAM_LRT};
+    launch_sumsq(G.g, G.ct, G.partial, s, &tick);
     launch_apply_adam(G.w, G.g, G.m, G.v, G.ema, G.ct, G.partial, dyn, s);
     refresh_transposes(RSRGAN_NET_G, s);
   }
```

Result: no change. 1.345 million, median of 6 (+0.8%).
